# dbolya/yolact

Hardware: AMD Instinct MI355X
Metric: images/sec (550x550, batch 8 per GPU), YOLACT yolact_resnet50 forward + Detect (Fast NMS) (higher is better)
Workload: dtype f32 (fp32 in / fp32 accumulate / fp32 out; 93 % of the GEMM time on fp16x2 tiles = every fp32 operand as two fp16 pieces by round to nearest (22 significant bits + 2 signs: exact for ~2/3 of all fp32 values, one fp32 ulp otherwise), 3 exact piece products per product on the fp16 matrix pipe; measure

## Files before the change

include/yolact_amd.h:

```cpp
#ifndef YOLACT_AMD_H
#define YOLACT_AMD_H
#include <stddef.h>
#include <stdint.h>

#ifdef __cplusplus
extern "C" {
#endif

#define YMI_ABI_VERSION 9

#define YMI_EFORMAT (-4)
#define YMI_EUNSUPPORTED (-5)

enum { YMI_ACT_NONE = 0, YMI_ACT_RELU = 1, YMI_ACT_LEAKY01 = 2, YMI_ACT_TANH = 3, YMI_ACT_SIGMOID = 4 };
enum { YMI_RES_NONE = 0, YMI_RES_ADD = 1, YMI_RES_BILINEAR = 2 };

typedef struct {
  int32_t n0, n1;
  int32_t act;
  int32_t row_stride;
  int64_t batch_stride;
  float *ptr;
} ymi_conv_seg;

typedef struct {
  const float *x;
  const float *w;
  const float *scale;
  const float *bias;
  const float *res;
  int32_t B, H, W, Cin, ldx;
  int32_t Ho, Wo, Cout;
  int32_t kh, kw, stride, pad;
  int32_t Kpad;
  int32_t res_mode;
  int32_t res_ld;
  int32_t res_H, res_W;
  int32_t res_after_act;
  int32_t nseg;
  int32_t tile;
  int32_t cin_alg;
  int32_t split_k;
  ymi_conv_seg seg[3];
  const void *w_x3;
  float *split_ws;
  int32_t cout_alg;
  int32_t _pad2;
  const void *w_h2;
  const float *scale_h2;
  const float *winv_h2;
  const float *x_amax;
  float *y_amax;
  float x_amax_mul;
  int32_t _pad3;
} ymi_conv_desc;

enum { YMI_TILE_AUTO = 0, YMI_TILE_128x128 = 1, YMI_TILE_128x64 = 2, YMI_TILE_64x64 = 3, YMI_TILE_128x32 = 4,
       YMI_TILE_64x128 = 5, YMI_TILE_32x32_K4 = 6, YMI_TILE_64x32_K2 = 7, YMI_TILE_32x64_K2 = 8,
       YMI_TILE_64x64_S3 = 9, YMI_TILE_64x64_S4 = 10, YMI_TILE_64x128_S3 = 11, YMI_TILE_128x64_S3 = 12,
       YMI_TILE_32x32_K4_S4 = 13, YMI_TILE_64x32_K2_S3 = 14, YMI_TILE_32x64_K2_S3 = 15,
       YMI_TILE_128x128_W8 = 16, YMI_TILE_256x128_W8 = 17, YMI_TILE_128x256_W8 = 18,
       YMI_TILE_128x128_S3 = 19, YMI_TILE_128x128_W8_S3 = 20, YMI_TILE_256x128_W8_S3 = 21, YMI_TILE_128x128_W8_S4 = 22,
       YMI_TILE_WG_128x256 = 23,
       YMI_TILE_X3 = 32,
       YMI_TILE_H2 = 64,
       YMI_TILE_DCNP = 128 };
enum { YMI_DCNP_64x128 = 1, YMI_DCNP_64x128_W8 = 2, YMI_DCNP_64x64 = 3, YMI_DCNP_128x128_W8 = 4, YMI_DCNP_128x64_W8 = 5,
       YMI_DCNP_32x128 = 6,
       YMI_DCNP_96x128_W6 = 7, YMI_DCNP_128x128_W8_R1 = 8, YMI_DCNP_160x128_W10 = 9, YMI_DCNP_192x128_W12 = 10,
       YMI_DCNP_64x256_W8 = 11, YMI_DCNP_96x256_W12 = 12, YMI_DCNP_128x256_W16 = 13,
       YMI_DCNP_128x256_W8T = 14, YMI_DCNP_128x128_W4T = 15, YMI_DCNP_256x128_W8T = 16,
       YMI_DCNP_128x32_W4 = 17, YMI_DCNP_256x32_W8 = 18, YMI_DCNP_64x32_W2 = 19,
       YMI_DCNP_WS_128x32_W4 = 20, YMI_DCNP_WS_256x32_W8 = 21, YMI_DCNP_WS_256x32_W4 = 22, YMI_DCNP_WS_512x32_W8 = 23,
       YMI_DCNP_WS_128x64_W4 = 24, YMI_DCNP_WS_256x64_W8 = 25, YMI_DCNP_WS_256x64_W4 = 26, YMI_DCNP_WS_512x64_W8 = 27,
       YMI_DCNP_PATCH_C64 = 28,
       YMI_DCNP_PC_128x128 = 29,
       YMI_DCNP_PATCH2_256 = 30, YMI_DCNP_PATCH2_192 = 31 };

int ymi_abi_version(void);
const char *ymi_strerror(int code);

int ymi_conv2d_nhwc_f32(const ymi_conv_desc *d, void *stream);
double ymi_conv_flops(const ymi_conv_desc *d);
int ymi_conv_pick_tile(const ymi_conv_desc *d);

typedef struct {
  const float *x;
  const float *u;
  const float *scale;
  const float *bias;
  float *y;
  float *V, *M;
  int32_t B, H, W, C, Cout;
  int32_t act;
  int32_t tile;
  int32_t nseg;
  int32_t m;
  int32_t _pad0;
  ymi_conv_seg seg[3];
  const void *u_x3;
  int32_t cout_alg;
  int32_t v_planes;
  const void *u_h2;
  const float *uinv_h2;
  const float *x_amax;
  float *y_amax;
  const float *x_up;
  int32_t up_relu, _pad4;
  const void *proj_w_h2;
  const float *proj_scale_h2, *proj_bias;
  float *proj_y, *proj_y_amax;
  int32_t proj_cout, proj_ldy, proj_act, _pad5;
} ymi_wino_desc;
int ymi_conv3x3_winograd_f32(const ymi_wino_desc *d, void *stream);

#define YMI_AMAX_SUB 16
#define YMI_AMAX_STRIDE 64
int ymi_amax_f32(const float *x, long n, float *out, void *stream);

int ymi_nchw_to_nhwc4_f32(const float *x, float *y, int B, int C, int H, int W, void *stream);
int ymi_nchw_to_nhwc4_amax_f32(const float *x, float *y, int B, int C, int H, int W, float *amax, void *stream);
int ymi_nhwc_to_nchw_f32(const float *x, float *y, int B, int C, int H, int W, void *stream);
int ymi_maxpool3x3s2_nhwc_f32(const float *x, float *y, int B, int H, int W, int C, int Ho, int Wo, void *stream);
int ymi_bilinear_nhwc_f32(const float *x, float *y, int B, int Hi, int Wi, int C, int Ho, int Wo,
                          float scale_h, float scale_w, int relu, void *stream);

int ymi_bilinear_add_nhwc_f32(const float *x, float *y, int B, int Hi, int Wi, int C, int Ho, int Wo, float *y_amax, void *stream);

int ymi_conv2d_direct_nhwc_f32(const float *x, const float *w, const float *bias, float *y, int B, int H, int W,
                               int Cin, int Ho, int Wo, int Cout, int kh, int kw, int stride, int pad, int relu,
                               void *stream);
int ymi_global_maxpool_nhwc_f32(const float *x, float *y, int B, int HW, int C, void *stream);

typedef struct {
  const float *conf;
  const float *loc;
  const float *coef;
  const float *priors;
  int32_t B, P, C, D;
  int32_t conf_is_logits;
  int32_t top_k;
  int32_t max_det;
  float conf_thresh;
  float nms_thresh;
  int32_t cross_class;
  int32_t conf_ld;
  int32_t _pad1;
  float *scores_t;
  int32_t *keep;
  int32_t *num_keep;
  float *maxsc;
  int32_t *argmax;
  float *cand_score;
  int32_t *cand_prior;
  int32_t *out_count;
  float *out_box;
  float *out_score;
  int64_t *out_class;
  float *out_coef;
  int32_t *out_prior;
  float *out_rec;
} ymi_detect_desc;
int ymi_detect_f32(const ymi_detect_desc *d, void *stream);

typedef struct {
  float box_scale;
  int32_t _pad0;
  void *ws;
} ymi_detect_greedy_ws;
int ymi_detect_traditional_f32(const ymi_detect_desc *d, const ymi_detect_greedy_ws *g, void *stream);

int ymi_lincomb_crop_f32(const float *proto, const float *coef, const float *box, float *masks_lo,
                         int ph, int pw, int D, int N, int crop, void *stream);
int ymi_mask_upsample_f32(const float *masks_lo, float *out, int N, int ph, int pw, int h, int w,
                          float thresh, void *stream);
int ymi_lincomb_crop_batch_f32(const float *proto, const float *coef, const float *box, const int32_t *count,
                               float *masks_lo, int B, int cap, int ph, int pw, int D, int crop, void *stream);
int ymi_mask_upsample_batch_f32(const float *masks_lo, const int32_t *count, float *out, int B, int cap, int ph, int pw,
                                int h, int w, float thresh, void *stream);
int ymi_boxes_to_pixels(const float *box, int64_t *out, int N, int w, int h, void *stream);

int ymi_fast_base_transform_f32(const float *img, float *out, int N, int H, int W, int oh, int ow,
                                const float *mean_bgr, const float *std_bgr, int mode, int out_nhwc4, void *stream);

int ymi_mask_iou_f32(const float *masks_a, const float *masks_b, int A, int B, long n, int iscrowd, float *ws, float *iou,
                     void *stream);

int ymi_jaccard_f32(const float *box_a, const float *box_b, int A, int B, int iscrowd, float *out, void *stream);
int ymi_mask_bits_f32(const float *masks, int N, long n, uint64_t *bits, void *stream);
int ymi_mask_upsample_bits(const float *masks_lo, int N, int ph, int pw, int h, int w, float thresh, uint64_t *bits, void *stream);
int ymi_mask_iou_bits(const uint64_t *bits_a, const uint64_t *bits_b, int A, int B, long W64, int iscrowd, float *iou, void *stream);

#define YMI_AP_NUM_THRESH 10
#define YMI_AP_MAX_DET 1024
#define YMI_AP_MAX_GT 2048
typedef struct {
  const int64_t *cls;
  const float *box_score;
  const float *mask_score;
  const float *box_iou;
  const float *mask_iou;
  const float *crowd_box_iou;
  const float *crowd_mask_iou;
  const int32_t *gt_cls;
  const int32_t *crowd_cls;
  int64_t *rec_key;
  float *rec_score;
  int32_t *rec_flags;
  int64_t *gt_count;
  int64_t base, cap;
  int32_t N, G, Gc, num_classes;
} ymi_ap_match_desc;
typedef struct {
  const int64_t *sorted_key;
  const int64_t *perm;
  const int32_t *rec_flags;
  const int64_t *gt_count;
  double *ap;
  int32_t *empty;
  int64_t M, cap;
  int32_t num_classes, _pad0;
} ymi_ap_finalize_desc;
int ymi_ap_match_f32(const ymi_ap_match_desc *d, void *stream);
int ymi_ap_finalize_f64(const ymi_ap_finalize_desc *d, void *stream);

int ymi_composite_masks_u8(const float *img, const float *masks, const float *colors, int n, int h, int w, float alpha,
                           unsigned char *out, void *stream);

int ymi_mask_rle_f32(const float *masks, int N, int h, int w, uint32_t *counts, int32_t *nruns, int cap, void *stream);
int ymi_mask_rle_upsampled_f32(const float *masks_lo, int N, int ph, int pw, int h, int w, float thresh, uint32_t *counts,
                               int32_t *nruns, int cap, void *stream);
int ymi_rle_to_string(const uint32_t *counts, const int32_t *nruns, int N, int cap, uint8_t *str, int32_t *nchars,
                      int cap_chars, void *stream);

enum { YMI_JPEG_YCBCR = 0, YMI_JPEG_RGB = 1, YMI_JPEG_GRAY = 2 };
typedef struct {
  int32_t width, height;
  int32_t ncomp;
  int32_t progressive;
  int32_t orientation;
  int32_t color;
  int32_t out_width, out_height;
  int32_t hs[3], vs[3];
  int32_t hf[3], vf[3];
  int32_t bw[3], bh[3];
  int32_t dw[3], dh[3];
  int64_t coef_count;
  int64_t plane_bytes;
} ymi_jpeg_info;
int ymi_jpeg_parse(const uint8_t *data, size_t n, ymi_jpeg_info *info);
int ymi_jpeg_decode_coefs(const uint8_t *data, size_t n, int16_t *coefs, int64_t coef_capacity, uint16_t *qt,
                          ymi_jpeg_info *info);
int ymi_jpeg_reconstruct_bgr_u8(const ymi_jpeg_info *info, const int16_t *coefs, const uint16_t *qt, uint8_t *planes_ws,
                                uint8_t *out, void *stream);

enum { YMI_JPEG_SUB_444 = 0, YMI_JPEG_SUB_420 = 2 };
#define YMI_JPEG_HEADER_BYTES 623
typedef struct ymi_jpeg_enc_desc {
  const uint8_t *img;
  int32_t h, w;
  int64_t row_stride;
  int32_t quality;
  int32_t subsampling;
  uint8_t *out;
  int64_t out_capacity;
  int64_t *out_len;
  void *ws;
} ymi_jpeg_enc_desc;
int ymi_jpeg_write_header(int h, int w, int quality, int subsampling, uint8_t *out, size_t cap, size_t *n);
int ymi_jpeg_enc_qtables(int quality, uint16_t *qt);
int ymi_jpeg_encode_bgr_u8(const ymi_jpeg_enc_desc *d, void *stream);

int ymi_coco_poly_fill_u8(const double *xy, int k, int h, int w, uint8_t *mask);
int ymi_coco_rle_fill_u8(const uint32_t *counts, long n, int h, int w, uint8_t *mask);
int ymi_coco_rle_string_fill_u8(const char *s, long len, int h, int w, uint8_t *mask);

typedef struct {
  ymi_conv_desc conv;
  const float *offmask;
  int32_t ldo;
  int32_t mask_is_prob;
  int32_t om_layout;
  int32_t _pad1;
} ymi_dcn_desc;
int ymi_dcn_v2_forward_f32(const ymi_dcn_desc *d, void *stream);

typedef struct ymi_dcn_bwd_desc {
  const float *x;
  const float *offmask;
  const float *w;
  const float *gy;
  float *gx;
  float *g_offset;
  float *g_mask;
  float *gw;
  float *gbias;
  int32_t B, H, W, Cin, ldx, Ho, Wo, Cout;
  int32_t kh, kw, stride, pad, dilation, deformable_groups;
  int32_t ldo, mask_is_prob, om_layout, _pad0;
} ymi_dcn_bwd_desc;
int ymi_dcn_v2_backward_f32(const ymi_dcn_bwd_desc *d, void *stream);

typedef struct ymi_stem_desc {
  const float *x;
  float *y;
  int32_t B, H, W, cout_pad;
  const void *w_h2;
  const float *scale_h2, *bias;
  float *y_amax;
  int32_t kpad, _pad0;
} ymi_stem_desc;
int ymi_stem_pool_f32(const ymi_stem_desc *d, void *stream);

typedef struct ymi_chain_desc {
  const float *x, *res;
  float *y, *z;
  const void *w_a_h2, *w_b_h2;
  const float *scale_a_h2, *bias_a, *scale_b_h2, *bias_b;
  const float *x_amax;
  float *y_amax, *z_amax;
  int64_t M;
  int32_t ldx, res_ld, ldy, ldz;
  int32_t k_a, n_a, n_b;
  int32_t cout_pad_a, cout_pad_b;
  int32_t act_a, act_b, _pad0;
  const float *res_amax;
  float gain_a, bias_max_a;
} ymi_chain_desc;
int ymi_pointwise_chain_f32(const ymi_chain_desc *d, void *stream);

enum { YMI_OP_NOP = 0, YMI_OP_CONV = 1, YMI_OP_WINO = 2, YMI_OP_DCN = 3, YMI_OP_CHAIN = 4, YMI_OP_STEM = 5, YMI_OP_INPUT = 6,
       YMI_OP_BILINEAR = 7, YMI_OP_MAXPOOL = 8, YMI_OP_BILINEAR_ADD = 9, YMI_OP_RECORD = 10, YMI_OP_WAIT = 11, YMI_OP_MEMSET = 12 };
enum { YMI_SEC_NONE = 0, YMI_SEC_BACKBONE = 1, YMI_SEC_FPN = 2, YMI_SEC_PROTO = 3, YMI_SEC_HEADS = 4 };
typedef struct ymi_plan_op {
  int32_t kind;
  int32_t stream;
  int32_t section;
  int32_t _pad;
  const void *desc;
  void *p[3];
  int64_t i[8];
  double f[2];
} ymi_plan_op;
int ymi_event_create(void **ev);
int ymi_event_destroy(void *ev);
int ymi_plan_run(const ymi_plan_op *ops, int first, int last, void *stream_a, void *stream_b, void *const *events, int overlap,
                 int skip_sections, int32_t *failed_op);

enum {
  YMI_WS_WINO_V = 1,
  YMI_WS_WINO_M = 2,
  YMI_WS_SPLITK = 3,
  YMI_WS_MASK_IOU = 4,
  YMI_WS_JPEG_COEFS = 5,
  YMI_WS_JPEG_PLANES = 6,
  YMI_WS_DETECT_SCORES_T = 7,
  YMI_WS_DETECT_PER_PRIOR = 8,
  YMI_WS_DETECT_CAND = 9,
  YMI_WS_DETECT_REC = 10,
  YMI_WS_AMAX_SLOT = 11,
  YMI_WS_RLE_COUNTS = 12,
  YMI_WS_DETECT_GREEDY = 13,
  YMI_WS_JPEG_ENC = 14,
  YMI_WS_JPEG_ENC_OUT = 15
};
typedef struct { int32_t A, B; int64_t n; } ymi_mask_iou_shape;
typedef struct { int32_t N, h, w, cap; } ymi_rle_shape;
int64_t ymi_workspace_bytes(int what, const void *desc);

int ymi_calib_mfma_f16(float *out, int blocks, int iters, double *flops, void *stream);
int ymi_calib_hbm_copy(const float *src, float *dst, long n_floats, double *bytes, void *stream);
int ymi_calib_l2_read(const float *src, long n_floats, int blocks, int iters, float *out, double *bytes, void *stream);
int ymi_calib_latency(const int32_t *chain, long n, int start, int hops, int32_t *out, void *stream);

int ymi_debug_set_trace(void *buf, long cap_blocks);
int ymi_prof_enable(int on);
int ymi_prof_count(void);
int ymi_prof_read(int i, float *ms, double *flops, int32_t *tile, int32_t *kind);
int ymi_prof_reset(void);

#ifdef __cplusplus
}
#endif
#endif
```

yolact_amd/_lib.py:

```python
from __future__ import annotations

import ctypes as C
import os

_HERE = os.path.dirname(os.path.abspath(__file__))
LIB_PATH = os.path.join(_HERE, 'libyolact_amd.so')

ABI_VERSION = 9

ACT_NONE, ACT_RELU, ACT_LEAKY01, ACT_TANH, ACT_SIGMOID = 0, 1, 2, 3, 4
RES_NONE, RES_ADD, RES_BILINEAR = 0, 1, 2
TILE_AUTO, TILE_128x128, TILE_128x64, TILE_64x64, TILE_128x32, TILE_64x128 = 0, 1, 2, 3, 4, 5
TILE_32x32_K4, TILE_64x32_K2, TILE_32x64_K2 = 6, 7, 8
TILE_64x64_S3, TILE_64x64_S4, TILE_64x128_S3, TILE_128x64_S3, TILE_32x32_K4_S4, TILE_64x32_K2_S3, TILE_32x64_K2_S3 = range(9, 16)
TILE_NAMES = {1: '128x128', 2: '128x64', 3: '64x64', 4: '128x32', 5: '64x128', 6: '32x32k4', 7: '64x32k2', 8: '32x64k2',
              9: '64x64s3', 10: '64x64s4', 11: '64x128s3', 12: '128x64s3', 13: '32x32k4s4', 14: '64x32k2s3', 15: '32x64k2s3',
              16: '128x128w8', 17: '256x128w8', 18: '128x256w8', 19: '128x128s3', 20: '128x128w8s3', 21: '256x128w8s3',
              22: '128x128w8s4'}
TILE_128x128_W8, TILE_256x128_W8, TILE_128x256_W8 = 16, 17, 18
TILE_128x128_S3, TILE_128x128_W8_S3, TILE_256x128_W8_S3, TILE_128x128_W8_S4 = 19, 20, 21, 22
TILE_WG_128x256 = 23
TILE_X3 = 32
X3_BASE_TILES = (1, 2, 3, 5, 6, 7, 8, 9, 11, 12, 16, 17, 19, 20, 21, 22)
for _t in X3_BASE_TILES:
    TILE_NAMES[_t | TILE_X3] = TILE_NAMES[_t] + 'x3'
BASIC_TILES = (1, 2, 3, 4, 5)
TILE_H2 = 64
H2_BASE_TILES = X3_BASE_TILES + (18, 13, 14, 15)
for _t in H2_BASE_TILES:
    TILE_NAMES[_t | TILE_H2] = TILE_NAMES[_t] + 'h2'
TILE_NAMES[TILE_WG_128x256 | TILE_H2] = 'wg128x256h2'
TILE_DCNP = 128
DCNP_64x128, DCNP_64x128_W8, DCNP_64x64, DCNP_128x128_W8, DCNP_128x64_W8, DCNP_32x128 = 1, 2, 3, 4, 5, 6
DCNP_96x128_W6, DCNP_128x128_W8_R1, DCNP_160x128_W10, DCNP_192x128_W12, DCNP_64x256_W8, DCNP_96x256_W12, DCNP_128x256_W16 = range(7, 14)
DCNP_TILES = {1: 'dcnp64x128', 2: 'dcnp64x128w8', 3: 'dcnp64x64', 4: 'dcnp128x128w8', 5: 'dcnp128x64w8', 6: 'dcnp32x128',
              7: 'dcnp96x128w6', 8: 'dcnp128x128w8r1', 9: 'dcnp160x128w10', 10: 'dcnp192x128w12',
              11: 'dcnp64x256w8', 12: 'dcnp96x256w12', 13: 'dcnp128x256w16',
              14: 'dcnp128x256w8t', 15: 'dcnp128x128w4t', 16: 'dcnp256x128w8t',
              17: 'dcnp128x32w4', 18: 'dcnp256x32w8', 19: 'dcnp64x32w2'}
DCNP_128x32_W4, DCNP_256x32_W8, DCNP_64x32_W2 = 17, 18, 19
DCNP_PLAIN_ONLY = (14, 15, 16, 17, 18, 19)
WS_TILES = {20: 'ws128x32w4', 21: 'ws256x32w8', 22: 'ws256x32w4', 23: 'ws512x32w8',
            24: 'ws128x64w4', 25: 'ws256x64w8', 26: 'ws256x64w4', 27: 'ws512x64w8'}
DCNP_WS_128x32_W4, DCNP_WS_512x64_W8 = 20, 27
DCNP_PATCH_C64 = 28
PATCH_TILES = {28: 'patch8x16c64'}
PC_TILES = {29: 'pc128x128'}
DCNP_PC_128x128 = 29
PATCH2_TILES = {30: 'patch2p256', 31: 'patch2p192'}
DCNP_PATCH2_256, DCNP_PATCH2_192 = 30, 31
for _t, _n in list(DCNP_TILES.items()) + list(WS_TILES.items()) + list(PATCH_TILES.items()) + list(PC_TILES.items()) + list(PATCH2_TILES.items()):
    TILE_NAMES[_t | TILE_H2 | TILE_DCNP] = _n
WINO_PLANES = 1024
KSPLIT_TILES = (6, 7, 8, 13, 14, 15, 6 | 32, 7 | 32, 8 | 32, 6 | 64, 7 | 64, 8 | 64, 13 | 64, 14 | 64, 15 | 64)


class ConvSeg(C.Structure):
    _fields_ = [('n0', C.c_int32), ('n1', C.c_int32), ('act', C.c_int32), ('row_stride', C.c_int32),
                ('batch_stride', C.c_int64), ('ptr', C.c_void_p)]


class ConvDesc(C.Structure):
    _fields_ = [('x', C.c_void_p), ('w', C.c_void_p), ('scale', C.c_void_p), ('bias', C.c_void_p),
                ('res', C.c_void_p),
                ('B', C.c_int32), ('H', C.c_int32), ('W', C.c_int32), ('Cin', C.c_int32), ('ldx', C.c_int32),
                ('Ho', C.c_int32), ('Wo', C.c_int32), ('Cout', C.c_int32),
                ('kh', C.c_int32), ('kw', C.c_int32), ('stride', C.c_int32), ('pad', C.c_int32),
                ('Kpad', C.c_int32), ('res_mode', C.c_int32), ('res_ld', C.c_int32),
                ('res_H', C.c_int32), ('res_W', C.c_int32), ('res_after_act', C.c_int32),
                ('nseg', C.c_int32), ('tile', C.c_int32), ('cin_alg', C.c_int32), ('split_k', C.c_int32),
                ('seg', ConvSeg * 3), ('w_x3', C.c_void_p), ('split_ws', C.c_void_p), ('cout_alg', C.c_int32),
                ('_pad2', C.c_int32),
                ('w_h2', C.c_void_p), ('scale_h2', C.c_void_p), ('winv_h2', C.c_void_p), ('x_amax', C.c_void_p),
                ('y_amax', C.c_void_p), ('x_amax_mul', C.c_float), ('_pad3', C.c_int32)]


class WinoDesc(C.Structure):
    _fields_ = [('x', C.c_void_p), ('u', C.c_void_p), ('scale', C.c_void_p), ('bias', C.c_void_p), ('y', C.c_void_p),
                ('V', C.c_void_p), ('M', C.c_void_p),
                ('B', C.c_int32), ('H', C.c_int32), ('W', C.c_int32), ('C', C.c_int32), ('Cout', C.c_int32),
                ('act', C.c_int32), ('tile', C.c_int32), ('nseg', C.c_int32), ('m', C.c_int32), ('_pad0', C.c_int32),
                ('seg', ConvSeg * 3), ('u_x3', C.c_void_p), ('cout_alg', C.c_int32), ('v_planes', C.c_int32),
                ('u_h2', C.c_void_p), ('uinv_h2', C.c_void_p), ('x_amax', C.c_void_p), ('y_amax', C.c_void_p),
                ('x_up', C.c_void_p), ('up_relu', C.c_int32), ('_pad4', C.c_int32),
                ('proj_w_h2', C.c_void_p), ('proj_scale_h2', C.c_void_p), ('proj_bias', C.c_void_p),
                ('proj_y', C.c_void_p), ('proj_y_amax', C.c_void_p),
                ('proj_cout', C.c_int32), ('proj_ldy', C.c_int32), ('proj_act', C.c_int32), ('_pad5', C.c_int32)]


class DcnDesc(C.Structure):
    _fields_ = [('conv', ConvDesc), ('offmask', C.c_void_p), ('ldo', C.c_int32), ('mask_is_prob', C.c_int32),
                ('om_layout', C.c_int32), ('_pad1', C.c_int32)]


class DcnBwdDesc(C.Structure):
    _fields_ = [('x', C.c_void_p), ('offmask', C.c_void_p), ('w', C.c_void_p), ('gy', C.c_void_p),
                ('gx', C.c_void_p), ('g_offset', C.c_void_p), ('g_mask', C.c_void_p), ('gw', C.c_void_p), ('gbias', C.c_void_p),
                ('B', C.c_int32), ('H', C.c_int32), ('W', C.c_int32), ('Cin', C.c_int32), ('ldx', C.c_int32),
                ('Ho', C.c_int32), ('Wo', C.c_int32), ('Cout', C.c_int32),
                ('kh', C.c_int32), ('kw', C.c_int32), ('stride', C.c_int32), ('pad', C.c_int32), ('dilation', C.c_int32),
                ('deformable_groups', C.c_int32),
                ('ldo', C.c_int32), ('mask_is_prob', C.c_int32), ('om_layout', C.c_int32), ('_pad0', C.c_int32)]


class DetectDesc(C.Structure):
    _fields_ = [('conf', C.c_void_p), ('loc', C.c_void_p), ('coef', C.c_void_p), ('priors', C.c_void_p),
                ('B', C.c_int32), ('P', C.c_int32), ('C', C.c_int32), ('D', C.c_int32),
                ('conf_is_logits', C.c_int32), ('top_k', C.c_int32), ('max_det', C.c_int32),
                ('conf_thresh', C.c_float), ('nms_thresh', C.c_float), ('cross_class', C.c_int32),
                ('conf_ld', C.c_int32), ('_pad1', C.c_int32),
                ('scores_t', C.c_void_p), ('keep', C.c_void_p), ('num_keep', C.c_void_p),
                ('maxsc', C.c_void_p), ('argmax', C.c_void_p),
                ('cand_score', C.c_void_p), ('cand_prior', C.c_void_p),
                ('out_count', C.c_void_p), ('out_box', C.c_void_p), ('out_score', C.c_void_p),
                ('out_class', C.c_void_p), ('out_coef', C.c_void_p), ('out_prior', C.c_void_p), ('out_rec', C.c_void_p)]


class DetectGreedyWs(C.Structure):
    _fields_ = [('box_scale', C.c_float), ('_pad0', C.c_int32), ('ws', C.c_void_p)]


class JpegInfo(C.Structure):
    _fields_ = [('width', C.c_int32), ('height', C.c_int32), ('ncomp', C.c_int32), ('progressive', C.c_int32),
                ('orientation', C.c_int32), ('color', C.c_int32), ('out_width', C.c_int32), ('out_height', C.c_int32),
                ('hs', C.c_int32 * 3), ('vs', C.c_int32 * 3), ('hf', C.c_int32 * 3), ('vf', C.c_int32 * 3),
                ('bw', C.c_int32 * 3), ('bh', C.c_int32 * 3), ('dw', C.c_int32 * 3), ('dh', C.c_int32 * 3),
                ('coef_count', C.c_int64), ('plane_bytes', C.c_int64)]


class JpegEncDesc(C.Structure):
    _fields_ = [('img', C.c_void_p), ('h', C.c_int32), ('w', C.c_int32), ('row_stride', C.c_int64), ('quality', C.c_int32),
                ('subsampling', C.c_int32), ('out', C.c_void_p), ('out_capacity', C.c_int64), ('out_len', C.c_void_p),
                ('ws', C.c_void_p)]


JPEG_SUB_444, JPEG_SUB_420 = 0, 2
JPEG_HEADER_BYTES = 623


class ChainDesc(C.Structure):
    _fields_ = [('x', C.c_void_p), ('res', C.c_void_p), ('y', C.c_void_p), ('z', C.c_void_p),
                ('w_a_h2', C.c_void_p), ('w_b_h2', C.c_void_p),
                ('scale_a_h2', C.c_void_p), ('bias_a', C.c_void_p), ('scale_b_h2', C.c_void_p), ('bias_b', C.c_void_p),
                ('x_amax', C.c_void_p), ('y_amax', C.c_void_p), ('z_amax', C.c_void_p),
                ('M', C.c_int64), ('ldx', C.c_int32), ('res_ld', C.c_int32), ('ldy', C.c_int32), ('ldz', C.c_int32),
                ('k_a', C.c_int32), ('n_a', C.c_int32), ('n_b', C.c_int32), ('cout_pad_a', C.c_int32), ('cout_pad_b', C.c_int32),
                ('act_a', C.c_int32), ('act_b', C.c_int32), ('_pad0', C.c_int32),
                ('res_amax', C.c_void_p), ('gain_a', C.c_float), ('bias_max_a', C.c_float)]


class StemDesc(C.Structure):
    _fields_ = [('x', C.c_void_p), ('y', C.c_void_p), ('B', C.c_int32), ('H', C.c_int32), ('W', C.c_int32), ('cout_pad', C.c_int32),
                ('w_h2', C.c_void_p), ('scale_h2', C.c_void_p), ('bias', C.c_void_p), ('y_amax', C.c_void_p),
                ('kpad', C.c_int32), ('_pad0', C.c_int32)]


class PlanOp(C.Structure):
    _fields_ = [('kind', C.c_int32), ('stream', C.c_int32), ('section', C.c_int32), ('_pad', C.c_int32), ('desc', C.c_void_p),
                ('p', C.c_void_p * 3), ('i', C.c_int64 * 8), ('f', C.c_double * 2)]


(OP_NOP, OP_CONV, OP_WINO, OP_DCN, OP_CHAIN, OP_STEM, OP_INPUT, OP_BILINEAR, OP_MAXPOOL, OP_BILINEAR_ADD, OP_RECORD, OP_WAIT,
 OP_MEMSET) = range(13)
SEC_NONE, SEC_BACKBONE, SEC_FPN, SEC_PROTO, SEC_HEADS = range(5)


class MaskIouShape(C.Structure):
    _fields_ = [('A', C.c_int32), ('B', C.c_int32), ('n', C.c_int64)]


class ApMatchDesc(C.Structure):
    _fields_ = [('cls', C.c_void_p), ('box_score', C.c_void_p), ('mask_score', C.c_void_p), ('box_iou', C.c_void_p),
                ('mask_iou', C.c_void_p), ('crowd_box_iou', C.c_void_p), ('crowd_mask_iou', C.c_void_p), ('gt_cls', C.c_void_p),
                ('crowd_cls', C.c_void_p), ('rec_key', C.c_void_p), ('rec_score', C.c_void_p), ('rec_flags', C.c_void_p),
                ('gt_count', C.c_void_p), ('base', C.c_int64), ('cap', C.c_int64),
                ('N', C.c_int32), ('G', C.c_int32), ('Gc', C.c_int32), ('num_classes', C.c_int32)]


class ApFinalizeDesc(C.Structure):
    _fields_ = [('sorted_key', C.c_void_p), ('perm', C.c_void_p), ('rec_flags', C.c_void_p), ('gt_count', C.c_void_p),
                ('ap', C.c_void_p), ('empty', C.c_void_p), ('M', C.c_int64), ('cap', C.c_int64),
                ('num_classes', C.c_int32), ('_pad0', C.c_int32)]


AP_NUM_THRESH, AP_MAX_DET, AP_MAX_GT = 10, 1024, 2048


class RleShape(C.Structure):
    _fields_ = [('N', C.c_int32), ('h', C.c_int32), ('w', C.c_int32), ('cap', C.c_int32)]


(WS_WINO_V, WS_WINO_M, WS_SPLITK, WS_MASK_IOU, WS_JPEG_COEFS, WS_JPEG_PLANES, WS_DETECT_SCORES_T, WS_DETECT_PER_PRIOR,
 WS_DETECT_CAND, WS_DETECT_REC, WS_AMAX_SLOT, WS_RLE_COUNTS, WS_DETECT_GREEDY, WS_JPEG_ENC, WS_JPEG_ENC_OUT) = range(1, 16)

EFORMAT, EUNSUPPORTED = -4, -5

_P, _I, _F = C.c_void_p, C.c_int, C.c_float
SYMBOLS = [
    ('ymi_abi_version', C.c_int, []),
    ('ymi_strerror', C.c_char_p, [C.c_int]),
    ('ymi_conv2d_nhwc_f32', C.c_int, [C.POINTER(ConvDesc), _P]),
    ('ymi_conv3x3_winograd_f32', C.c_int, [C.POINTER(WinoDesc), _P]),
    ('ymi_conv_flops', C.c_double, [C.POINTER(ConvDesc)]),
    ('ymi_conv_pick_tile', C.c_int, [C.POINTER(ConvDesc)]),
    ('ymi_amax_f32', C.c_int, [_P, C.c_long, _P, _P]),
    ('ymi_nchw_to_nhwc4_f32', C.c_int, [_P, _P, _I, _I, _I, _I, _P]),
    ('ymi_nchw_to_nhwc4_amax_f32', C.c_int, [_P, _P, _I, _I, _I, _I, _P, _P]),
    ('ymi_nhwc_to_nchw_f32', C.c_int, [_P, _P, _I, _I, _I, _I, _P]),
    ('ymi_maxpool3x3s2_nhwc_f32', C.c_int, [_P, _P, _I, _I, _I, _I, _I, _I, _P]),
    ('ymi_bilinear_nhwc_f32', C.c_int, [_P, _P, _I, _I, _I, _I, _I, _I, _F, _F, _I, _P]),
    ('ymi_bilinear_add_nhwc_f32', C.c_int, [_P, _P, _I, _I, _I, _I, _I, _I, _P, _P]),
    ('ymi_conv2d_direct_nhwc_f32', C.c_int, [_P, _P, _P, _P] + [_I] * 12 + [_P]),
    ('ymi_global_maxpool_nhwc_f32', C.c_int, [_P, _P, _I, _I, _I, _P]),
    ('ymi_detect_f32', C.c_int, [C.POINTER(DetectDesc), _P]),
    ('ymi_detect_traditional_f32', C.c_int, [C.POINTER(DetectDesc), C.POINTER(DetectGreedyWs), _P]),
    ('ymi_lincomb_crop_f32', C.c_int, [_P, _P, _P, _P, _I, _I, _I, _I, _I, _P]),
    ('ymi_mask_upsample_f32', C.c_int, [_P, _P, _I, _I, _I, _I, _I, _F, _P]),
    ('ymi_lincomb_crop_batch_f32', C.c_int, [_P, _P, _P, _P, _P, _I, _I, _I, _I, _I, _I, _P]),
    ('ymi_mask_upsample_batch_f32', C.c_int, [_P, _P, _P, _I, _I, _I, _I, _I, _I, _F, _P]),
    ('ymi_boxes_to_pixels', C.c_int, [_P, _P, _I, _I, _I, _P]),
    ('ymi_dcn_v2_forward_f32', C.c_int, [C.POINTER(DcnDesc), _P]),
    ('ymi_dcn_v2_backward_f32', C.c_int, [C.POINTER(DcnBwdDesc), _P]),
    ('ymi_composite_masks_u8', C.c_int, [_P, _P, _P, _I, _I, _I, _F, _P, _P]),
    ('ymi_mask_iou_f32', C.c_int, [_P, _P, _I, _I, C.c_long, _I, _P, _P, _P]),
    ('ymi_jaccard_f32', C.c_int, [_P, _P, _I, _I, _I, _P, _P]),
    ('ymi_mask_bits_f32', C.c_int, [_P, _I, C.c_long, _P, _P]),
    ('ymi_mask_upsample_bits', C.c_int, [_P, _I, _I, _I, _I, _I, _F, _P, _P]),
    ('ymi_mask_iou_bits', C.c_int, [_P, _P, _I, _I, C.c_long, _I, _P, _P]),
    ('ymi_ap_match_f32', C.c_int, [C.POINTER(ApMatchDesc), _P]),
    ('ymi_ap_finalize_f64', C.c_int, [C.POINTER(ApFinalizeDesc), _P]),
    ('ymi_stem_pool_f32', C.c_int, [_P, _P]),
    ('ymi_pointwise_chain_f32', C.c_int, [_P, _P]),
    ('ymi_mask_rle_f32', C.c_int, [_P, _I, _I, _I, _P, _P, _I, _P]),
    ('ymi_mask_rle_upsampled_f32', C.c_int, [_P, _I, _I, _I, _I, _I, _F, _P, _P, _I, _P]),
    ('ymi_rle_to_string', C.c_int, [_P, _P, _I, _I, _P, _P, _I, _P]),
    ('ymi_fast_base_transform_f32', C.c_int, [_P, _P, _I, _I, _I, _I, _I, C.POINTER(C.c_float), C.POINTER(C.c_float), _I, _I, _P]),
    ('ymi_jpeg_parse', C.c_int, [_P, C.c_size_t, C.POINTER(JpegInfo)]),
    ('ymi_jpeg_decode_coefs', C.c_int, [_P, C.c_size_t, _P, C.c_int64, _P, C.POINTER(JpegInfo)]),
    ('ymi_jpeg_reconstruct_bgr_u8', C.c_int, [C.POINTER(JpegInfo), _P, _P, _P, _P, _P]),
    ('ymi_jpeg_write_header', C.c_int, [_I, _I, _I, _I, _P, C.c_size_t, C.POINTER(C.c_size_t)]),
    ('ymi_jpeg_enc_qtables', C.c_int, [_I, _P]),
    ('ymi_jpeg_encode_bgr_u8', C.c_int, [C.POINTER(JpegEncDesc), _P]),
    ('ymi_coco_poly_fill_u8', C.c_int, [_P, _I, _I, _I, _P]),
    ('ymi_coco_rle_fill_u8', C.c_int, [_P, C.c_long, _I, _I, _P]),
    ('ymi_coco_rle_string_fill_u8', C.c_int, [C.c_char_p, C.c_long, _I, _I, _P]),
    ('ymi_event_create', C.c_int, [C.POINTER(C.c_void_p)]),
    ('ymi_event_destroy', C.c_int, [_P]),
    ('ymi_plan_run', C.c_int, [C.POINTER(PlanOp), _I, _I, _P, _P, C.POINTER(C.c_void_p), _I, _I, C.POINTER(C.c_int32)]),
    ('ymi_workspace_bytes', C.c_int64, [_I, _P]),
    ('ymi_calib_mfma_f16', C.c_int, [_P, _I, _I, C.POINTER(C.c_double), _P]),
    ('ymi_calib_hbm_copy', C.c_int, [_P, _P, C.c_long, C.POINTER(C.c_double), _P]),
    ('ymi_calib_l2_read', C.c_int, [_P, C.c_long, _I, _I, _P, C.POINTER(C.c_double), _P]),
    ('ymi_calib_latency', C.c_int, [_P, C.c_long, _I, _I, _P, _P]),
    ('ymi_debug_set_trace', C.c_int, [_P, C.c_long]),
    ('ymi_prof_enable', C.c_int, [_I]),
    ('ymi_prof_count', C.c_int, []),
    ('ymi_prof_read', C.c_int, [_I, C.POINTER(C.c_float), C.POINTER(C.c_double), C.POINTER(C.c_int32),
                                C.POINTER(C.c_int32)]),
    ('ymi_prof_reset', C.c_int, []),
]

_lib = None


def lib():
    global _lib
    if _lib is None:
        if not os.path.exists(LIB_PATH):
            raise RuntimeError(
                'yolact_amd: HIP library %s not found. Build it with `python -c "import __graft_entry__ as g; '
                'g.build()"` or `make -C yolact_amd/csrc`. There is no CPU fallback.' % LIB_PATH)
        l = C.CDLL(LIB_PATH)
        for name, res, args in SYMBOLS:
            fn = getattr(l, name)
            fn.restype = res
            fn.argtypes = args
        if l.ymi_abi_version() != ABI_VERSION:
            raise RuntimeError('yolact_amd: ABI mismatch: library %d, binding %d' % (l.ymi_abi_version(), ABI_VERSION))
        _lib = l
    return _lib


def check(rc: int, what: str = ''):
    if rc != 0:
        msg = lib().ymi_strerror(rc).decode()
        raise RuntimeError('yolact_amd: %s failed: %s (code %d)' % (what or 'call', msg, rc))


def stream_ptr():
    import torch
    return C.c_void_p(torch.cuda.current_stream().cuda_stream)


def require_cuda(t, name='tensor'):
    if not t.is_cuda:
        raise RuntimeError('yolact_amd: %s must live on the GPU (MI355X/HIP); there is no CPU path in the product '
                           '(the CPU oracle lives under oracle/ and is test-only)' % name)
```

yolact_amd/csrc/plan_exec.cpp:

```cpp
#include "../../include/yolact_amd.h"
#include <hip/hip_runtime_api.h>

extern "C" {

int ymi_event_create(void **ev) {
  if (!ev) return -3;
  hipEvent_t e;
  const hipError_t rc = hipEventCreateWithFlags(&e, hipEventDisableTiming);
  if (rc != hipSuccess) return (int)rc;
  *ev = (void *)e;
  return 0;
}

int ymi_event_destroy(void *ev) {
  if (!ev) return -3;
  return (int)hipEventDestroy((hipEvent_t)ev);
}

int ymi_plan_run(const ymi_plan_op *ops, int first, int last, void *stream_a, void *stream_b, void *const *events, int overlap,
                 int skip_sections, int32_t *failed_op) {
  if (!ops || first < 0 || last < first) return -1;
  void *const sb = overlap ? stream_b : stream_a;
  for (int k = first; k < last; ++k) {
    const ymi_plan_op &o = ops[k];
    if (o.section && (skip_sections & (1 << o.section))) continue;
    void *const s = o.stream == 1 ? sb : stream_a;
    int rc = 0;
    switch (o.kind) {
      case YMI_OP_NOP: break;
      case YMI_OP_CONV: rc = ymi_conv2d_nhwc_f32((const ymi_conv_desc *)o.desc, s); break;
      case YMI_OP_WINO: rc = ymi_conv3x3_winograd_f32((const ymi_wino_desc *)o.desc, s); break;
      case YMI_OP_DCN: rc = ymi_dcn_v2_forward_f32((const ymi_dcn_desc *)o.desc, s); break;
      case YMI_OP_CHAIN: rc = ymi_pointwise_chain_f32((const ymi_chain_desc *)o.desc, s); break;
      case YMI_OP_STEM: rc = ymi_stem_pool_f32((const ymi_stem_desc *)o.desc, s); break;
      case YMI_OP_INPUT:
        rc = o.p[2] ? ymi_nchw_to_nhwc4_amax_f32((const float *)o.p[0], (float *)o.p[1], (int)o.i[0], (int)o.i[1], (int)o.i[2], (int)o.i[3],
                                                 (float *)o.p[2], s)
                    : ymi_nchw_to_nhwc4_f32((const float *)o.p[0], (float *)o.p[1], (int)o.i[0], (int)o.i[1], (int)o.i[2], (int)o.i[3], s);
        break;
      case YMI_OP_BILINEAR:
        rc = ymi_bilinear_nhwc_f32((const float *)o.p[0], (float *)o.p[1], (int)o.i[0], (int)o.i[1], (int)o.i[2], (int)o.i[3], (int)o.i[4],
                                   (int)o.i[5], (float)o.f[0], (float)o.f[1], (int)o.i[6], s);
        break;
      case YMI_OP_MAXPOOL:
        rc = ymi_maxpool3x3s2_nhwc_f32((const float *)o.p[0], (float *)o.p[1], (int)o.i[0], (int)o.i[1], (int)o.i[2], (int)o.i[3],
                                       (int)o.i[4], (int)o.i[5], s);
        break;
      case YMI_OP_BILINEAR_ADD:
        rc = ymi_bilinear_add_nhwc_f32((const float *)o.p[0], (float *)o.p[1], (int)o.i[0], (int)o.i[1], (int)o.i[2], (int)o.i[3],
                                       (int)o.i[4], (int)o.i[5], (float *)o.p[2], s);
        break;
      case YMI_OP_RECORD:
        if (overlap) rc = (int)hipEventRecord((hipEvent_t)events[o.i[0]], (hipStream_t)s);
        break;
      case YMI_OP_WAIT:
        if (overlap) rc = (int)hipStreamWaitEvent((hipStream_t)s, (hipEvent_t)events[o.i[0]], 0);
        break;
      case YMI_OP_MEMSET:
        rc = (int)hipMemsetAsync(o.p[0], 0, (size_t)o.i[0], (hipStream_t)s);
        break;
      default: rc = -1;
    }
    if (rc != 0) {
      if (failed_op) *failed_op = k;
      return rc;
    }
  }
  return 0;
}

}
```

yolact_amd/csrc/winograd.hip:

```cpp
#include "gemm_h2.h"

int ymi_internal_grouped_gemm(const ymi_conv_desc *d, int groups, long x_gs, long w_gs, long y_gs, double prof_flops,
                              int prof_kind, hipStream_t s, const void *a2 = nullptr, unsigned a2_plane = 0, long a2_gs = 0,
                              unsigned sc_gs = 0);
int ymi_internal_wgemm(const void *v, const void *u, const float *uinv, const float *x_amax, float amax_mul, float *m, int G, long T,
                       int C, int Ng, int cout_pad, double prof_flops, int prof_kind, hipStream_t s);
int ymi_internal_prof_begin(double flops, int tile, int kind, hipStream_t s);
void ymi_internal_prof_end(int idx, hipStream_t s);

namespace {

typedef _Float16 f16x4 __attribute__((ext_vector_type(4)));

__device__ __forceinline__ void store_v_planes(_Float16 *o, long e, long stride_e2, long plane, const f32x4 v, float s) {
  f16x4 h, l;
#pragma unroll
  for (int k = 0; k < 4; ++k) {
    const float t = v[k] * s;
    h[k] = (_Float16)t;
    l[k] = (_Float16)(t - (float)h[k]);
  }
  *reinterpret_cast<f16x4 *>(o + e * stride_e2) = h;
  *reinterpret_cast<f16x4 *>(o + e * stride_e2 + plane) = l;
}

__device__ __forceinline__ f32x4 ld4(const float *p, bool ok) {
  const f32x4 z = {0.f, 0.f, 0.f, 0.f};
  return ok ? *reinterpret_cast<const f32x4 *>(p) : z;
}

template <bool PLANES>
__global__ __launch_bounds__(256) void wino_in_k(const float *__restrict__ x, float *__restrict__ V, int H, int W, int C4,
                                                 int th, int tw, long T, long total, const float *__restrict__ x_amax) {
  float vs = 1.f, vinv = 1.f;
  if (PLANES) ymi_h2_scale(ymi_amax_read(x_amax) * 4.f, vs, vinv);
  for (unsigned i = blockIdx.x * 256u + threadIdx.x; i < (unsigned)total; i += gridDim.x * 256u) {
    const unsigned tu = i / (unsigned)C4, ru = tu / (unsigned)tw, bu = ru / (unsigned)th;
    const int c4 = (int)(i - tu * (unsigned)C4), tx = (int)(tu - ru * (unsigned)tw), ty = (int)(ru - bu * (unsigned)th);
    const long t = tu, b = bu;
    const int y0 = 2 * ty - 1, x0 = 2 * tx - 1;
    const float *base = x + ((b * H) * (long)W) * (C4 * 4L) + c4 * 4;
    f32x4 d[4][4];
#pragma unroll
    for (int iy = 0; iy < 4; ++iy) {
      const int yy = y0 + iy;
      const bool yok = (unsigned)yy < (unsigned)H;
#pragma unroll
      for (int ix = 0; ix < 4; ++ix) {
        const int xx = x0 + ix;
        const bool ok = yok && (unsigned)xx < (unsigned)W;
        d[iy][ix] = ld4(base + ((long)(ok ? yy : 0) * W + (ok ? xx : 0)) * (C4 * 4L), ok);
      }
    }
    f32x4 u[4][4];
#pragma unroll
    for (int j = 0; j < 4; ++j) {
      u[0][j] = d[0][j] - d[2][j];
      u[1][j] = d[1][j] + d[2][j];
      u[2][j] = d[2][j] - d[1][j];
      u[3][j] = d[1][j] - d[3][j];
    }
    const long stride_e = T * (C4 * 4L);
    float *o = V + t * (C4 * 4L) + c4 * 4;
    _Float16 *o2 = reinterpret_cast<_Float16 *>(V) + t * (C4 * 4L) + c4 * 4;
#pragma unroll
    for (int iy = 0; iy < 4; ++iy) {
      const f32x4 v0 = u[iy][0] - u[iy][2], v1 = u[iy][1] + u[iy][2], v2 = u[iy][2] - u[iy][1], v3 = u[iy][1] - u[iy][3];
      if (PLANES) {
        store_v_planes(o2, iy * 4 + 0, 2 * stride_e, stride_e, v0, vs);
        store_v_planes(o2, iy * 4 + 1, 2 * stride_e, stride_e, v1, vs);
        store_v_planes(o2, iy * 4 + 2, 2 * stride_e, stride_e, v2, vs);
        store_v_planes(o2, iy * 4 + 3, 2 * stride_e, stride_e, v3, vs);
      } else {
        *reinterpret_cast<f32x4 *>(o + (iy * 4 + 0) * stride_e) = v0;
        *reinterpret_cast<f32x4 *>(o + (iy * 4 + 1) * stride_e) = v1;
        *reinterpret_cast<f32x4 *>(o + (iy * 4 + 2) * stride_e) = v2;
        *reinterpret_cast<f32x4 *>(o + (iy * 4 + 3) * stride_e) = v3;
      }
    }
  }
}

__global__ __launch_bounds__(256) void wino_out_k(const float *__restrict__ Mm, float *__restrict__ y,
                                                  const float *__restrict__ scale, const float *__restrict__ bias, int Ho,
                                                  int Wo, int N4, int th, int tw, long T, int act, long total,
                                                  float *__restrict__ y_amax) {
  float am = 0.f;
  const ymi_amax_pre apre = ymi_amax_prefetch(y_amax);
  for (unsigned i = blockIdx.x * 256u + threadIdx.x; i < (unsigned)total; i += gridDim.x * 256u) {
    const unsigned tu = i / (unsigned)N4, ru = tu / (unsigned)tw, bu = ru / (unsigned)th;
    const int n4 = (int)(i - tu * (unsigned)N4), tx = (int)(tu - ru * (unsigned)tw), ty = (int)(ru - bu * (unsigned)th);
    const long t = tu, b = bu;
    const long stride_e = T * (N4 * 4L);
    const float *src = Mm + t * (N4 * 4L) + n4 * 4;
    f32x4 m[4][4];
#pragma unroll
    for (int e = 0; e < 16; ++e) m[e >> 2][e & 3] = *reinterpret_cast<const f32x4 *>(src + e * stride_e);
    f32x4 s[2][4];
#pragma unroll
    for (int j = 0; j < 4; ++j) {
      s[0][j] = (m[0][j] + m[1][j]) + m[2][j];
      s[1][j] = (m[1][j] - m[2][j]) - m[3][j];
    }
    f32x4 sc = {1.f, 1.f, 1.f, 1.f}, bi = {0.f, 0.f, 0.f, 0.f};
    if (scale) sc = *reinterpret_cast<const f32x4 *>(scale + n4 * 4);
    if (bias) bi = *reinterpret_cast<const f32x4 *>(bias + n4 * 4);
    const float slope = ymi_act_slope(act);
    f32x4 vv[2][2];
#pragma unroll
    for (int iy = 0; iy < 2; ++iy) {
      const f32x4 o0 = (s[iy][0] + s[iy][1]) + s[iy][2], o1 = (s[iy][1] - s[iy][2]) - s[iy][3];
#pragma unroll
      for (int ix = 0; ix < 2; ++ix) {
        f32x4 v = (ix == 0 ? o0 : o1) * sc + bi;
#pragma unroll
        for (int e = 0; e < 4; ++e) v[e] = fmaxf(v[e], slope * v[e]);
        vv[iy][ix] = v;
        const bool ok = 2 * ty + iy < Ho && 2 * tx + ix < Wo;
        am = fmaxf(am, ok ? ymi_absmax4(v) : 0.f);
      }
    }
#pragma unroll
    for (int iy = 0; iy < 2; ++iy)
#pragma unroll
      for (int ix = 0; ix < 2; ++ix) {
        const int oy = 2 * ty + iy, ox = 2 * tx + ix;
        if (oy < Ho && ox < Wo) *reinterpret_cast<f32x4 *>(y + ((b * Ho + oy) * (long)Wo + ox) * (N4 * 4L) + n4 * 4) = vv[iy][ix];
      }
  }
  if (y_amax) ymi_amax_finish(apre, am);
}

struct SegTab { ymi_conv_seg seg[3]; int nseg; };

__device__ __forceinline__ float wino_act(float v, int act) {
  switch (act) {
    case YMI_ACT_RELU: return v > 0.f ? v : 0.f;
    case YMI_ACT_LEAKY01: return v > 0.f ? v : 0.1f * v;
    case YMI_ACT_TANH: return tanhf(v);
    case YMI_ACT_SIGMOID: return 1.f / (1.f + expf(-v));
    default: return v;
  }
}

__device__ __forceinline__ int seg_vec4(const SegTab &st, int n, int Cout) {
  if (n + 3 >= Cout) return -1;
#pragma unroll
  for (int k = 0; k < 3; ++k)
    if (k < st.nseg && n >= st.seg[k].n0 && n + 3 < st.seg[k].n1 && ((n - st.seg[k].n0) & 3) == 0 &&
        (st.seg[k].row_stride & 3) == 0 && (st.seg[k].batch_stride & 3) == 0 && (((uintptr_t)st.seg[k].ptr) & 15) == 0)
      return k;
  return -1;
}

struct SegVec {
  float *ptr; long bs; int rs, act;
  f32x4 sc, bi;
};
__device__ __forceinline__ SegVec seg_vec_setup(const SegTab &st, int k, const float *__restrict__ scale,
                                                const float *__restrict__ bias, int n) {
  ymi_conv_seg sg = st.seg[0];
  if (k == 1) sg = st.seg[1];
  if (k == 2) sg = st.seg[2];
  SegVec v;
  v.ptr = sg.ptr + (n - sg.n0); v.bs = sg.batch_stride; v.rs = sg.row_stride; v.act = sg.act;
#pragma unroll
  for (int e = 0; e < 4; ++e) { v.sc[e] = scale ? scale[n + e] : 1.f; v.bi[e] = bias ? bias[n + e] : 0.f; }
  return v;
}

constexpr int YMI_AMAX_SLOT = YMI_AMAX_SUB * YMI_AMAX_STRIDE;
__device__ __forceinline__ void seg_amax_add(float (&am)[3], int k, float v) {
  am[0] = k == 0 ? fmaxf(am[0], v) : am[0];
  am[1] = k == 1 ? fmaxf(am[1], v) : am[1];
  am[2] = k == 2 ? fmaxf(am[2], v) : am[2];
}
__device__ __forceinline__ void seg_amax_commit(float *y_amax, int nseg, const ymi_amax_pre &apre0, const float (&am)[3]) {
  if (!y_amax) return;
  ymi_amax_finish(apre0, am[0]);
  if (nseg > 1) ymi_amax_finish(ymi_amax_prefetch(y_amax + YMI_AMAX_SLOT), am[1]);
  if (nseg > 2) ymi_amax_finish(ymi_amax_prefetch(y_amax + 2 * YMI_AMAX_SLOT), am[2]);
}

__device__ __forceinline__ float seg_vec_store(const SegVec &sv, f32x4 v, long b, long pix) {
  v = v * sv.sc + sv.bi;
  if (sv.act <= YMI_ACT_LEAKY01) {
    const float slope = ymi_act_slope(sv.act);
#pragma unroll
    for (int e = 0; e < 4; ++e) v[e] = fmaxf(v[e], slope * v[e]);
  } else {
#pragma unroll
    for (int e = 0; e < 4; ++e) v[e] = wino_act(v[e], sv.act);
  }
  *reinterpret_cast<f32x4 *>(sv.ptr + b * sv.bs + pix * sv.rs) = v;
  return ymi_absmax4(v);
}

__global__ __launch_bounds__(256) void wino_out_seg_k(const float *__restrict__ Mm, const SegTab st,
                                                      const float *__restrict__ scale, const float *__restrict__ bias,
                                                      int Ho, int Wo, int N4, int Cout, int th, int tw, long T, long total, float *__restrict__ y_amax) {
  float am[3] = {0.f, 0.f, 0.f};
  const ymi_amax_pre apre = ymi_amax_prefetch(y_amax);
  for (unsigned i = blockIdx.x * 256u + threadIdx.x; i < (unsigned)total; i += gridDim.x * 256u) {
    const unsigned tu = i / (unsigned)N4, ru = tu / (unsigned)tw, bu = ru / (unsigned)th;
    const int n4 = (int)(i - tu * (unsigned)N4), tx = (int)(tu - ru * (unsigned)tw), ty = (int)(ru - bu * (unsigned)th);
    const long t = tu, b = bu;
    const long stride_e = T * (N4 * 4L);
    const float *src = Mm + t * (N4 * 4L) + n4 * 4;
    f32x4 m[4][4];
#pragma unroll
    for (int e = 0; e < 16; ++e) m[e >> 2][e & 3] = *reinterpret_cast<const f32x4 *>(src + e * stride_e);
    f32x4 s[2][4];
#pragma unroll
    for (int j = 0; j < 4; ++j) {
      s[0][j] = (m[0][j] + m[1][j]) + m[2][j];
      s[1][j] = (m[1][j] - m[2][j]) - m[3][j];
    }
    f32x4 o[2][2];
#pragma unroll
    for (int iy = 0; iy < 2; ++iy) {
      o[iy][0] = (s[iy][0] + s[iy][1]) + s[iy][2];
      o[iy][1] = (s[iy][1] - s[iy][2]) - s[iy][3];
    }
    const int kv = seg_vec4(st, n4 * 4, Cout);
    if (kv >= 0) {
      const SegVec sv = seg_vec_setup(st, kv, scale, bias, n4 * 4);
#pragma unroll
      for (int iy = 0; iy < 2; ++iy)
#pragma unroll
        for (int ix = 0; ix < 2; ++ix) {
          const int oy = 2 * ty + iy, ox = 2 * tx + ix;
          if (oy < Ho && ox < Wo) seg_amax_add(am, kv, seg_vec_store(sv, o[iy][ix], b, (long)oy * Wo + ox));
        }
      continue;
    }
#pragma unroll
    for (int e = 0; e < 4; ++e) {
      const int n = n4 * 4 + e;
      if (n >= Cout) continue;
      float *ptr = nullptr; long bs = 0; int rs = 0, act = 0, n0 = 0, ks = 0;
#pragma unroll
      for (int k = 0; k < 3; ++k)
        if (k < st.nseg && n >= st.seg[k].n0 && n < st.seg[k].n1) {
          ptr = st.seg[k].ptr; bs = st.seg[k].batch_stride; rs = st.seg[k].row_stride; act = st.seg[k].act; n0 = st.seg[k].n0; ks = k;
        }
      if (!ptr) continue;
      const float sc = scale ? scale[n] : 1.f, bi = bias ? bias[n] : 0.f;
#pragma unroll
      for (int iy = 0; iy < 2; ++iy) {
        const int oy = 2 * ty + iy;
        if (oy >= Ho) continue;
#pragma unroll
        for (int ix = 0; ix < 2; ++ix) {
          const int ox = 2 * tx + ix;
          if (ox >= Wo) continue;
          const float val = wino_act(o[iy][ix][e] * sc + bi, act);
          seg_amax_add(am, ks, fabsf(val));
          ptr[b * bs + ((long)oy * Wo + ox) * rs + (n - n0)] = val;
        }
      }
    }
  }
  seg_amax_commit(y_amax, st.nseg, apre, am);
}


__device__ __forceinline__ void bt6(const f32x4 v0, const f32x4 v1, const f32x4 v2, const f32x4 v3, const f32x4 v4, const f32x4 v5,
                                    f32x4 &t0, f32x4 &t1, f32x4 &t2, f32x4 &t3, f32x4 &t4, f32x4 &t5) {
  const f32x4 a = v4 - v2 * 4.f, b = v3 - v1 * 4.f;
  const f32x4 c = v4 - v2, e = (v3 - v1) * 2.f;
  t0 = (v0 * 4.f - v2 * 5.f) + v4;
  t1 = a + b;
  t2 = a - b;
  t3 = c + e;
  t4 = c - e;
  t5 = (v1 * 4.f - v3 * 5.f) + v5;
}

__device__ __forceinline__ void up2_coord(int dst, int in_size, float &l1) {
  float src = 0.5f * ((float)dst + 0.5f) - 0.5f;
  src = src < 0.f ? 0.f : src;
  int i0 = (int)src;
  if (i0 > in_size - 1) i0 = in_size - 1;
  l1 = src - (float)i0;
}

template <bool PLANES, bool UPS = false>
__global__ __launch_bounds__(256) void wino43_in_k(const float *__restrict__ x, float *__restrict__ V, int H, int W, int C4,
                                                   int th, int tw, long T, long total, const float *__restrict__ x_amax,
                                                   int up_relu = 0) {
  float vs = 1.f, vinv = 1.f;
  if (PLANES) ymi_h2_scale(ymi_amax_read(x_amax) * 100.f, vs, vinv);
  for (unsigned i = blockIdx.x * 256u + threadIdx.x; i < (unsigned)total; i += gridDim.x * 256u) {
    const unsigned tu = i / (unsigned)C4, ru = tu / (unsigned)tw, bu = ru / (unsigned)th;
    const int c4 = (int)(i - tu * (unsigned)C4), tx = (int)(tu - ru * (unsigned)tw), ty = (int)(ru - bu * (unsigned)th);
    const long t = tu, b = bu;
    const int y0 = 4 * ty - 1, x0 = 4 * tx - 1;
    f32x4 u[6][6];
    if constexpr (UPS) {
      const int Hl = H >> 1, Wl = W >> 1;
      const float *lbase = x + ((b * Hl) * (long)Wl) * (C4 * 4L) + c4 * 4;
      f32x4 lo[4][4];
#pragma unroll
      for (int k = 0; k < 4; ++k) {
        int wy = 2 * ty - 1 + k; wy = wy < 0 ? 0 : (wy > Hl - 1 ? Hl - 1 : wy);
#pragma unroll
        for (int q = 0; q < 4; ++q) {
          int wx = 2 * tx - 1 + q; wx = wx < 0 ? 0 : (wx > Wl - 1 ? Wl - 1 : wx);
          lo[k][q] = *reinterpret_cast<const f32x4 *>(lbase + ((long)wy * Wl + wx) * (C4 * 4L));
        }
      }
      float lx[6], ly[6];
#pragma unroll
      for (int j = 0; j < 6; ++j) { up2_coord(x0 + j, Wl, lx[j]); up2_coord(y0 + j, Hl, ly[j]); }
      f32x4 hrow[4][6];
#pragma unroll
      for (int k = 0; k < 4; ++k)
#pragma unroll
        for (int j = 0; j < 6; ++j) hrow[k][j] = (1.f - lx[j]) * lo[k][j >> 1] + lx[j] * lo[k][(j >> 1) + 1];
#pragma unroll
      for (int j = 0; j < 6; ++j) {
        const bool xok = (unsigned)(x0 + j) < (unsigned)W;
        f32x4 dcol[6];
#pragma unroll
        for (int iy = 0; iy < 6; ++iy) {
          const bool ok = xok && (unsigned)(y0 + iy) < (unsigned)H;
          f32x4 v = (1.f - ly[iy]) * hrow[iy >> 1][j] + ly[iy] * hrow[(iy >> 1) + 1][j];
          if (up_relu) {
#pragma unroll
            for (int e = 0; e < 4; ++e) v[e] = v[e] < 0.f ? 0.f : v[e];
          }
          const f32x4 z = {0.f, 0.f, 0.f, 0.f};
          dcol[iy] = ok ? v : z;
        }
        bt6(dcol[0], dcol[1], dcol[2], dcol[3], dcol[4], dcol[5], u[0][j], u[1][j], u[2][j], u[3][j], u[4][j], u[5][j]);
      }
    } else {
    const float *base = x + ((b * H) * (long)W) * (C4 * 4L) + c4 * 4;
#pragma unroll
    for (int j = 0; j < 6; ++j) {
      const int xx = x0 + j;
      const bool xok = (unsigned)xx < (unsigned)W;
      f32x4 dcol[6];
#pragma unroll
      for (int iy = 0; iy < 6; ++iy) {
        const int yy = y0 + iy;
        const bool ok = xok && (unsigned)yy < (unsigned)H;
        dcol[iy] = ld4(base + ((long)(ok ? yy : 0) * W + (ok ? xx : 0)) * (C4 * 4L), ok);
      }
      bt6(dcol[0], dcol[1], dcol[2], dcol[3], dcol[4], dcol[5], u[0][j], u[1][j], u[2][j], u[3][j], u[4][j], u[5][j]);
    }
    }
    const long stride_e = T * (C4 * 4L);
    float *o = V + t * (C4 * 4L) + c4 * 4;
    _Float16 *o2 = reinterpret_cast<_Float16 *>(V) + t * (C4 * 4L) + c4 * 4;
#pragma unroll
    for (int iy = 0; iy < 6; ++iy) {
      f32x4 v[6];
      bt6(u[iy][0], u[iy][1], u[iy][2], u[iy][3], u[iy][4], u[iy][5], v[0], v[1], v[2], v[3], v[4], v[5]);
#pragma unroll
      for (int l = 0; l < 6; ++l) {
        if (PLANES) store_v_planes(o2, iy * 6 + l, 2 * stride_e, stride_e, v[l], vs);
        else *reinterpret_cast<f32x4 *>(o + (iy * 6 + l) * stride_e) = v[l];
      }
    }
  }
}

__device__ __forceinline__ void at6(const f32x4 v0, const f32x4 v1, const f32x4 v2, const f32x4 v3, const f32x4 v4, const f32x4 v5,
                                    f32x4 &s0, f32x4 &s1, f32x4 &s2, f32x4 &s3) {
  const f32x4 p12 = v1 + v2, m12 = v1 - v2, p34 = v3 + v4, m34 = v3 - v4;
  s0 = (v0 + p12) + p34;
  s1 = m12 + m34 * 2.f;
  s2 = p12 + p34 * 4.f;
  s3 = (m12 + m34 * 8.f) + v5;
}

__device__ __forceinline__ void wino43_out_tile(const float *__restrict__ src, long stride_e, f32x4 (&o)[4][4]) {
  f32x4 s[4][6];
#pragma unroll
  for (int j = 0; j < 6; ++j) {
    f32x4 mc[6];
#pragma unroll
    for (int iy = 0; iy < 6; ++iy) mc[iy] = *reinterpret_cast<const f32x4 *>(src + (iy * 6 + j) * stride_e);
    at6(mc[0], mc[1], mc[2], mc[3], mc[4], mc[5], s[0][j], s[1][j], s[2][j], s[3][j]);
  }
#pragma unroll
  for (int iy = 0; iy < 4; ++iy) at6(s[iy][0], s[iy][1], s[iy][2], s[iy][3], s[iy][4], s[iy][5], o[iy][0], o[iy][1], o[iy][2], o[iy][3]);
}

__global__ __launch_bounds__(256) void wino43_out_k(const float *__restrict__ Mm, float *__restrict__ y,
                                                    const float *__restrict__ scale, const float *__restrict__ bias, int Ho,
                                                    int Wo, int N4, int th, int tw, long T, int act, long total,
                                                    float *__restrict__ y_amax) {
  float am = 0.f;
  const ymi_amax_pre apre = ymi_amax_prefetch(y_amax);
  for (unsigned i = blockIdx.x * 256u + threadIdx.x; i < (unsigned)total; i += gridDim.x * 256u) {
    const unsigned tu = i / (unsigned)N4, ru = tu / (unsigned)tw, bu = ru / (unsigned)th;
    const int n4 = (int)(i - tu * (unsigned)N4), tx = (int)(tu - ru * (unsigned)tw), ty = (int)(ru - bu * (unsigned)th);
    const long t = tu, b = bu;
    f32x4 o[4][4];
    wino43_out_tile(Mm + t * (N4 * 4L) + n4 * 4, T * (N4 * 4L), o);
    f32x4 sc = {1.f, 1.f, 1.f, 1.f}, bi = {0.f, 0.f, 0.f, 0.f};
    if (scale) sc = *reinterpret_cast<const f32x4 *>(scale + n4 * 4);
    if (bias) bi = *reinterpret_cast<const f32x4 *>(bias + n4 * 4);
    const float slope = ymi_act_slope(act);
#pragma unroll
    for (int iy = 0; iy < 4; ++iy)
#pragma unroll
      for (int ix = 0; ix < 4; ++ix) {
        f32x4 v = o[iy][ix] * sc + bi;
#pragma unroll
        for (int e = 0; e < 4; ++e) v[e] = fmaxf(v[e], slope * v[e]);
        o[iy][ix] = v;
        const bool ok = 4 * ty + iy < Ho && 4 * tx + ix < Wo;
        am = fmaxf(am, ok ? ymi_absmax4(v) : 0.f);
      }
#pragma unroll
    for (int iy = 0; iy < 4; ++iy)
#pragma unroll
      for (int ix = 0; ix < 4; ++ix) {
        const int oy = 4 * ty + iy, ox = 4 * tx + ix;
        if (oy < Ho && ox < Wo) *reinterpret_cast<f32x4 *>(y + ((b * Ho + oy) * (long)Wo + ox) * (N4 * 4L) + n4 * 4) = o[iy][ix];
      }
  }
  if (y_amax) ymi_amax_finish(apre, am);
}

struct ProjArgs {
  const void *w_h2; const float *scale_h2, *bias; float *y, *y_amax;
  int cout, ldy, act; unsigned w_plane;
};
constexpr int PJ_ROW = 528, PJ_YPLANE = 16 * PJ_ROW, PJ_WPLANE = 32 * PJ_ROW, PJ_LDS = 2 * PJ_WPLANE + 4 * 2 * PJ_YPLANE;

__global__ __launch_bounds__(256) void wino43_out_proj_k(const float *__restrict__ Mm, const float *__restrict__ scale,
                                                         const float *__restrict__ bias, int Ho, int Wo, int th, int tw, long T,
                                                         int act, const ProjArgs pp) {
#if defined(__HIP_DEVICE_COMPILE__)
  __shared__ __attribute__((aligned(16))) char lds[PJ_LDS];
  typedef _Float16 f16x8 __attribute__((ext_vector_type(8)));
  typedef _Float16 f16x4 __attribute__((ext_vector_type(4)));
  const int t = threadIdx.x, lane = t & 63, wave = __builtin_amdgcn_readfirstlane(t >> 6);
  const int lr = lane & 15, g = lane >> 4;
  const ymi_amax_pre apre = ymi_amax_prefetch(pp.y_amax);
  for (int u = t; u < 2 * 32 * 32; u += 256) {
    const int plane = u >> 10, row = (u >> 5) & 31, pc = u & 31;
    const f32x4 v = *reinterpret_cast<const f32x4 *>(reinterpret_cast<const char *>(pp.w_h2) + (size_t)plane * pp.w_plane + (size_t)row * 512 + pc * 16);
    *reinterpret_cast<f32x4 *>(lds + plane * PJ_WPLANE + row * PJ_ROW + pc * 16) = v;
  }
  __syncthreads();
  char *ytile = lds + 2 * PJ_WPLANE + wave * (2 * PJ_YPLANE);
  f32x4 sc = {1.f, 1.f, 1.f, 1.f}, bi = {0.f, 0.f, 0.f, 0.f};
  if (scale) sc = *reinterpret_cast<const f32x4 *>(scale + lane * 4);
  if (bias) bi = *reinterpret_cast<const f32x4 *>(bias + lane * 4);
  const float slope = ymi_act_slope(act);
  const float slope2 = ymi_act_slope(pp.act);
  float am = 0.f;
  for (long tl = (long)blockIdx.x * 4 + wave; tl < T; tl += (long)gridDim.x * 4) {
    const unsigned tu = (unsigned)tl, ru = tu / (unsigned)tw, bu = ru / (unsigned)th;
    const int tx = (int)(tu - ru * (unsigned)tw), ty = (int)(ru - bu * (unsigned)th);
    f32x4 o[4][4];
    wino43_out_tile(Mm + tl * 256L + lane * 4, T * 256L, o);
    float tm = 0.f;
#pragma unroll
    for (int iy = 0; iy < 4; ++iy)
#pragma unroll
      for (int ix = 0; ix < 4; ++ix) {
        f32x4 v = o[iy][ix] * sc + bi;
#pragma unroll
        for (int e = 0; e < 4; ++e) v[e] = fmaxf(v[e], slope * v[e]);
        o[iy][ix] = v;
        tm = fmaxf(tm, ymi_absmax4(v));
      }
    const unsigned tmb = ymi_wave_umax63(__builtin_bit_cast(unsigned, tm));
    float sT, invT;
    ymi_h2_scale(__builtin_bit_cast(float, (unsigned)__builtin_amdgcn_readlane((int)tmb, 63)), sT, invT);
#pragma unroll
    for (int iy = 0; iy < 4; ++iy)
#pragma unroll
      for (int ix = 0; ix < 4; ++ix) {
        const f32x4 v = o[iy][ix] * sT;
        f16x4 h4, l4;
#pragma unroll
        for (int e = 0; e < 4; ++e) {
          const _Float16 h = (_Float16)v[e];
          h4[e] = h;
          l4[e] = (_Float16)(v[e] - (float)h);
        }
        char *dst = ytile + (iy * 4 + ix) * PJ_ROW + lane * 8;
        *reinterpret_cast<f16x4 *>(dst) = h4;
        *reinterpret_cast<f16x4 *>(dst + PJ_YPLANE) = l4;
      }
    __builtin_amdgcn_fence(__ATOMIC_RELEASE, "wavefront");
    __builtin_amdgcn_wave_barrier();
    f32x4 acc[2];
    acc[0] = f32x4{0.f, 0.f, 0.f, 0.f};
    acc[1] = f32x4{0.f, 0.f, 0.f, 0.f};
#pragma unroll
    for (int c = 0; c < 8; ++c) {
      const f16x8 xh = *reinterpret_cast<const f16x8 *>(ytile + lr * PJ_ROW + c * 64 + g * 16);
      const f16x8 xl = *reinterpret_cast<const f16x8 *>(ytile + PJ_YPLANE + lr * PJ_ROW + c * 64 + g * 16);
#pragma unroll
      for (int j = 0; j < 2; ++j) {
        const f16x8 wh = *reinterpret_cast<const f16x8 *>(lds + (j * 16 + lr) * PJ_ROW + c * 64 + g * 16);
        const f16x8 wl = *reinterpret_cast<const f16x8 *>(lds + PJ_WPLANE + (j * 16 + lr) * PJ_ROW + c * 64 + g * 16);
        acc[j] = ymi_mfma16(wl, xh, acc[j]);
        acc[j] = ymi_mfma16(wh, xl, acc[j]);
        acc[j] = ymi_mfma16(wh, xh, acc[j]);
      }
    }
    __builtin_amdgcn_fence(__ATOMIC_ACQUIRE, "wavefront");
    __builtin_amdgcn_wave_barrier();
    const int oy = 4 * ty + (lr >> 2), ox = 4 * tx + (lr & 3);
#pragma unroll
    for (int j = 0; j < 2; ++j) {
      const int n = j * 16 + 4 * g;
      if (n < pp.cout && oy < Ho && ox < Wo) {
        f32x4 v;
#pragma unroll
        for (int e = 0; e < 4; ++e) {
          const float r = acc[j][e] * (pp.scale_h2[n + e] * invT) + (pp.bias ? pp.bias[n + e] : 0.f);
          v[e] = fmaxf(r, slope2 * r);
        }
        am = fmaxf(am, ymi_absmax4(v));
        *reinterpret_cast<f32x4 *>(pp.y + (((long)bu * Ho + oy) * (long)Wo + ox) * pp.ldy + n) = v;
      }
    }
  }
  if (pp.y_amax) ymi_amax_finish(apre, am);
#endif
}

__global__ __launch_bounds__(256) void wino43_out_seg_k(const float *__restrict__ Mm, const SegTab st,
                                                        const float *__restrict__ scale, const float *__restrict__ bias,
                                                        int Ho, int Wo, int N4, int Cout, int th, int tw, long T, long total, float *__restrict__ y_amax) {
  float am[3] = {0.f, 0.f, 0.f};
  const ymi_amax_pre apre = ymi_amax_prefetch(y_amax);
  for (unsigned i = blockIdx.x * 256u + threadIdx.x; i < (unsigned)total; i += gridDim.x * 256u) {
    const unsigned tu = i / (unsigned)N4, ru = tu / (unsigned)tw, bu = ru / (unsigned)th;
    const int n4 = (int)(i - tu * (unsigned)N4), tx = (int)(tu - ru * (unsigned)tw), ty = (int)(ru - bu * (unsigned)th);
    const long t = tu, b = bu;
    f32x4 o[4][4];
    wino43_out_tile(Mm + t * (N4 * 4L) + n4 * 4, T * (N4 * 4L), o);
    const int kv = seg_vec4(st, n4 * 4, Cout);
    if (kv >= 0) {
      const SegVec sv = seg_vec_setup(st, kv, scale, bias, n4 * 4);
#pragma unroll
      for (int iy = 0; iy < 4; ++iy)
#pragma unroll
        for (int ix = 0; ix < 4; ++ix) {
          const int oy = 4 * ty + iy, ox = 4 * tx + ix;
          if (oy < Ho && ox < Wo) seg_amax_add(am, kv, seg_vec_store(sv, o[iy][ix], b, (long)oy * Wo + ox));
        }
      continue;
    }
#pragma unroll
    for (int e = 0; e < 4; ++e) {
      const int n = n4 * 4 + e;
      if (n >= Cout) continue;
      float *ptr = nullptr; long bs = 0; int rs = 0, act = 0, n0 = 0, ks = 0;
#pragma unroll
      for (int k = 0; k < 3; ++k)
        if (k < st.nseg && n >= st.seg[k].n0 && n < st.seg[k].n1) {
          ptr = st.seg[k].ptr; bs = st.seg[k].batch_stride; rs = st.seg[k].row_stride; act = st.seg[k].act; n0 = st.seg[k].n0; ks = k;
        }
      if (!ptr) continue;
      const float sc = scale ? scale[n] : 1.f, bi = bias ? bias[n] : 0.f;
#pragma unroll
      for (int iy = 0; iy < 4; ++iy) {
        const int oy = 4 * ty + iy;
        if (oy >= Ho) continue;
#pragma unroll
        for (int ix = 0; ix < 4; ++ix) {
          const int ox = 4 * tx + ix;
          if (ox >= Wo) continue;
          const float val = wino_act(o[iy][ix][e] * sc + bi, act);
          seg_amax_add(am, ks, fabsf(val));
          ptr[b * bs + ((long)oy * Wo + ox) * rs + (n - n0)] = val;
        }
      }
    }
  }
  seg_amax_commit(y_amax, st.nseg, apre, am);
}

unsigned grid_for(long total) {
  long g = (total + 255) / 256;
  const long cap = 256L * 64;
  return (unsigned)(g > cap ? cap : g);
}

}

extern "C" int ymi_conv3x3_winograd_f32(const ymi_wino_desc *d, void *stream) {
  if (!d || (!d->x && !d->x_up) || !d->u || !d->V || !d->M) return YMI_ENULL;
  if (d->x_up && (d->m != 4 || (d->H & 1) || (d->W & 1) || (((uintptr_t)d->x_up) & 15))) return YMI_ESHAPE;
  if (d->B <= 0 || d->H <= 0 || d->W <= 0 || d->C <= 0 || d->Cout <= 0 || d->nseg < 0 || d->nseg > 3) return YMI_EARG;
  const bool proj = d->proj_w_h2 != nullptr;
  if (proj && (d->m != 4 || d->nseg != 0 || d->Cout != 256 || d->proj_cout <= 0 || d->proj_cout > 32 || (d->proj_cout & 3) ||
               (d->proj_ldy & 3) || d->proj_ldy < d->proj_cout || d->proj_act > YMI_ACT_LEAKY01 || d->proj_act < 0))
    return YMI_ESHAPE;
  if (proj && (!d->proj_scale_h2 || !d->proj_y || (((uintptr_t)d->proj_w_h2) & 15) || (((uintptr_t)d->proj_y) & 15))) return YMI_ENULL;
  if (d->nseg == 0 && ((!d->y && !proj) || (d->Cout & 3) || d->act > YMI_ACT_LEAKY01 || d->act < 0)) return YMI_ESHAPE;
  for (int k = 0; k < d->nseg; ++k) if (!d->seg[k].ptr) return YMI_ENULL;
  if (d->C & 31) return YMI_ESHAPE;
  if (d->m != 0 && d->m != 2 && d->m != 4) return YMI_EARG;
  const int mt = d->m == 4 ? 4 : 2;
  const int ng = (mt + 2) * (mt + 2);
  const int Ng = (d->Cout + 3) / 4 * 4;
  hipStream_t s = (hipStream_t)stream;
  const int th = (d->H + mt - 1) / mt, tw = (d->W + mt - 1) / mt;
  const long T = (long)d->B * th * tw;
  if (T * (long)(d->C > Ng ? d->C : Ng) >= (1L << 29)) return YMI_ESHAPE;
  const int C4 = d->C / 4, N4 = Ng / 4;
  const double alg = 2.0 * d->B * d->H * d->W * (double)(d->cout_alg > 0 ? d->cout_alg : d->Cout) * 9.0 * d->C;
  const double exe = 2.0 * ng * (double)T * d->C * Ng;
  const int outer = ymi_internal_prof_begin(alg, d->tile ? d->tile : YMI_TILE_64x64, mt == 4 ? 4 : 3, s);
  const bool h2 = (d->tile & YMI_TILE_H2) != 0;
  if (h2 && (!d->u_h2 || !d->uinv_h2 || !d->x_amax)) return YMI_ENULL;
  const bool planes = h2 && d->v_planes != 0;
#ifdef YMI_DIAGNOSTICS
  static const int wabl = [] { const char *e = getenv("YMI_WINO_ABLATE"); return e ? atoi(e) : 0; }();
  if (!(wabl & 1)) {
#endif
  if (mt == 4) {
    if (d->x_up) {
      if (planes) hipLaunchKernelGGL((wino43_in_k<true, true>), dim3(grid_for(T * C4)), dim3(256), 0, s, d->x_up, d->V, d->H, d->W, C4, th, tw, T, T * C4, d->x_amax, d->up_relu);
      else hipLaunchKernelGGL((wino43_in_k<false, true>), dim3(grid_for(T * C4)), dim3(256), 0, s, d->x_up, d->V, d->H, d->W, C4, th, tw, T, T * C4, d->x_amax, d->up_relu);
    } else if (planes) hipLaunchKernelGGL((wino43_in_k<true, false>), dim3(grid_for(T * C4)), dim3(256), 0, s, d->x, d->V, d->H, d->W, C4, th, tw, T, T * C4, d->x_amax, 0);
    else hipLaunchKernelGGL((wino43_in_k<false, false>), dim3(grid_for(T * C4)), dim3(256), 0, s, d->x, d->V, d->H, d->W, C4, th, tw, T, T * C4, d->x_amax, 0);
  } else {
    if (planes) hipLaunchKernelGGL(wino_in_k<true>, dim3(grid_for(T * C4)), dim3(256), 0, s, d->x, d->V, d->H, d->W, C4, th, tw, T, T * C4, d->x_amax);
    else hipLaunchKernelGGL(wino_in_k<false>, dim3(grid_for(T * C4)), dim3(256), 0, s, d->x, d->V, d->H, d->W, C4, th, tw, T, T * C4, d->x_amax);
  }
#ifdef YMI_DIAGNOSTICS
  }
#endif
  int rc = ymi_launch_status();
  if (rc) return rc;
  ymi_conv_desc g = {};
  g.x = d->V; g.w = d->u;
  g.B = 1; g.H = (int)T; g.W = 1; g.Cin = d->C; g.ldx = d->C;
  g.Ho = (int)T; g.Wo = 1; g.Cout = Ng;
  g.kh = g.kw = 1; g.stride = 1; g.pad = 0; g.Kpad = d->C;
  g.nseg = 1; g.tile = d->tile;
  g.w_x3 = d->u_x3;
  g.w_h2 = d->u_h2; g.scale_h2 = d->uinv_h2; g.winv_h2 = d->uinv_h2;
  g.x_amax = d->x_amax; g.x_amax_mul = mt == 4 ? 100.f : 4.f;
  g.seg[0].n0 = 0; g.seg[0].n1 = Ng; g.seg[0].act = YMI_ACT_NONE; g.seg[0].row_stride = Ng;
  g.seg[0].batch_stride = T * Ng; g.seg[0].ptr = d->M;
  const long cout_pad = ((long)d->Cout + 127) / 128 * 128;
  if ((d->tile & 31) == YMI_TILE_WG_128x256) {
    if (!planes || (d->tile & YMI_TILE_X3)) return YMI_EARG;
    rc = ymi_internal_wgemm(d->V, d->u_h2, d->uinv_h2, d->x_amax, mt == 4 ? 100.f : 4.f, d->M, ng, T, d->C, Ng, (int)cout_pad, exe,
                            mt == 4 ? 6 : 5, s);
  } else if (planes)
    rc = ymi_internal_grouped_gemm(&g, ng, T * d->C, cout_pad * d->C, T * Ng, exe, mt == 4 ? 6 : 5, s, d->V,
                                   (unsigned)(T * d->C * 2), 2L * T * d->C * 2, (unsigned)cout_pad);
  else
    rc = ymi_internal_grouped_gemm(&g, ng, T * d->C, cout_pad * d->C, T * Ng, exe, mt == 4 ? 6 : 5 , s,
                                   nullptr, 0, 0, (unsigned)cout_pad);
  if (rc) return rc;
  if (d->nseg > 0) {
    SegTab st;
    st.nseg = d->nseg;
    for (int k = 0; k < 3; ++k) st.seg[k] = d->seg[k];
    if (mt == 4)
      hipLaunchKernelGGL(wino43_out_seg_k, dim3(grid_for(T * N4)), dim3(256), 0, s, d->M, st, d->scale, d->bias, d->H, d->W,
                         N4, d->Cout, th, tw, T, T * N4, d->y_amax);
    else
      hipLaunchKernelGGL(wino_out_seg_k, dim3(grid_for(T * N4)), dim3(256), 0, s, d->M, st, d->scale, d->bias, d->H, d->W, N4,
                         d->Cout, th, tw, T, T * N4, d->y_amax);
    rc = ymi_launch_status();
    ymi_internal_prof_end(outer, s);
    return rc;
  }
  if (proj) {
    ProjArgs pa;
    pa.w_h2 = d->proj_w_h2; pa.scale_h2 = d->proj_scale_h2; pa.bias = d->proj_bias; pa.y = d->proj_y; pa.y_amax = d->proj_y_amax;
    pa.cout = d->proj_cout; pa.ldy = d->proj_ldy; pa.act = d->proj_act; pa.w_plane = (unsigned)(128L * 256 * 2);
    const long blocks = (T + 3) / 4;
    hipLaunchKernelGGL(wino43_out_proj_k, dim3((unsigned)(blocks < 256 ? blocks : 256)), dim3(256), 0, s, d->M, d->scale, d->bias, d->H,
                       d->W, th, tw, T, d->act, pa);
    rc = ymi_launch_status();
    ymi_internal_prof_end(outer, s);
    if (rc == YMI_OK) {
      const int pr = ymi_internal_prof_begin(2.0 * d->B * d->H * d->W * 256.0 * d->proj_cout, d->tile ? d->tile : YMI_TILE_64x64, 12, s);
      ymi_internal_prof_end(pr, s);
    }
    return rc;
  }
  if (mt == 4)
    hipLaunchKernelGGL(wino43_out_k, dim3(grid_for(T * N4)), dim3(256), 0, s, d->M, d->y, d->scale, d->bias, d->H, d->W, N4, th,
                       tw, T, d->act, T * N4, d->y_amax);
  else
    hipLaunchKernelGGL(wino_out_k, dim3(grid_for(T * N4)), dim3(256), 0, s, d->M, d->y, d->scale, d->bias, d->H, d->W, N4, th,
                       tw, T, d->act, T * N4, d->y_amax);
  rc = ymi_launch_status();
  ymi_internal_prof_end(outer, s);
  return rc;
}
```

yolact_amd/engine.py:

```python
from __future__ import annotations

import ctypes as C
import json
import os
from typing import List, Optional

import torch
import torch.nn as nn

from . import _lib as L
from .config import act_name, make_priors_host
from . import modules as M


def _ceil(a, b):
    return (a + b - 1) // b * b


SPLIT_DEFAULT = '2'
TUNE_GEN = 5
AMAX_SLOT_FLOATS = 16 * 64
TUNE_DIR = os.path.join(os.path.dirname(os.path.abspath(__file__)), 'tune')
_table_cache = {}


def _read_table_file(path):
    try:
        with open(path) as f:
            doc = json.load(f)
    except (OSError, ValueError):
        return {}
    if not isinstance(doc, dict) or doc.get('gen') != TUNE_GEN or not isinstance(doc.get('abi'), int) or doc['abi'] > L.ABI_VERSION:
        return {}
    return dict(doc.get('entries', {}))


def _write_table_file(path, entries, device=None, note=None):
    doc = {'gen': TUNE_GEN, 'abi': L.ABI_VERSION,
           'device': torch.cuda.get_device_name(device) if device is not None and device.type == 'cuda' else None,
           'note': note or 'tile id per conv shape (B,H,W,Cin,Cout,kh,kw,stride,pad,res_mode,nseg,Kpad); wino(...) -> '
                           '[m, gemm tile, direct ms, winograd ms, F(2x2) ms, F(4x4) ms]',
           'entries': {k: entries[k] for k in sorted(entries)}}
    tmp = path + '.tmp%d' % os.getpid()
    with open(tmp, 'w') as f:
        json.dump(doc, f, indent=0, separators=(',', ':'))
    os.replace(tmp, path)


def load_tune_table(device):
    arch = 'gfx950'
    if device.type == 'cuda':
        arch = getattr(torch.cuda.get_device_properties(device), 'gcnArchName', 'gfx950').split(':')[0]
    if arch not in _table_cache:
        _table_cache[arch] = _read_table_file(os.path.join(TUNE_DIR, arch + '.json'))
    return dict(_table_cache[arch])


def build_meta():
    try:
        with open(os.path.join(os.path.dirname(os.path.abspath(__file__)), 'build_meta.json')) as f:
            doc = json.load(f)
        return doc if isinstance(doc, dict) else {}
    except (OSError, ValueError):
        return {}


def patch_tile_allowed():
    return os.environ.get('YOLACT_AMD_PATCH', '1') == '1' and build_meta().get('lint', 'ok') != 'skipped'


def split3_planes(w: torch.Tensor) -> torch.Tensor:
    w = w.detach().to(torch.float32).contiguous()
    mask = -65536

    def hi(t):
        u = t.view(torch.int32) & mask
        return u.view(torch.float32), (u >> 16).to(torch.int16)
    h, hb = hi(w)
    r = w - h
    m, mb = hi(r)
    r2 = r - m
    l, lb = hi(r2)
    assert bool(((h + m + l - w).abs() <= 1e-38).all()) or not torch.isfinite(w).all()
    return torch.stack([hb, mb, lb], dim=-3).contiguous()


def split2_planes_f16(w: torch.Tensor):
    w = w.detach().to(torch.float32).contiguous()
    amax = w.abs().amax(dim=-1)
    _, e = torch.frexp(amax)
    s = torch.ldexp(torch.ones_like(amax), 14 - e)
    s = torch.where(amax > 0, s, torch.ones_like(s))
    t = w * s.unsqueeze(-1)
    h = t.to(torch.float16)
    l = (t - h.to(torch.float32)).to(torch.float16)
    assert bool(torch.isfinite(h.float()).all()), 'fp16x2 filter planes overflowed'
    planes = torch.stack([h, l], dim=-3).contiguous().view(torch.int16)
    return planes, (1.0 / s).contiguous()


class Packed:

    def __init__(self, weight, bias=None, bn: Optional[nn.BatchNorm2d] = None, stride=1, pad=0, cin_pad=None,
                 device=None):
        weight = weight.detach().to(torch.float32)
        Cout, Cin, kh, kw = weight.shape
        cin_p = cin_pad or Cin
        w = weight.permute(0, 2, 3, 1)
        if cin_p != Cin:
            w = torch.nn.functional.pad(w, (0, cin_p - Cin))
        K = kh * kw * cin_p
        self.Kpad, self.CoutPad = _ceil(K, 32), _ceil(Cout, 128)
        wp = torch.zeros(self.CoutPad, self.Kpad, dtype=torch.float32, device=weight.device)
        wp[:Cout, :K] = w.reshape(Cout, K)
        self.w = wp.to(device).contiguous()
        self._wp_host, self._w3, self._h2 = wp, None, None
        self.weight_oihw = weight if (kh == 3 and kw == 3) else None
        self.Cin, self.Cout, self.kh, self.kw, self.stride, self.pad = cin_p, Cout, kh, kw, stride, pad
        self.cin_alg = Cin
        self.cout_alg = Cout
        scale = shift = None
        if bn is not None:
            invstd = 1.0 / torch.sqrt(bn.running_var.detach().float() + bn.eps)
            scale = bn.weight.detach().float() * invstd
            shift = bn.bias.detach().float() - bn.running_mean.detach().float() * scale
            if bias is not None:
                shift = shift + bias.detach().float() * scale
        elif bias is not None:
            shift = bias.detach().float()
        self.scale = scale.to(device).contiguous() if scale is not None else None
        self.bias = shift.to(device).contiguous() if shift is not None else None

    def tiny_columns(self, binades=10, in_gain=None):
        memo = getattr(self, '_tiny_memo', None)
        if memo is None:
            memo = self._tiny_memo = {}
        mkey = (binades, None if in_gain is None else (id(in_gain), int(in_gain.numel())))
        if mkey in memo and (in_gain is None or memo[mkey][1] is in_gain):
            return memo[mkey][0]
        r = self._tiny_columns(binades, in_gain)
        memo[mkey] = (r, in_gain)
        return r

    def _tiny_columns(self, binades, in_gain):
        w = self._wp_host[:self.Cout, :self.kh * self.kw * self.Cin].abs().float().cpu()
        col = w.view(self.Cout, self.kh * self.kw, self.Cin).amax(dim=(0, 1))
        nzm = col > 0
        if int(nzm.sum()) <= 8:
            return False
        tiny = nzm & (col * float(2 ** binades) < col[nzm].median())
        if not bool(tiny.any()):
            return False
        if in_gain is None:
            return True
        g = in_gain.detach().float().cpu().flatten()
        if g.numel() < self.Cin:
            g = torch.nn.functional.pad(g, (0, self.Cin - g.numel()))
        g = g[:self.Cin]
        pos = g[g > 0]
        if pos.numel() == 0:
            return True
        return bool((tiny & (g >= pos.median() * float(2 ** max(binades - 4, 1)))).any())

    def out_gain(self):
        if getattr(self, '_out_gain', None) is None:
            g = self._wp_host[:self.Cout].abs().amax(dim=1).float().cpu()
            if self.scale is not None:
                g = g * self.scale.detach().abs().float().cpu()
            if self.bias is not None:
                g = g + self.bias.detach().abs().float().cpu()[:self.Cout]
            self._out_gain = g
        return self._out_gain

    def _invalidate(self):
        self._w3 = self._h2 = None
        self._out_gain = self._l1_gain = None
        self._tiny_memo = {}

    def scale_out_channels(self, f: torch.Tensor):
        f = f.detach().float().cpu()
        dev = self.w.device
        sc = self.scale.detach().float().cpu() if self.scale is not None else torch.ones(self.Cout)
        self.scale = (sc * f).to(dev).contiguous()
        if self.bias is not None:
            self.bias = (self.bias.detach().float().cpu() * f).to(dev).contiguous()
        self._invalidate()

    def scale_in_channels(self, f: torch.Tensor):
        f = f.detach().float().cpu()
        taps = self.kh * self.kw
        assert self.Kpad == taps * self.Cin and f.numel() == self.Cin
        wp = self._wp_host.detach().float().cpu().clone()
        wp.view(self.CoutPad, taps, self.Cin).mul_(f.view(1, 1, -1))
        self._wp_host = wp
        self.w = wp.to(self.w.device).contiguous()
        if self.weight_oihw is not None:
            self.weight_oihw = self.weight_oihw.detach().float().cpu() * f.view(1, -1, 1, 1)
        self._invalidate()

    def in_column_max(self):
        w = self._wp_host[:self.Cout, :self.kh * self.kw * self.Cin].detach().abs().float().cpu()
        return w.view(self.Cout, self.kh * self.kw, self.Cin).amax(dim=(0, 1))

    def l1_gain(self):
        if getattr(self, '_l1_gain', None) is None:
            g = self._wp_host[:self.Cout].detach().cpu().abs().double().sum(dim=1)
            if self.scale is not None:
                g = g * self.scale.detach().abs().double().cpu()
            b = float(self.bias.detach().abs().max().cpu()) if self.bias is not None else 0.0
            self._l1_gain = (float(g.max()) * (1.0 + 2.0 ** -20), b)
        return self._l1_gain

    def w3(self):
        if self._w3 is None:
            self._w3 = split3_planes(self._wp_host.cpu()).to(self.w.device)
        return self._w3


    def h2(self):
        if self._h2 is None:
            planes, winv = split2_planes_f16(self._wp_host.cpu())
            sc = torch.ones(self.CoutPad, dtype=torch.float32, device='cpu')
            if self.scale is not None:
                sc[:self.Cout] = self.scale.detach().float().cpu()
            dev = self.w.device
            self._h2 = (planes.to(dev), (sc * winv).contiguous().to(dev), winv.to(dev))
        return self._h2


class WinoPacked:

    G2 = torch.tensor([[1.0, 0.0, 0.0], [0.5, 0.5, 0.5], [0.5, -0.5, 0.5], [0.0, 0.0, 1.0]], dtype=torch.float64)
    G4 = torch.tensor([[1 / 4, 0, 0], [-1 / 6, -1 / 6, -1 / 6], [-1 / 6, 1 / 6, -1 / 6], [1 / 24, 1 / 12, 1 / 6],
                       [1 / 24, -1 / 12, 1 / 6], [0, 0, 1]], dtype=torch.float64)

    def __init__(self, weight, device, m=2):
        w = weight.detach().to(torch.float64).cpu()
        Cout, Cin = w.shape[:2]
        G = self.G4 if m == 4 else self.G2
        a = m + 2
        u = torch.einsum('ai,ncij,bj->abnc', G, w, G)
        self.m = m
        self.CoutPad = _ceil(Cout, 128)
        up = torch.zeros(a * a, self.CoutPad, Cin, dtype=torch.float32)
        up[:, :Cout] = u.reshape(a * a, Cout, Cin).to(torch.float32)
        self.u = up.to(device).contiguous()
        self._up_host, self._u3, self._uh2 = up, None, None

    def u3(self):
        if self._u3 is None:
            self._u3 = split3_planes(self._up_host).to(self.u.device)
        return self._u3


def _wino_h2(self):
    if self._uh2 is None:
        planes, uinv = split2_planes_f16(self._up_host)
        self._uh2 = (planes.to(self.u.device), uinv.to(self.u.device))
    return self._uh2


WinoPacked.h2 = _wino_h2


def wino_eligible(pk, res, segs, act, x_C):
    if not (pk.kh == 3 and pk.kw == 3 and pk.stride == 1 and pk.pad == 1 and pk.Cin % 32 == 0
            and pk.cin_alg == pk.Cin and x_C == pk.Cin and res is None):
        return False
    if segs is not None:
        return len(segs) <= 3
    return pk.Cout % 4 == 0 and act in (L.ACT_NONE, L.ACT_RELU, L.ACT_LEAKY01)


def pack_offmask(conv: nn.Conv2d, device, interleave: bool) -> Packed:
    w, b = conv.weight.detach().float(), conv.bias.detach().float()
    assert w.shape[0] == 27 and conv.stride[0] == conv.stride[1] and conv.padding == (1, 1), 'conv_offset_mask of a 3x3 one-group DCN'
    order = [c for k in range(9) for c in (2 * k, 2 * k + 1, 18 + k)] if interleave else list(range(27))
    wp, bp = w.new_zeros((32,) + tuple(w.shape[1:])), b.new_zeros(32)
    wp[:27], bp[:27] = w[order], b[order]
    pk = Packed(wp, bp, None, conv.stride[0], 1, None, device)
    pk.cout_alg = 27
    return pk


def pack_module(conv: nn.Conv2d, bn=None, device=None, cin_pad=None) -> Packed:
    assert conv.dilation == (1, 1) and conv.groups == 1
    assert conv.stride[0] == conv.stride[1] and conv.padding[0] == conv.padding[1]
    return Packed(conv.weight, conv.bias, bn, conv.stride[0], conv.padding[0], cin_pad, device)


class T:
    __slots__ = ('buf', 'B', 'H', 'W', 'C', 'slot', 'gain')

    def __init__(self, buf, B, H, W, C, slot=None, gain=None):
        self.buf, self.B, self.H, self.W, self.C = buf, B, H, W, C
        self.slot = slot
        self.gain = gain

    @property
    def ptr(self):
        return self.buf.data_ptr()

    def view(self):
        return self.buf[: self.B * self.H * self.W * self.C].view(self.B, self.H, self.W, self.C)


class Arena:

    def __init__(self, device):
        self.device = device
        self.free_list: List[torch.Tensor] = []
        self.all: List[torch.Tensor] = []

    def alloc(self, numel) -> torch.Tensor:
        best = None
        for i, b in enumerate(self.free_list):
            if b.numel() >= numel and (best is None or b.numel() < self.free_list[best].numel()):
                best = i
        if best is not None:
            return self.free_list.pop(best)
        b = torch.empty(numel, dtype=torch.float32, device=self.device)
        self.all.append(b)
        return b

    def free(self, t):
        if isinstance(t, _Borrowed):
            return
        buf = t.buf if isinstance(t, T) else t
        assert all(buf is not f for f in self.free_list)
        self.free_list.append(buf)

    def total_bytes(self):
        return sum(b.numel() * 4 for b in self.all)


def out_size(n, k, s, p):
    return (n + 2 * p - k) // s + 1


_SIDE_STREAMS = {}


def _side_stream(device):
    n = int(os.environ.get('YOLACT_AMD_SIDE_STREAMS', '2'))
    if n <= 0:
        return torch.cuda.Stream(device=device)
    pool = _side_pool(device, n)
    st = pool['streams'][pool['next'] % n]
    pool['next'] += 1
    return st


def _side_pool(device, n):
    key = (device.type, device.index if device.index is not None else torch.cuda.current_device())
    pool = _SIDE_STREAMS.get(key)
    if pool is None:
        pool = _SIDE_STREAMS[key] = {'streams': [torch.cuda.Stream(device=device) for _ in range(n)], 'next': 0}
    return pool


def side_stream_pool(device):
    n = int(os.environ.get('YOLACT_AMD_SIDE_STREAMS', '2'))
    return tuple(_side_pool(device, n)['streams']) if n > 0 else ()


class _OpList(list):
    version = 0

    def _bump(self):
        self.version += 1

    def __setitem__(self, k, v):
        self._bump(); list.__setitem__(self, k, v)

    def __delitem__(self, k):
        self._bump(); list.__delitem__(self, k)

    def append(self, v):
        self._bump(); list.append(self, v)

    def insert(self, k, v):
        self._bump(); list.insert(self, k, v)

    def pop(self, *a):
        self._bump(); return list.pop(self, *a)

    def extend(self, it):
        self._bump(); list.extend(self, it)


def _split_k_ids(tid, blocks, nk, Cout):
    out = []
    if blocks < 400 and Cout % 4 == 0:
        for S in (2, 3, 4, 5, 6, 8, 9, 12, 16):
            per = -(-nk // S)
            if per >= 4 and per * (S - 1) < nk and 128 <= blocks * S <= 1100:
                out.append(tid + 256 * S)
    return out


class Plan:
    def __init__(self, net, B, H, W, device, dry_two_streams=False):
        self.net, self.B, self.H, self.W, self.device = net, B, H, W, device
        self.ops = _OpList()
        self.conv_meta = []
        self.arena = Arena(device)
        self.keepalive = []
        self.lib = L.lib()
        self.two_streams = (device.type == 'cuda' and os.environ.get('YOLACT_AMD_STREAMS', '2') != '1') or dry_two_streams
        self.stream_b = _side_stream(device) if self.two_streams and device.type == 'cuda' else None
        self.overlap = True
        self.events = {}
        self._cur = 'A'
        wsel = os.environ.get('YOLACT_AMD_WINOGRAD', '1')
        self.use_winograd = device.type == 'cuda' and wsel != '0'
        self.wino_variants = (2,) if wsel == '2' else (4,) if wsel == '4' else (2, 4)
        self.wino_force = os.environ.get('YOLACT_AMD_WINOGRAD_FORCE', '0') == '1'
        smode = os.environ.get('YOLACT_AMD_SPLIT', SPLIT_DEFAULT)
        self.split = smode == '1'
        self.h2 = smode == '2'
        self.mode_key = '|x3' if self.split else '|h2' if self.h2 else ''
        self.amax = torch.zeros(512 * AMAX_SLOT_FLOATS, dtype=torch.float32, device=device)
        self._nslots = 0
        self.splitk = os.environ.get('YOLACT_AMD_SPLITK', '1') == '1'
        self.pipe = os.environ.get('YOLACT_AMD_PIPE', '1') == '1'
        self.wide_guard = os.environ.get('YOLACT_AMD_WIDE_GUARD', '1') == '1'
        self.om_pad = os.environ.get('YOLACT_AMD_OM_PAD', '1') == '1'
        self.om_interleave = os.environ.get('YOLACT_AMD_OM_INTERLEAVE', '1') == '1'
        self.native_exec = device.type == 'cuda' and os.environ.get('YOLACT_AMD_NATIVE_EXEC', '1') == '1'
        self._native, self._native_events, self._stem_desc = None, None, None
        self.wide_ops = set()
        self.wide_layers = []
        self._sk_ws = {}
        self.down_on_side_stream = os.environ.get('YOLACT_AMD_DOWN_STREAM', 'B') == 'B'
        self.wino_alt, self._wino_packed, self._wino_ws = {}, {}, {}
        self._upsrc, self.wino_up = {}, {}
        self._done_event = None
        self._priors_timed = False
        self.param_stamp = None
        self.tune_misses = 0
        self._build()
        if self.wide_layers:
            import warnings
            warnings.warn('yolact_amd: %d layer(s) consume compensated OUTLIER channels (tiny filter columns on channels their producer '
                          'amplifies, Packed.tiny_columns) and run on bf16x3 / exact-fp32 tiles instead of fp16x2, without Winograd and '
                          'the fp16x2-only fusions: %s.  YOLACT_AMD_WIDE_GUARD=0 keeps fp16x2 (at reduced accuracy for such checkpoints).'
                          % (len(self.wide_layers), ', '.join(self.wide_layers[:12]) + (' ...' if len(self.wide_layers) > 12 else '')),
                          RuntimeWarning, stacklevel=2)
        self._bind_wino_workspaces()
        self.sections = [None if op[0] in ('record', 'wait', 'detect', 'nop') else self.section_of(op[2]) for op in self.ops]

    def _arena(self):
        if self._cur == 'B':
            if not hasattr(self, 'arena_b'):
                self.arena_b = Arena(self.device)
            return self.arena_b
        return self.arena

    def _new(self, B, H, W, C, slot=None, gain=None) -> T:
        return T(self._arena().alloc(B * H * W * C), B, H, W, C, slot, gain)

    def _slot(self):
        self._nslots += 1
        assert self._nslots * AMAX_SLOT_FLOATS <= self.amax.numel()
        return self._nslots - 1

    def _slot_ptr(self, slot):
        return self.amax.data_ptr() + 4 * AMAX_SLOT_FLOATS * slot

    def bound(self, slot):
        return float(self.amax[slot * AMAX_SLOT_FLOATS:(slot + 1) * AMAX_SLOT_FLOATS].max())

    def free(self, t):
        self._arena().free(t)

    def conv(self, name, x: T, pk: Packed, act=L.ACT_NONE, res: Optional[T] = None, res_mode=L.RES_NONE,
             res_after_act=0, out: Optional[T] = None, segs=None, dcn_offmask: Optional[T] = None) -> Optional[T]:
        assert x.C == pk.Cin, (name, x.C, pk.Cin)
        Ho, Wo = out_size(x.H, pk.kh, pk.stride, pk.pad), out_size(x.W, pk.kw, pk.stride, pk.pad)
        d = L.ConvDesc()
        d.x, d.w = x.ptr, pk.w.data_ptr()
        d.scale = pk.scale.data_ptr() if pk.scale is not None else None
        d.bias = pk.bias.data_ptr() if pk.bias is not None else None
        d.B, d.H, d.W, d.Cin, d.ldx = x.B, x.H, x.W, pk.Cin, x.C
        d.Ho, d.Wo, d.Cout = Ho, Wo, pk.Cout
        d.kh, d.kw, d.stride, d.pad, d.Kpad = pk.kh, pk.kw, pk.stride, pk.pad, pk.Kpad
        d.res_mode = res_mode
        d.res_after_act = res_after_act
        if res is not None:
            d.res, d.res_ld, d.res_H, d.res_W = res.ptr, res.C, res.H, res.W
            if res_mode == L.RES_ADD:
                assert (res.B, res.H, res.W, res.C) == (x.B, Ho, Wo, pk.Cout), name
        d.tile = L.TILE_AUTO
        d.cin_alg = pk.cin_alg
        d.cout_alg = pk.cout_alg
        wide = self.h2 and self.wide_guard and pk.Cin % 32 == 0 and pk.tiny_columns(in_gain=x.gain)
        pk.wide = wide
        if wide:
            self.wide_layers.append(name)
        og = pk.out_gain()
        if res is not None and res.gain is not None and res.gain.numel() == og.numel():
            og = torch.maximum(og, res.gain)
        self.last_out_gain = og
        if (self.split or wide) and dcn_offmask is None:
            d.w_x3 = pk.w3().data_ptr()
        yslot = self._slot()
        for _ in range(len(segs) - 1 if segs else 0):
            self._slot()
        if self.h2:
            d.y_amax = self._slot_ptr(yslot)
        if x.slot is not None:
            d.x_amax = self._slot_ptr(x.slot)
        if self.h2:
            assert x.slot is not None, name
            planes, sc2, winv = pk.h2()
            d.w_h2, d.scale_h2, d.winv_h2 = planes.data_ptr(), sc2.data_ptr(), winv.data_ptr()
        self.last_yslot = yslot
        y = None
        if segs is None:
            y = out if out is not None else self._new(x.B, Ho, Wo, pk.Cout)
            y.slot = yslot
            y.gain = og
            d.nseg = 1
            d.seg[0] = L.ConvSeg(0, pk.Cout, act, pk.Cout, Ho * Wo * pk.Cout, y.ptr)
        else:
            d.nseg = len(segs)
            for i, s in enumerate(segs):
                d.seg[i] = L.ConvSeg(*s)
        self.keepalive.append(pk)
        if not hasattr(self, '_desc_info'):
            self._desc_info = {}
        self._desc_info[C.addressof(d)] = (pk, res.slot if res is not None else None)
        wino = None
        if (self.use_winograd and dcn_offmask is None and out is None and pk.weight_oihw is not None and not wide
                and wino_eligible(pk, res, segs, act, x.C)):
            wino = [w for w in (self._wino_op(x, pk, act, y, name, segs, m) for m in self.wino_variants) if w is not None]
            wino = wino or None
        if dcn_offmask is not None:
            dd = L.DcnDesc()
            dd.conv = d
            dd.offmask, dd.ldo = dcn_offmask.ptr, dcn_offmask.C
            dd.om_layout = 1 if (self.om_pad and self.om_interleave) else 0
            self.ops.append((self.lib.ymi_dcn_v2_forward_f32, C.pointer(dd), name, self._cur))
            self.conv_meta.append((name, dd.conv))
            if wide:
                self.wide_ops.add(len(self.ops) - 1)
        else:
            self.ops.append((self.lib.ymi_conv2d_nhwc_f32, C.pointer(d), name, self._cur))
            self.conv_meta.append((name, d))
            if wide:
                self.wide_ops.add(len(self.ops) - 1)
            if wino is not None:
                self.wino_alt[len(self.ops) - 1] = wino
                if id(x) in self._upsrc:
                    self.wino_up[len(self.ops) - 1] = self._upsrc[id(x)]
        return y

    def _wino_op(self, x: T, pk: Packed, act, y: Optional[T], name, segs=None, m=2):
        key = (id(pk), m)
        wp = self._wino_packed.get(key)
        if wp is None:
            wp = self._wino_packed[key] = WinoPacked(pk.weight_oihw, self.device, m)
        th, tw = (x.H + m - 1) // m, (x.W + m - 1) // m
        Tn = x.B * th * tw
        Ng = _ceil(pk.Cout, 4)
        if Tn * max(pk.Cin, Ng) >= (1 << 29):
            return None
        g = (m + 2) * (m + 2)
        need_v, need_m = g * Tn * pk.Cin, g * Tn * Ng
        ws = self._wino_ws.setdefault(self._cur, [None, None])
        if ws[0] is None or ws[0].numel() < need_v:
            ws[0] = torch.empty(need_v, dtype=torch.float32, device=self.device)
        if ws[1] is None or ws[1].numel() < need_m:
            ws[1] = torch.empty(need_m, dtype=torch.float32, device=self.device)
        d = L.WinoDesc()
        d.x, d.u = x.ptr, wp.u.data_ptr()
        if self.split:
            d.u_x3 = wp.u3().data_ptr()
        if self.h2:
            planes, uinv = wp.h2()
            d.u_h2, d.uinv_h2 = planes.data_ptr(), uinv.data_ptr()
        if x.slot is not None:
            d.x_amax = self._slot_ptr(x.slot)
        if self.h2:
            d.y_amax = self._slot_ptr(self.last_yslot)
        if segs is None:
            d.y = y.ptr
        else:
            d.nseg = len(segs)
            for i, s in enumerate(segs):
                d.seg[i] = L.ConvSeg(*s)
        d.scale = pk.scale.data_ptr() if pk.scale is not None else None
        d.bias = pk.bias.data_ptr() if pk.bias is not None else None
        d.B, d.H, d.W, d.C, d.Cout, d.act, d.tile, d.m = x.B, x.H, x.W, pk.Cin, pk.Cout, act, L.TILE_AUTO, m
        d.cout_alg = pk.cout_alg
        return d

    def _bind_wino_workspaces(self):
        for idx, alts in self.wino_alt.items():
            ws = self._wino_ws[self.ops[idx][3]]
            for d in alts:
                d.V, d.M = ws[0].data_ptr(), ws[1].data_ptr()

    def call(self, fn, *args, name=''):
        self.ops.append((fn, args, name, self._cur))

    def _stage_done(self, li, t):
        sel = self.net.backbone_selected
        if not self._early_lat_on or li not in sel or sel.index(li) >= len(sel) - 1:
            return
        self._pending_lat.append((li, t))

    def _flush_early_laterals(self):
        sel = self.net.backbone_selected
        n = len(sel)
        for li, t in self._pending_lat:
            j = sel.index(li)
            i = n - 1 - j
            self.record('latgo%d' % i)
            self.on('B')
            self.wait('latgo%d' % i)
            raw = self.conv('fpn.lat%d' % i, t, self._pack(self.net.fpn.lat_layers[i]))
            self.record('lat%d' % i)
            self.on('A')
            self.early_lat[j] = raw
        self._pending_lat = []

    def on(self, which):
        self._cur = which if self.two_streams else 'A'

    def record(self, ev):
        if self.two_streams:
            self.events[ev] = torch.cuda.Event() if self.device.type == 'cuda' else None
            self.ops.append(('record', ev, ev, self._cur))

    def wait(self, ev):
        if self.two_streams:
            self.ops.append(('wait', ev, ev, self._cur))

    def _pack(self, conv, bn=None, cin_pad=None) -> Packed:
        key = (id(conv), id(bn), cin_pad)
        pk = self._pk_cache.get(key)
        if pk is None:
            pk = self._pk_cache[key] = pack_module(conv, bn, self.device, cin_pad)
        return pk

    def _rebalance_outliers(self, bb):
        self.rebalanced = []
        if not (self.h2 and os.environ.get('YOLACT_AMD_REBALANCE', '1') == '1' and isinstance(bb, M.ResNetBackbone)):
            return

        def exps(gain, cols, thr=6):
            g = gain.double().clamp_min(0)
            pos = g[g > 0]
            if pos.numel() < 8:
                return None
            kg = torch.floor(torch.log2((g / pos.median()).clamp_min(2.0 ** -126)))
            c = cols.double()
            cpos = c[c > 0]
            if cpos.numel() < 8:
                return None
            kc = torch.floor(torch.log2((cpos.median() / c.clamp_min(2.0 ** -126))))
            k = torch.minimum(kg, kc).clamp(min=0, max=40)
            k = torch.where((kg >= thr) & (kc >= thr) & (c > 0), k, torch.zeros_like(k))
            return k if bool((k > 0).any()) else None
        layers = list(bb.layers)
        sel = list(self.net.backbone_selected)
        fpn = self.net.fpn
        for li, layer in enumerate(layers):
            blocks = list(layer)
            if not blocks or blocks[0].downsample is None:
                continue
            prod = [self._pack(b.conv3, b.bn3) for b in blocks] + [self._pack(blocks[0].downsample[0], blocks[0].downsample[1])]
            cons = [self._pack(b.conv1, b.bn1) for b in blocks[1:]]
            if li + 1 < len(layers):
                nb = list(layers[li + 1])[0]
                cons.append(self._pack(nb.conv1, nb.bn1))
                if nb.downsample is not None:
                    cons.append(self._pack(nb.downsample[0], nb.downsample[1]))
            if li in sel:
                cons.append(self._pack(fpn.lat_layers[len(sel) - 1 - sel.index(li)]))
            if not cons or any(pk.Cin != prod[0].Cout or pk.Kpad != pk.kh * pk.kw * pk.Cin for pk in cons):
                continue
            gain = torch.stack([pk.out_gain()[:prod[0].Cout] for pk in prod]).amax(0)
            cols = torch.stack([pk.in_column_max() for pk in cons]).amax(0)
            k = exps(gain, cols)
            if k is None:
                continue
            down, up = torch.pow(2.0, -k).float(), torch.pow(2.0, k).float()
            for pk in prod:
                pk.scale_out_channels(down)
            for pk in cons:
                pk.scale_in_channels(up)
            self.rebalanced.append(('C%d' % (li + 2), int((k > 0).sum()), int(k.max())))
        pm_ = list(self.net.proto_net)
        self._proto0_down = None
        if (len(pm_) > 2 and isinstance(pm_[0], nn.Conv2d) and isinstance(pm_[1], nn.ReLU) and isinstance(pm_[2], nn.Conv2d)
                and pm_[0].bias is not None):
            p0, p2 = self._pack(pm_[0]), self._pack(pm_[2])
            if p2.Cin == p0.Cout and p2.Kpad == p2.kh * p2.kw * p2.Cin:
                k = exps(p0.out_gain(), p2.in_column_max())
                if k is not None:
                    down, up = torch.pow(2.0, -k).float(), torch.pow(2.0, k).float()
                    p0.scale_out_channels(down)
                    p2.scale_in_channels(up)
                    self._proto0_down = down
                    self.rebalanced.append(('proto_net.0', int((k > 0).sum()), int(k.max())))

    def _build(self):
        net, B, H, W, dev = self.net, self.B, self.H, self.W, self.device
        cfg = net.cfg
        lib = self.lib
        ar = self.arena

        self.early_lat, self._pending_lat = {}, []
        self._early_lat_on = self.two_streams and os.environ.get('YOLACT_AMD_EARLY_LAT', '0') == '1'
        bb = net.backbone
        self._pk_cache = {}
        self._rebalance_outliers(bb)
        c1 = getattr(bb, 'conv1', None)
        self.fused_stem = (self.h2 and isinstance(bb, M.ResNetBackbone) and os.environ.get('YOLACT_AMD_FUSED_STEM', '1') == '1'
                           and c1 is not None and tuple(c1.kernel_size) == (7, 7) and tuple(c1.stride) == (2, 2)
                           and tuple(c1.padding) == (3, 3) and c1.in_channels == 3 and c1.out_channels == 64 and H >= 7 and W >= 7)
        x4 = None
        if not self.fused_stem:
            x4 = self._new(B, H, W, 4, slot=self._slot())
            self.in_args = [None, x4.ptr, B, 3, H, W]
            self.in_amax = (x4.ptr, B * H * W * 4, self._slot_ptr(x4.slot))
            self.ops.append(('input', None, 'nchw_to_nhwc4', 'A'))
        if isinstance(bb, M.ResNetBackbone):
            outs = self._resnet(bb, x4)
        else:
            outs = self._darknet(bb, x4)
        self._flush_early_laterals()
        sel = [outs[i] for i in net.backbone_selected]
        for i, t in enumerate(outs):
            if i not in net.backbone_selected and t is not None:
                ar.free(t)

        fpn = net.fpn
        n = len(sel)
        sums = [None] * n
        prev = None
        for i in range(n):
            j = n - 1 - i
            pk = self._pack(fpn.lat_layers[i])
            if j in self.early_lat and prev is not None:
                raw = self.early_lat[j]
                self.wait('lat%d' % i)
                slot = self._slot()
                self.call(lib.ymi_bilinear_add_nhwc_f32, prev.ptr, raw.ptr, raw.B, prev.H, prev.W, raw.C, raw.H, raw.W,
                          self._slot_ptr(slot) if self.h2 else None, name='fpn.add%d' % i)
                raw.slot = slot
                if raw.gain is not None and prev.gain is not None and raw.gain.numel() == prev.gain.numel():
                    raw.gain = torch.maximum(raw.gain, prev.gain)
                sums[j] = raw
            elif prev is None:
                sums[j] = self.conv('fpn.lat%d' % i, sel[j], pk)
            else:
                sums[j] = self.conv('fpn.lat%d' % i, sel[j], pk, res=prev, res_mode=L.RES_BILINEAR)
            prev = sums[j]
        for t in sel:
            ar.free(t)

        shapes = [(t.H, t.W) for t in sums]
        for _ in fpn.downsample_layers:
            shapes.append((out_size(shapes[-1][0], 3, 2, 1), out_size(shapes[-1][1], 3, 2, 1)))
        self.feat_shapes = shapes
        nlev = len(shapes)

        pm = net.prediction_layers[0]
        A = pm.num_priors
        Ccls, D = cfg.num_classes, net.mask_dim
        cells = [h * w for h, w in shapes]
        P = sum(cells) * A
        self.P, self.A, self.D, self.Ccls = P, A, D, Ccls
        Cp = _ceil(Ccls, 4) if os.environ.get('YOLACT_AMD_PAD_CONF', '1') == '1' else Ccls
        self.conf_ld = Cp
        self.loc = torch.empty(B, P, 4, device=dev)
        self.conf = torch.zeros(B, P, Cp, device=dev)
        self.coef = torch.empty(B, P, D, device=dev)
        up_pk = [pack_module(m, device=dev) for m in pm.upfeature if isinstance(m, nn.Conv2d)] \
            if hasattr(pm, 'upfeature') else []
        cw, cb = pm.conf_layer.weight, pm.conf_layer.bias
        if Cp != Ccls:
            cw = torch.nn.functional.pad(cw.view(A, Ccls, *cw.shape[1:]), (0, 0, 0, 0, 0, 0, 0, Cp - Ccls)).reshape(A * Cp, *cw.shape[1:])
            cb = torch.nn.functional.pad(cb.view(A, Ccls), (0, Cp - Ccls)).reshape(A * Cp)
        wcat = torch.cat([pm.bbox_layer.weight, pm.mask_layer.weight, cw], 0)
        bcat = torch.cat([pm.bbox_layer.bias, pm.mask_layer.bias, cb], 0)
        hp = pm.bbox_layer
        head_pk = Packed(wcat, bcat, None, hp.stride[0], hp.padding[0], None, dev)
        head_pk.cout_alg = A * (4 + D + Ccls)
        coef_act = {'tanh': L.ACT_TANH, 'sigmoid': L.ACT_SIGMOID, 'relu': L.ACT_RELU, 'none': L.ACT_NONE}[
            act_name(cfg.mask_proto_coeff_activation)]
        n_b, n_c, n_m = A * 4, A * Cp, A * D
        offs = [sum(cells[:l]) * A for l in range(nlev)]
        bbc = cfg.backbone
        pri = []
        for lvl, (fh, fw) in enumerate(shapes):
            pri += make_priors_host(fh, fw, bbc.pred_scales[lvl], bbc.pred_aspect_ratios[lvl], cfg.max_size, bbc)

        pmods = list(net.proto_net)
        up_convs = [m for m in pm.upfeature if isinstance(m, nn.Conv2d)] if hasattr(pm, 'upfeature') else []
        self._merged_p3 = None
        merge_p3 = (os.environ.get('YOLACT_AMD_MERGE_P3', '1') == '1' and len(up_convs) == 1 and len(pmods) > 2
                    and isinstance(pmods[0], nn.Conv2d) and isinstance(pmods[1], nn.ReLU)
                    and all(c.kernel_size == (3, 3) and c.padding == (1, 1) and c.stride == (1, 1) and c.bias is not None
                            for c in (up_convs[0], pmods[0]))
                    and up_convs[0].in_channels == pmods[0].in_channels and up_convs[0].out_channels % 4 == 0
                    and pmods[0].out_channels % 4 == 0)

        def head(lvl, f):
            off = offs[lvl]
            u = f
            if lvl == 0 and merge_p3:
                cu, cp = up_convs[0], pmods[0]
                u = self._new(f.B, f.H, f.W, cu.out_channels)
                t0 = self._new(f.B, f.H, f.W, cp.out_channels)
                pkm = Packed(torch.cat([cu.weight, cp.weight], 0), torch.cat([cu.bias, cp.bias], 0), None, 1, 1, None, dev)
                if getattr(self, '_proto0_down', None) is not None:
                    pkm.scale_out_channels(torch.cat([torch.ones(cu.out_channels), self._proto0_down]))
                hw = f.H * f.W
                self.conv('head0.up0+proto.0', f, pkm, segs=[
                    (0, cu.out_channels, L.ACT_RELU, cu.out_channels, hw * cu.out_channels, u.ptr),
                    (cu.out_channels, cu.out_channels + cp.out_channels, L.ACT_RELU, cp.out_channels, hw * cp.out_channels,
                     t0.ptr)])
                u.slot, t0.slot = self.last_yslot, self.last_yslot + 1
                u.gain, t0.gain = self.last_out_gain[:cu.out_channels], self.last_out_gain[cu.out_channels:]
                self._merged_p3 = t0
            else:
                for k, pk in enumerate(up_pk):
                    nu = self.conv('head%d.up%d' % (lvl, k), u, pk, act=L.ACT_RELU)
                    if u is not f:
                        self.free(u)
                    u = nu
            segs = [
                (0, n_b, L.ACT_NONE, n_b, P * 4, self.loc.data_ptr() + off * 4 * 4),
                (n_b, n_b + n_m, coef_act, n_m, P * D, self.coef.data_ptr() + off * D * 4),
                (n_b + n_m, n_b + n_m + n_c, L.ACT_NONE, n_c, P * Cp, self.conf.data_ptr() + off * Cp * 4),
            ]
            self.conv('head%d.out' % lvl, u, head_pk, segs=segs)
            if u is not f:
                self.free(u)

        def pred(j):
            i = n - 1 - j
            return self.conv('fpn.pred%d' % i, sums[j], pack_module(fpn.pred_layers[i], device=dev), act=L.ACT_RELU)

        assert net.proto_src == 0, 'prototypes are taken from P3 in every shipped config'
        self.record('fork')
        self.on('B')
        self.wait('fork')
        self.on('A')
        p3 = pred(0)
        self.free(sums[0])
        self.on('B')
        feats_b = [pred(j) for j in range(1, n)]
        for j in range(1, n):
            self.free(sums[j])
        for i, m in enumerate(fpn.downsample_layers):
            feats_b.append(self.conv('fpn.down%d' % i, feats_b[-1], pack_module(m, device=dev)))
        self.on('A')
        head(0, p3)
        self.record('head0')
        self.on('B')
        for lvl in range(1, nlev):
            head(lvl, feats_b[lvl - 1])
        self.wait('head0')
        for f in feats_b:
            self.free(f)
        self.ops.append(('detect', None, 'detect', self._cur))
        self.record('b_done')
        self.on('A')

        t = p3
        mods = list(net.proto_net)
        conv_idx = [i for i, m in enumerate(mods) if isinstance(m, nn.Conv2d)]
        self.proto_patch = None
        self.proto_patch_wino = None
        self.wino_proj = None
        prev_conv_op = None
        held = None
        for i, m in enumerate(mods):
            if i == 0 and self._merged_p3 is not None:
                self.free(t)
                t = self._merged_p3
                continue
            if isinstance(m, nn.Conv2d):
                last = i == conv_idx[-1]
                has_relu = (i + 1 < len(mods) and isinstance(mods[i + 1], nn.ReLU))
                if last:
                    a = {'relu': L.ACT_RELU, 'none': L.ACT_NONE, 'sigmoid': L.ACT_SIGMOID, 'tanh': L.ACT_TANH}[
                        act_name(cfg.mask_proto_prototype_activation)]
                    assert not has_relu
                else:
                    a = L.ACT_RELU if has_relu else L.ACT_NONE
                pk = self._pack(m)
                if last:
                    Ho, Wo = out_size(t.H, pk.kh, pk.stride, pk.pad), out_size(t.W, pk.kw, pk.stride, pk.pad)
                    self.proto_shape = (B, Ho, Wo, pk.Cout)
                    self.conv('proto.%d' % i, t, pk, segs=[(0, pk.Cout, a, pk.Cout, Ho * Wo * pk.Cout, None)])
                    self.proto_patch = self.ops[-1][1].contents
                    nt = None
                    if (self.h2 and prev_conv_op is not None and prev_conv_op in self.wino_alt and (pk.kh, pk.kw, pk.stride, pk.pad) == (1, 1, 1, 0)
                            and pk.Cin == 256 and pk.Cout <= 32 and pk.Cout % 4 == 0 and a <= L.ACT_LEAKY01 and not getattr(pk, 'wide', False)
                            and os.environ.get('YOLACT_AMD_WINO_PROJ', '1') == '1'):
                        self.wino_proj = (prev_conv_op, len(self.ops) - 1)
                else:
                    nt = self.conv('proto.%d' % i, t, pk, act=a)
                    prev_conv_op = len(self.ops) - 1
                self.free(t)
                if held is not None:
                    self.free(held)
                    held = None
                t = nt
            elif isinstance(m, M.InterpolateModule):
                prev_conv_op = None
                s = int(m.scale_factor)
                has_relu = (i + 1 < len(mods) and isinstance(mods[i + 1], nn.ReLU))
                y = self._new(t.B, t.H * s, t.W * s, t.C, slot=t.slot, gain=t.gain)
                self.call(lib.ymi_bilinear_nhwc_f32, t.ptr, y.ptr, t.B, t.H, t.W, t.C, y.H, y.W,
                          C.c_float(1.0 / s), C.c_float(1.0 / s), 1 if has_relu else 0, name='proto.interp')
                if s == 2 and os.environ.get('YOLACT_AMD_FUSED_UPSAMPLE', '1') == '1':
                    self._upsrc[id(y)] = (len(self.ops) - 1, t.ptr, 1 if has_relu else 0)
                    held = t
                else:
                    self.free(t)
                t = y
        assert self.proto_patch is not None and held is None
        self.wait('b_done')
        self.priors = torch.tensor(pri, dtype=torch.float32).view(-1, 4).to(dev)
        assert self.priors.shape[0] == P

    def _resnet(self, bb: M.ResNetBackbone, x4: T):
        dev, ar, lib = self.device, self.arena, self.lib
        pk0 = pack_module(bb.conv1, bb.bn1, dev, cin_pad=4)
        if self.fused_stem:
            B, H, W = self.B, self.H, self.W
            Hs, Ws = out_size(H, 7, 2, 3), out_size(W, 7, 2, 3)
            Hp, Wp = out_size(Hs, 3, 2, 1), out_size(Ws, 3, 2, 1)
            x = self._new(B, Hp, Wp, 64, slot=self._slot(), gain=pk0.out_gain())
            planes, sc2, winv = pk0.h2()
            sd = L.StemDesc()
            sd.y, sd.B, sd.H, sd.W, sd.cout_pad, sd.kpad = x.ptr, B, H, W, pk0.CoutPad, pk0.Kpad
            sd.w_h2, sd.scale_h2, sd.bias, sd.y_amax = planes.data_ptr(), sc2.data_ptr(), pk0.bias.data_ptr(), self._slot_ptr(x.slot)
            self.keepalive.append(pk0)
            md = L.ConvDesc()
            md.B, md.H, md.W, md.Cin, md.ldx, md.Ho, md.Wo, md.Cout = B, H, W, 4, 4, Hs, Ws, 64
            md.kh, md.kw, md.stride, md.pad, md.Kpad, md.cin_alg, md.cout_alg = 7, 7, 2, 3, pk0.Kpad, 3, 64
            self.conv_meta.append(('stem', md))
            self.ops.append(('stem', sd, 'stem+maxpool', 'A'))
            self._stem_desc = sd
        else:
            stem = self.conv('stem', x4, pk0, act=L.ACT_RELU)
            ar.free(x4)
            Hp, Wp = out_size(stem.H, 3, 2, 1), out_size(stem.W, 3, 2, 1)
            x = self._new(stem.B, Hp, Wp, stem.C, slot=stem.slot, gain=stem.gain)
            self.call(lib.ymi_maxpool3x3s2_nhwc_f32, stem.ptr, x.ptr, stem.B, stem.H, stem.W, stem.C, Hp, Wp, name='maxpool')
            ar.free(stem)
        outs = []
        for li, layer in enumerate(bb.layers):
            for bi, blk in enumerate(layer):
                nm = 'layer%d.%d' % (li, bi)
                side_down = blk.downsample is not None and self.two_streams and self.down_on_side_stream
                if side_down:
                    self.record(nm + '.in')
                    self.on('B')
                    self.wait(nm + '.in')
                    res = self.conv(nm + '.down', x, self._pack(blk.downsample[0], blk.downsample[1]))
                    self.record(nm + '.down')
                    self.on('A')
                o1 = self.conv(nm + '.conv1', x, self._pack(blk.conv1, blk.bn1), act=L.ACT_RELU)
                if blk.use_dcn:
                    dcn = blk.conv2
                    om = self.conv(nm + '.offmask', o1, pack_offmask(dcn.conv_offset_mask, dev, self.om_interleave) if self.om_pad
                                   else pack_module(dcn.conv_offset_mask, None, dev))
                    pk = Packed(dcn.weight, dcn.bias, blk.bn2, dcn.stride[0], 1, None, dev)
                    o2 = self.conv(nm + '.dcn', o1, pk, act=L.ACT_RELU, dcn_offmask=om)
                    ar.free(om)
                else:
                    o2 = self.conv(nm + '.conv2', o1, pack_module(blk.conv2, blk.bn2, dev), act=L.ACT_RELU)
                ar.free(o1)
                if side_down:
                    self.wait(nm + '.down')
                elif blk.downsample is not None:
                    res = self.conv(nm + '.down', x, self._pack(blk.downsample[0], blk.downsample[1]))
                else:
                    res = x
                y = self.conv(nm + '.conv3', o2, self._pack(blk.conv3, blk.bn3), act=L.ACT_RELU, res=res,
                              res_mode=L.RES_ADD)
                ar.free(o2)
                if side_down:
                    self.on('B')
                    self.free(res)
                    self.on('A')
                elif res is not x:
                    ar.free(res)
                ar.free(x)
                x = y
                if bi == 0:
                    self._flush_early_laterals()
            outs.append(x)
            self._stage_done(li, x)
            x = _Borrowed(x)
        return outs

    def _darknet(self, bb: M.DarkNetBackbone, x4: T):
        dev, ar = self.device, self.arena

        def unit(name, t, seq, cin_pad=None, res=None):
            pk = pack_module(seq[0], seq[1], dev, cin_pad=cin_pad)
            if res is None:
                return self.conv(name, t, pk, act=L.ACT_LEAKY01)
            return self.conv(name, t, pk, act=L.ACT_LEAKY01, res=res, res_mode=L.RES_ADD, res_after_act=1)

        x = unit('preconv', x4, bb._preconv, cin_pad=4)
        ar.free(x4)
        outs = []
        for li, layer in enumerate(bb.layers):
            mods = list(layer)
            y = unit('dark%d.down' % li, x, mods[0])
            ar.free(x)
            x = y
            for bi, blk in enumerate(mods[1:]):
                a = unit('dark%d.%d.conv1' % (li, bi), x, blk.conv1)
                y = unit('dark%d.%d.conv2' % (li, bi), a, blk.conv2, res=x)
                ar.free(a)
                ar.free(x)
                x = y
                if bi == 0:
                    self._flush_early_laterals()
            outs.append(x)
            self._stage_done(li, x)
            x = _Borrowed(x)
        return outs

    @staticmethod
    def section_of(name):
        if name.startswith('fpn.'):
            return 'fpn'
        if name.startswith('proto.'):
            return 'proto'
        if name.startswith('head'):
            return 'pred_heads'
        return 'backbone'

    def mark_done(self):
        if self.device.type == 'cuda' and not torch.cuda.is_current_stream_capturing():
            if self._done_event is None:
                self._done_event = torch.cuda.Event()
            self._done_event.record(torch.cuda.current_stream(self.device))

    def run(self, x: torch.Tensor, detect=None, timer=None, skip_proto=False):
        lib = self.lib
        cur = torch.cuda.current_stream(self.device)
        capturing = torch.cuda.is_current_stream_capturing()
        if self._done_event is not None and not capturing:
            cur.wait_event(self._done_event)
        sa = C.c_void_p(cur.cuda_stream)
        two = self.two_streams and self.overlap
        sb = C.c_void_p(self.stream_b.cuda_stream) if two else sa
        proto = None
        if not skip_proto:
            proto = torch.empty(self.proto_shape, dtype=torch.float32, device=self.device)
            self.proto_patch.seg[0].ptr = proto.data_ptr()
            if self.proto_patch_wino is not None:
                self.proto_patch_wino.proj_y = proto.data_ptr()
        if timer is not None and not all(hasattr(timer, a) for a in ('start', 'stop', 'env')):
            timer = None
        if timer is None and self.native_exec:
            nat = self._native_plan()
            if nat is not None:
                det = self._run_native(nat, x, sa, sb, two, detect, skip_proto)
                self.mark_done()
                return proto, det
        if self.h2:
            self.amax[:self._nslots * AMAX_SLOT_FLOATS].zero_()
        self._sec = None
        try:
            det = self._dispatch(x, cur, sa, sb, two, detect, timer, skip_proto)
        finally:
            if timer is not None and self._sec is not None:
                timer.stop(self._sec)
        self.mark_done()
        return proto, det

    _SEC_ID = {'backbone': L.SEC_BACKBONE, 'fpn': L.SEC_FPN, 'proto': L.SEC_PROTO, 'pred_heads': L.SEC_HEADS}

    def _native_plan(self):
        key = (self.ops.version, len(self.ops)) if isinstance(self.ops, _OpList) else tuple(map(id, self.ops))
        if self._native is not None and self._native[0] == key:
            return self._native[1]
        lib = self.lib
        n = len(self.ops)
        arr = (L.PlanOp * (n + 1))()
        arr[0].kind, arr[0].stream = L.OP_MEMSET, 0
        arr[0].p[0], arr[0].i[0] = self.amax.data_ptr(), 4 * self._nslots * AMAX_SLOT_FLOATS
        ev_index, det_idx, in_idx, ok = {}, None, None, True
        by_fn = {id(lib.ymi_conv2d_nhwc_f32): L.OP_CONV, id(lib.ymi_conv3x3_winograd_f32): L.OP_WINO,
                 id(lib.ymi_dcn_v2_forward_f32): L.OP_DCN, id(lib.ymi_pointwise_chain_f32): L.OP_CHAIN}
        for k, (fn, args, name, where) in enumerate(self.ops):
            o = arr[k + 1]
            o.stream = 1 if where == 'B' else 0
            o.section = self._SEC_ID.get(self.sections[k], 0) if self.sections[k] else 0
            if fn == 'input':
                a = self.in_args
                o.kind, in_idx = L.OP_INPUT, k + 1
                o.p[1] = a[1]
                o.p[2] = self.in_amax[2] if self.h2 else None
                o.i[0], o.i[1], o.i[2], o.i[3] = a[2], a[3], a[4], a[5]
            elif fn == 'stem':
                o.kind, o.desc = L.OP_STEM, C.addressof(args)
            elif fn == 'nop':
                o.kind = L.OP_NOP
            elif fn in ('record', 'wait'):
                o.kind = L.OP_RECORD if fn == 'record' else L.OP_WAIT
                o.i[0] = ev_index.setdefault(args, len(ev_index))
            elif fn == 'detect':
                o.kind, det_idx = L.OP_NOP, k + 1
            elif id(fn) in by_fn:
                o.kind, o.desc = by_fn[id(fn)], C.addressof(args.contents)
            elif fn is lib.ymi_bilinear_nhwc_f32:
                o.kind = L.OP_BILINEAR
                o.p[0], o.p[1] = args[0], args[1]
                for q in range(6):
                    o.i[q] = args[2 + q]
                o.f[0], o.f[1], o.i[6] = args[8].value, args[9].value, args[10]
            elif fn is lib.ymi_maxpool3x3s2_nhwc_f32:
                o.kind = L.OP_MAXPOOL
                o.p[0], o.p[1] = args[0], args[1]
                for q in range(6):
                    o.i[q] = args[2 + q]
            elif fn is lib.ymi_bilinear_add_nhwc_f32:
                o.kind = L.OP_BILINEAR_ADD
                o.p[0], o.p[1], o.p[2] = args[0], args[1], args[8]
                for q in range(6):
                    o.i[q] = args[2 + q]
            else:
                ok = False
                break
        if not ok or det_idx is None:
            self._native = (key, None)
            return None
        if self._native_events is None or len(self._native_events) < len(ev_index):
            for h in (self._native_events or ()):
                if h:
                    lib.ymi_event_destroy(C.c_void_p(h))
            evs = (C.c_void_p * max(len(ev_index), 1))()
            for q in range(len(ev_index)):
                h = C.c_void_p()
                L.check(lib.ymi_event_create(C.byref(h)), 'ymi_event_create')
                evs[q] = h.value
            self._native_events = evs
        nat = (arr, det_idx, self._native_events, in_idx, n + 1)
        self._native = (key, nat)
        return nat

    def _run_native(self, nat, x, sa, sb, two, detect, skip_proto):
        arr, det_idx, evs, in_idx, n = nat
        lib = self.lib
        if in_idx is not None:
            arr[in_idx].p[0] = x.data_ptr()
        if self._stem_desc is not None:
            self._stem_desc.x = x.data_ptr()
        skip = (1 << L.SEC_PROTO) if skip_proto else 0
        failed = C.c_int32(-1)
        ov = 1 if two else 0

        def go(first, last):
            rc = lib.ymi_plan_run(arr, first, last, sa, sb, evs, ov, skip, C.byref(failed))
            if rc != 0:
                L.check(rc, self.ops[failed.value - 1][2] if failed.value > 0 else 'plan op')
        go(0 if self.h2 else 1, det_idx)
        det = None
        if detect is not None:
            det = detect(sb if self.ops[det_idx - 1][3] == 'B' else sa)
        go(det_idx + 1, n)
        return det

    def __del__(self):
        try:
            if getattr(self, '_native_events', None) is not None:
                for h in self._native_events:
                    if h:
                        self.lib.ymi_event_destroy(h)
        except Exception:
            pass

    def _dispatch(self, x, cur, sa, sb, two, detect, timer, skip_proto=False):
        lib = self.lib
        det = None
        for (fn, args, name, where), nsec in zip(self.ops, self.sections):
            s = sb if where == 'B' else sa
            if timer is not None and nsec is not None and nsec != self._sec:
                if self._sec is not None:
                    timer.stop(self._sec)
                timer.start(nsec)
                self._sec = nsec
                if nsec == 'pred_heads' and not self._priors_timed:
                    with timer.env('makepriors'):
                        self._priors_timed = True
            if fn == 'input':
                a = self.in_args
                if self.h2:
                    rc = lib.ymi_nchw_to_nhwc4_amax_f32(x.data_ptr(), a[1], a[2], a[3], a[4], a[5], self.in_amax[2], s)
                else:
                    rc = lib.ymi_nchw_to_nhwc4_f32(x.data_ptr(), a[1], a[2], a[3], a[4], a[5], s)
            elif fn == 'nop' or (skip_proto and nsec == 'proto'):
                continue
            elif fn == 'stem':
                args.x = x.data_ptr()
                rc = lib.ymi_stem_pool_f32(C.byref(args), s)
            elif fn == 'record':
                if two:
                    self.events[args].record(self.stream_b if where == 'B' else cur)
                continue
            elif fn == 'wait':
                if two:
                    (self.stream_b if where == 'B' else cur).wait_event(self.events[args])
                continue
            elif fn == 'detect':
                if detect is not None:
                    det = detect(s)
                continue
            elif isinstance(args, tuple):
                rc = fn(*args, s)
            else:
                rc = fn(args, s)
            if rc != 0:
                L.check(rc, name)
        return det

    def tune(self, x: torch.Tensor, reps: int = 3):
        mode = os.environ.get('YOLACT_AMD_AUTOTUNE', '1')
        self.tune_table, self.wino_table, self.tune_misses = [], [], 0
        if mode == '0':
            return []
        cache_path = os.environ.get('YOLACT_AMD_TUNE_CACHE')
        disk = {}
        if mode != 'force':
            disk.update(load_tune_table(self.device))
            if cache_path and os.path.exists(cache_path):
                disk.update(_read_table_file(cache_path))
        n0 = len(disk)
        self.run(x)
        s = L.stream_ptr()
        e0, e1 = torch.cuda.Event(enable_timing=True), torch.cuda.Event(enable_timing=True)
        measure = mode != 'table'
        self._tune_direct(e0, e1, s, reps, disk, measure)
        self._tune_winograd(e0, e1, s, reps, disk, measure)
        self._fuse_pointwise_chains(e0, e1, s, reps, disk, measure)
        torch.cuda.synchronize(self.device)
        if cache_path and (len(disk) != n0 or mode == 'force'):
            _write_table_file(cache_path, disk, self.device)
        self.tune_entries = disk
        return self.tune_table

    autotune = tune

    def _splitk_ws(self, where, numel):
        ws = self._sk_ws.get(where)
        if ws is None or ws.numel() < numel:
            ws = self._sk_ws[where] = torch.empty(numel, dtype=torch.float32, device=self.device)
            for fn, dptr, _n, w in self.ops:
                if fn is self.lib.ymi_conv2d_nhwc_f32 and w == where and dptr.contents.split_k > 1:
                    dptr.contents.split_ws = ws.data_ptr()
                elif fn is self.lib.ymi_dcn_v2_forward_f32 and w == where and dptr.contents.conv.split_k > 1:
                    dptr.contents.conv.split_ws = ws.data_ptr()
        return ws

    @staticmethod
    def _splitk_ok(d):
        return (d.kh == 1 and d.kw == 1 and d.pad == 0 and d.Cin == d.Kpad and d.Cin % 32 == 0 and d.nseg == 1
                and d.Cout % 4 == 0 and d.seg[0].act <= L.ACT_LEAKY01 and d.res_mode in (L.RES_NONE, L.RES_ADD)
                and d.B * d.Ho * d.Wo <= 16384 and d.Kpad >= 256)

    def _fuse_pointwise_chains(self, e0, e1, s, reps, disk, measure):
        self.chain_table = []
        if not self.h2 or os.environ.get('YOLACT_AMD_CHAIN', '1') != '1':
            return
        lib = self.lib

        def timed(run):
            run()
            best = 1e30
            for _ in range(2):
                e0.record()
                for _ in range(reps):
                    run()
                e1.record()
                e1.synchronize()
                best = min(best, e0.elapsed_time(e1) / reps)
            return best
        i = 0
        while i < len(self.ops):
            f3, p3, n3, w3 = self.ops[i]
            i += 1
            if f3 is not lib.ymi_conv2d_nhwc_f32 or (i - 1) in self.wide_ops:
                continue
            d3 = p3.contents
            M = d3.B * d3.Ho * d3.Wo
            P_ = d3.Cin
            if not ((d3.kh, d3.kw, d3.stride, d3.pad, d3.nseg) == (1, 1, 1, 0, 1) and P_ in (64, 128, 256) and d3.Cout == 4 * P_
                    and d3.res_mode == L.RES_ADD and not d3.res_after_act and d3.seg[0].n0 == 0 and d3.seg[0].act <= L.ACT_LEAKY01
                    and d3.w_h2 and d3.x_amax and M * max(d3.seg[0].row_stride, d3.res_ld) < (1 << 29)):
                continue
            if P_ > 64 and os.environ.get('YOLACT_AMD_CHAIN2', '0') not in ('1', 'force'):
                continue
            pair = False
            if i < len(self.ops) and self.ops[i][0] is lib.ymi_conv2d_nhwc_f32 and self.ops[i][3] == w3 and i not in self.wide_ops:
                d1 = self.ops[i][1].contents
                pair = ((d1.kh, d1.kw, d1.stride, d1.pad, d1.Cin, d1.Cout, d1.nseg) == (1, 1, 1, 0, 4 * P_, P_, 1)
                        and d1.res_mode == L.RES_NONE and d1.x == d3.seg[0].ptr and d1.ldx == d3.seg[0].row_stride
                        and d1.seg[0].n0 == 0 and d1.seg[0].act <= L.ACT_LEAKY01 and bool(d1.w_h2))
            if P_ > 64 and not pair:
                continue
            cd = L.ChainDesc()
            cd.x, cd.res, cd.y = d3.x, d3.res, d3.seg[0].ptr
            cd.w_a_h2, cd.scale_a_h2, cd.bias_a = d3.w_h2, d3.scale_h2, d3.bias
            cd.x_amax, cd.y_amax = d3.x_amax, d3.y_amax
            cd.M, cd.ldx, cd.res_ld, cd.ldy = M, d3.ldx, d3.res_ld, d3.seg[0].row_stride
            cd.k_a, cd.n_a, cd.n_b, cd.cout_pad_a, cd.cout_pad_b = P_, 4 * P_, P_, _ceil(4 * P_, 128), _ceil(P_, 128)
            cd.act_a = d3.seg[0].act
            if P_ > 64:
                info = getattr(self, '_desc_info', {}).get(C.addressof(d3))
                if info is None or info[1] is None:
                    continue
                cd.gain_a, cd.bias_max_a = info[0].l1_gain()
                cd.res_amax = self._slot_ptr(info[1])
            name = n3
            if pair:
                f1, p1, n1, w1 = self.ops[i]
                cd.z, cd.ldz, cd.z_amax, cd.act_b = d1.seg[0].ptr, d1.seg[0].row_stride, d1.y_amax, d1.seg[0].act
                cd.w_b_h2, cd.scale_b_h2, cd.bias_b = d1.w_h2, d1.scale_h2, d1.bias
                name = n3 + '+' + n1
            if pair:
                def span(ptr, ld):
                    return (int(ptr), int(ptr) + 4 * M * int(ld))

                def overlap(a, b):
                    return a[0] < b[1] and b[0] < a[1]
                zs, xs = span(cd.z, cd.ldz), span(cd.x, cd.ldx)
                in_place = int(cd.z) == int(cd.x) and cd.ldz == cd.ldx
                if overlap(zs, span(cd.y, cd.ldy)) or overlap(zs, span(cd.res, cd.res_ld)) or (overlap(zs, xs) and not in_place):
                    continue
            cptr = C.pointer(cd)
            key = ('chain' if pair else 'chain1') + str((d3.B, d3.Ho, d3.Wo) + ((P_,) if P_ > 64 else ())) + self.mode_key
            ent = disk.get(key)
            if P_ > 64 and os.environ.get('YOLACT_AMD_CHAIN2') == 'force':
                ent = [1, 0.0, 0.0]
            if ent is None:
                self.tune_misses += 1
                if not measure or lib.ymi_pointwise_chain_f32(cptr, s) != 0:
                    continue
                t_plan = timed((lambda: (f3(p3, s), f1(p1, s))) if pair else (lambda: f3(p3, s)))
                t_one = timed(lambda: lib.ymi_pointwise_chain_f32(cptr, s))
                ent = disk[key] = [1 if t_one < 0.97 * t_plan else 0, round(t_plan, 4), round(t_one, 4)]
            self.chain_table.append((name, ent[0], ent[1], ent[2]))
            if ent[0] and lib.ymi_pointwise_chain_f32(cptr, s) == 0:
                self.keepalive.append(cd)
                self.ops[i - 1] = (lib.ymi_pointwise_chain_f32, cptr, name, w3)
                if pair:
                    self.ops[i] = ('nop', None, n1 + '[fused into ' + n3 + ']', w1)
                    i += 1

    def _apply_choice(self, fn, dptr, where, val, s):
        d = dptr.contents.conv if fn is self.lib.ymi_dcn_v2_forward_f32 else dptr.contents
        tile, S = int(val) & 255, int(val) >> 8
        d.tile = tile
        if S > 1:
            is_dcn = fn is self.lib.ymi_dcn_v2_forward_f32
            if tile & L.TILE_DCNP:
                nk_ = d.Kpad // 32
                if -(-nk_ // S) * (S - 1) >= nk_:
                    return -1
            elif is_dcn or not self._splitk_ok(d) or (d.Kpad // 32) % S:
                return -1
            d.split_k = S
            d.split_ws = self._splitk_ws(where, S * d.B * d.Ho * d.Wo * d.Cout).data_ptr()
        else:
            d.split_k = 0
        return fn(dptr, s)

    @staticmethod
    def _pipe_ok(d):
        return ((d.kh, d.kw, d.pad) in ((3, 3, 1), (1, 1, 0)) and d.Cin % 32 == 0 and d.Kpad == d.kh * d.kw * d.Cin and d.Kpad >= 64
                and d.nseg == 1 and d.Cout % 4 == 0 and d.seg[0].n0 == 0 and d.seg[0].act <= L.ACT_LEAKY01
                and d.seg[0].row_stride % 4 == 0 and d.seg[0].batch_stride == d.Ho * d.Wo * d.seg[0].row_stride
                and d.res_mode in (L.RES_NONE, L.RES_ADD))

    @staticmethod
    def dcnp_candidates(d, dcn=False):
        M, nk = d.B * d.Ho * d.Wo, d.Kpad // 32
        out = []
        for t, name in sorted(L.DCNP_TILES.items()):
            bm, bn = (int(v) for v in name[4:].split('w')[0].split('x'))
            if (bn > 128 and d.Cout < 256) or (dcn and t in L.DCNP_PLAIN_ONLY) or (bn == 32) != (d.Cout <= 32):
                continue
            tid = t | L.TILE_H2 | L.TILE_DCNP
            out.append(tid)
            out += _split_k_ids(tid, -(-M // bm) * -(-d.Cout // bn), nk, d.Cout)
        return out

    @staticmethod
    def patch2_candidates(d):
        if os.environ.get('YOLACT_AMD_PATCH2', '1') != '1':
            return []
        if not ((d.kh, d.kw, d.stride, d.pad) == (3, 3, 1, 1) and d.Cin % 32 == 0 and d.Kpad == 9 * d.Cin and d.Cout >= 64 and d.Cout % 4 == 0
                and d.res_mode == L.RES_NONE and 1 <= d.nseg <= 3 and d.w_h2):
            return []
        cov = 0
        for i in range(d.nseg):
            g = d.seg[i]
            if (g.n0 != cov or g.n0 % 128 or g.act > L.ACT_LEAKY01 or g.act < 0 or g.row_stride % 4 or g.row_stride < g.n1 - g.n0
                    or g.batch_stride != d.Ho * d.Wo * g.row_stride):
                return []
            cov = g.n1
        if cov < d.Cout:
            return []
        return [t | L.TILE_H2 | L.TILE_DCNP for t in sorted(L.PATCH2_TILES)]

    @staticmethod
    def pc_candidates(d):
        if os.environ.get('YOLACT_AMD_PC', '0') != '1' or d.Cout <= 32:
            return []
        M, nk = d.B * d.Ho * d.Wo, d.Kpad // 32
        out = []
        for t, name in sorted(L.PC_TILES.items()):
            bm, bn = (int(v) for v in os.environ.get('YOLACT_AMD_PC_SHAPE', name[2:]).split('x'))
            if bn > 128 and d.Cout < 256:
                continue
            tid = t | L.TILE_H2 | L.TILE_DCNP
            out.append(tid)
            out += _split_k_ids(tid, -(-M // bm) * -(-d.Cout // bn), nk, d.Cout)
        return out

    @staticmethod
    def ws_candidates(d):
        if d.res_mode != L.RES_NONE or d.Cout > 64:
            return []
        M, nk = d.B * d.Ho * d.Wo, d.Kpad // 32
        out = []
        for t, name in sorted(L.WS_TILES.items()):
            bm, bn = (int(v) for v in name[2:].split('w')[0].split('x'))
            if (bn == 32) != (d.Cout <= 32):
                continue
            cap = (64 * 1024) // (bn * 128)
            blocks, n = -(-M // bm), 0
            for S in (1, 2, 3, 4, 5, 6, 8, 9, 12, 16):
                per = -(-nk // S)
                if per > cap or (S > 1 and per * (S - 1) >= nk):
                    continue
                if n and blocks * S > 1200:
                    break
                out.append((t | L.TILE_H2 | L.TILE_DCNP) + 256 * (S if S > 1 else 0))
                n += 1
                if n == 3:
                    break
        return out

    def direct_candidates(self, fn, d, wide=False):
        is_dcn = fn is self.lib.ymi_dcn_v2_forward_f32
        h2_, split_ = self.h2 and not wide, self.split or (wide and not is_dcn)
        if is_dcn:
            cands = [t for t in L.BASIC_TILES if t != L.TILE_128x32]
        elif d.Cin % 32 != 0:
            cands = [L.TILE_128x64, L.TILE_64x64] if d.Cout <= 64 else list(L.BASIC_TILES)
        elif d.Cout <= 32:
            cands = [L.TILE_128x32, L.TILE_64x64, L.TILE_64x64_S3, L.TILE_32x32_K4, L.TILE_32x32_K4_S4,
                     L.TILE_64x32_K2, L.TILE_64x32_K2_S3]
        elif d.Cout <= 64:
            cands = [L.TILE_128x64, L.TILE_128x64_S3, L.TILE_64x64, L.TILE_64x64_S3, L.TILE_64x64_S4,
                     L.TILE_32x32_K4, L.TILE_32x32_K4_S4, L.TILE_64x32_K2, L.TILE_64x32_K2_S3,
                     L.TILE_32x64_K2, L.TILE_32x64_K2_S3]
        else:
            cands = [t for t in sorted(L.TILE_NAMES) if t != L.TILE_128x32 and not (t & (L.TILE_X3 | L.TILE_H2))]
            if d.Cout < 256:
                cands = [t for t in cands if t != L.TILE_128x256_W8]
        spflag = (L.TILE_X3 if split_ else L.TILE_H2 if h2_ else 0) if not (is_dcn and split_) else 0
        if spflag:
            base_ok = L.H2_BASE_TILES if spflag == L.TILE_H2 else L.X3_BASE_TILES
            cands = cands + [t | spflag for t in cands if t in base_ok
                             and (d.Cin % 32 == 0 or t in L.BASIC_TILES)]
        if is_dcn and h2_:
            cands = cands + self.dcnp_candidates(d, dcn=True)
        if not is_dcn and h2_ and self.pipe and self._pipe_ok(d):
            cands = cands + self.dcnp_candidates(d) + self.ws_candidates(d)
            cands = cands + self.pc_candidates(d)
        if not is_dcn and h2_ and self.pipe:
            cands = cands + self.patch2_candidates(d)
            if ((d.kh, d.kw, d.stride, d.pad, d.Cin, d.Cout) == (3, 3, 1, 1, 64, 64) and d.res_mode == L.RES_NONE
                    and patch_tile_allowed()):
                cands = cands + [L.DCNP_PATCH_C64 | L.TILE_H2 | L.TILE_DCNP]
        if not is_dcn and self._splitk_ok(d) and self.splitk:
            x3 = spflag
            for S in (2, 4):
                if (d.Kpad // 32) % S == 0 and d.Kpad // S >= 128:
                    cands += [(t | x3) + 256 * S for t in (L.TILE_128x128, L.TILE_64x128, L.TILE_128x64, L.TILE_64x64,
                                                          L.TILE_256x128_W8)]

        return cands

    def _tune_direct(self, e0, e1, s, reps, disk, measure):
        cache = {}
        for opi, (fn, dptr, name, where) in enumerate(self.ops):
            is_dcn = fn is self.lib.ymi_dcn_v2_forward_f32
            if fn is not self.lib.ymi_conv2d_nhwc_f32 and not is_dcn:
                continue
            d = dptr.contents.conv if is_dcn else dptr.contents
            key = (d.B, d.H, d.W, d.Cin, d.Cout, d.kh, d.kw, d.stride, d.pad, d.res_mode, d.nseg, d.Kpad) + (('dcn',) if is_dcn else ())
            wide = opi in self.wide_ops
            h2_, split_ = self.h2 and not wide, self.split or (wide and not is_dcn)
            skey = str(key) + ('|x3' if split_ else '|h2' if h2_ else '')
            key = key + (('wide',) if wide else ())
            if key not in cache and skey in disk:
                v_ = int(disk[skey])
                patch_off = ((v_ & 255) == (L.DCNP_PATCH_C64 | L.TILE_H2 | L.TILE_DCNP) and not patch_tile_allowed())
                if not patch_off and self._apply_choice(fn, dptr, where, disk[skey], s) == 0:
                    cache[key] = v_
            if key not in cache:
                self.tune_misses += 1
                if not measure:
                    cache[key] = L.TILE_AUTO
                    d.tile, d.split_k = L.TILE_AUTO, 0
                    continue
                cands = self.direct_candidates(fn, d, wide)
                def cname(v):
                    return L.TILE_NAMES[v & 255] + ('/k%d' % (v >> 8) if v >> 8 else '')
                best, best_ms, times = None, 1e30, {}
                ok_cands = []
                for t in cands:
                    if self._apply_choice(fn, dptr, where, t, s) == 0:
                        ok_cands.append(t)
                yslot = self.amax[(d.y_amax - self.amax.data_ptr()) // 4:][:AMAX_SLOT_FLOATS] if d.y_amax else None
                for rnd in range(2):
                    for t in ok_cands:
                        self._apply_choice(fn, dptr, where, t, s)
                        e0.record()
                        for _ in range(reps):
                            if yslot is not None:
                                yslot.zero_()
                            fn(dptr, s)
                        e1.record()
                        e1.synchronize()
                        ms = e0.elapsed_time(e1) / reps
                        times[cname(t)] = round(min(ms, times.get(cname(t), 1e30)), 4)
                for t in ok_cands:
                    if times[cname(t)] < best_ms:
                        best, best_ms = t, times[cname(t)]
                assert best is not None, name
                cache[key] = best
                disk[skey] = best
                self.tune_table.append((name, cname(best), times))
            self._apply_choice(fn, dptr, where, cache[key], s)

    def _tune_winograd(self, e0, e1, s, reps, disk, measure):
        lib = self.lib
        self.wino_toggle = {}
        wtiles = [L.TILE_64x64, L.TILE_64x128, L.TILE_128x64, L.TILE_128x128_W8, L.TILE_64x128_S3, L.TILE_32x64_K2,
                  L.TILE_128x128, L.TILE_128x128_S3, L.TILE_128x128_W8_S3, L.TILE_256x128_W8, L.TILE_256x128_W8_S3]
        if self.split:
            wtiles = wtiles + [t | L.TILE_X3 for t in wtiles]
        if self.h2:
            hb = wtiles + [L.TILE_128x256_W8]
            wtiles = wtiles + [t | L.TILE_H2 for t in hb] + [t | L.TILE_H2 | L.WINO_PLANES for t in hb]
            if os.environ.get('YOLACT_AMD_WGEMM', '1') == '1':
                wtiles = wtiles + [L.TILE_WG_128x256 | L.TILE_H2 | L.WINO_PLANES]
        memo = {}
        for idx, alts in sorted(self.wino_alt.items()):
            fn, dptr, name, where = self.ops[idx]
            if fn is not lib.ymi_conv2d_nhwc_f32:
                continue
            w0 = alts[0]
            key = 'wino' + str((w0.B, w0.H, w0.W, w0.C, w0.Cout, w0.act, w0.nseg, tuple(a.m for a in alts))) + (
                self.mode_key)
            if key not in memo and key in disk:
                ent = tuple(disk[key])
                ok = True
                if ent[1]:
                    wd = [a for a in alts if a.m == ent[0]]
                    if wd:
                        wd[0].tile, wd[0].v_planes = int(ent[1]) & 255, 1 if int(ent[1]) & L.WINO_PLANES else 0
                        ok = lib.ymi_conv3x3_winograd_f32(C.byref(wd[0]), s) == 0
                    else:
                        ok = False
                if ok:
                    memo[key] = ent
            if key not in memo:
                self.tune_misses += 1
                if not measure:
                    memo[key] = (0, 0, 0.0, 0.0, 0.0, 0.0)
                else:
                    def timed(f, arg):
                        f(arg, s)
                        best = 1e30
                        for _ in range(2):
                            e0.record()
                            for _ in range(reps):
                                f(arg, s)
                            e1.record()
                            e1.synchronize()
                            best = min(best, e0.elapsed_time(e1) / reps)
                        return best
                    t_direct = timed(fn, dptr)
                    best_m, best_t, best_ms, per_m = 0, 0, 1e30, {}
                    for wd in alts:
                        for t in wtiles:
                            wd.tile, wd.v_planes = t & 255, 1 if t & L.WINO_PLANES else 0
                            if lib.ymi_conv3x3_winograd_f32(C.byref(wd), s) != 0:
                                continue
                            ms = timed(lib.ymi_conv3x3_winograd_f32, C.pointer(wd))
                            per_m[wd.m] = min(ms, per_m.get(wd.m, 1e30))
                            if ms < best_ms:
                                best_m, best_t, best_ms = wd.m, t, ms
                    memo[key] = (best_m, best_t, round(t_direct, 4), round(best_ms, 4),
                                 round(per_m.get(2, 0.0), 4), round(per_m.get(4, 0.0), 4))
                    disk[key] = list(memo[key])
            best_m, best_t, t_direct, t_wino, t_f2, t_f4 = memo[key]
            self.wino_table.append((name, 'F%d/%s%s' % (best_m, L.TILE_NAMES.get(int(best_t) & 255, '-'),
                                                         'p' if int(best_t) & L.WINO_PLANES else ''), t_direct, t_wino, t_f2, t_f4))
            instep_direct = disk.get('instep|' + key) == 0 and not self.wino_force
            if best_t and not (self.wino_up.get(idx) is not None or (self.wino_proj is not None and self.wino_proj[0] == idx)):
                wd_ = [a for a in alts if a.m == best_m][0]
                wd_.tile, wd_.v_planes = int(best_t) & 255, 1 if int(best_t) & L.WINO_PLANES else 0
                self.wino_toggle.setdefault(key, []).append(
                    (idx, (fn, dptr, name, where), (lib.ymi_conv3x3_winograd_f32, C.pointer(wd_), name + '[wino]', where),
                     bool(t_wino < 0.97 * t_direct)))
            if best_t and (self.wino_force or (t_wino < 0.97 * t_direct and not instep_direct)):
                wd = [a for a in alts if a.m == best_m][0]
                wd.tile, wd.v_planes = int(best_t) & 255, 1 if int(best_t) & L.WINO_PLANES else 0
                self.ops[idx] = (lib.ymi_conv3x3_winograd_f32, C.pointer(wd), name + '[wino]', where)
                up = self.wino_up.get(idx)
                if up is not None and best_m == 4 and wd.H % 2 == 0 and wd.W % 2 == 0:
                    bidx, lo_ptr, relu = up
                    wd.x_up, wd.up_relu = lo_ptr, relu
                    bfn, bargs, bname, bwhere = self.ops[bidx]
                    self.ops[bidx] = ('nop', None, bname + '[fused into ' + name + ']', bwhere)
                if self.wino_proj is not None and self.wino_proj[0] == idx and best_m == 4 and wd.Cout == 256 and wd.nseg == 0:
                    pidx = self.wino_proj[1]
                    pfn, pdptr, pname, pwhere = self.ops[pidx]
                    if pfn is lib.ymi_conv2d_nhwc_f32 and pwhere == where:
                        pd = pdptr.contents
                        wd.proj_w_h2, wd.proj_scale_h2, wd.proj_bias = pd.w_h2, pd.scale_h2, pd.bias
                        wd.proj_y, wd.proj_y_amax = pd.seg[0].ptr, pd.y_amax
                        wd.proj_cout, wd.proj_ldy, wd.proj_act = pd.Cout, pd.seg[0].row_stride, pd.seg[0].act
                        scratch = torch.empty(self.proto_shape, dtype=torch.float32, device=self.device)
                        wd.proj_y = scratch.data_ptr()
                        rc = lib.ymi_conv3x3_winograd_f32(C.byref(wd), s)
                        torch.cuda.synchronize(self.device)
                        wd.proj_y = None
                        if rc != 0:
                            wd.proj_w_h2 = None
                            self.wino_proj_rejected = rc
                        else:
                            self.ops[pidx] = ('nop', None, pname + '[fused into ' + name + ']', pwhere)
                            self.proto_patch_wino = wd

    def set_winograd(self, key, on: bool):
        for idx, direct_op, wino_op, _ in self.wino_toggle.get(key, []):
            self.ops[idx] = wino_op if on else direct_op

    def conv_flops(self):
        return sum(self.lib.ymi_conv_flops(C.byref(d)) for _, d in self.conv_meta)


class _Borrowed(T):
    __slots__ = ()

    def __init__(self, t: T):
        super().__init__(t.buf, t.B, t.H, t.W, t.C, t.slot, t.gain)
```

Before: 2327.

## Batch shared-weight head convs across pyramid levels into one Winograd GEMM

Adds a multi-level Winograd 3x3 conv op that concatenates the tiles of several FPN levels into a single input transform, one GEMM and one output transform. The prediction head's upfeature conv and its output conv share weights across levels, so they now run once over all levels instead of per level. This cuts kernel launches and gives the small-level GEMMs a larger M dimension. The cost is per-tile level lookup overhead and a single shared amax scale across levels. A tuning pass is added for the merged op.

```diff
diff --git a/include/yolact_amd.h b/include/yolact_amd.h
--- a/include/yolact_amd.h
+++ b/include/yolact_amd.h
@@ -114,6 +114,35 @@
 } ymi_wino_desc;
 int ymi_conv3x3_winograd_f32(const ymi_wino_desc *d, void *stream);
 
+#define YMI_WINO_MAX_LEVELS 4
+typedef struct {
+  const float *x;
+  float *y;
+  const float *x_amax;
+  int32_t H, W;
+  int64_t row0;
+  int64_t seg_off[3];
+} ymi_wino_level;
+typedef struct {
+  ymi_wino_level lv[YMI_WINO_MAX_LEVELS];
+  int32_t nlev;
+  int32_t B, C, Cout;
+  int32_t act;
+  int32_t tile;
+  int32_t nseg;
+  int32_t cout_alg;
+  ymi_conv_seg seg[3];
+  const float *scale;
+  const float *bias;
+  const float *u;
+  const void *u_h2;
+  const float *uinv_h2;
+  float *V, *M;
+  float *x_amax_group;
+  float *y_amax;
+} ymi_wino_levels_desc;
+int ymi_conv3x3_winograd_levels_f32(const ymi_wino_levels_desc *d, void *stream);
+
 #define YMI_AMAX_SUB 16
 #define YMI_AMAX_STRIDE 64
 int ymi_amax_f32(const float *x, long n, float *out, void *stream);
@@ -330,7 +359,8 @@
 int ymi_pointwise_chain_f32(const ymi_chain_desc *d, void *stream);
 
 enum { YMI_OP_NOP = 0, YMI_OP_CONV = 1, YMI_OP_WINO = 2, YMI_OP_DCN = 3, YMI_OP_CHAIN = 4, YMI_OP_STEM = 5, YMI_OP_INPUT = 6,
-       YMI_OP_BILINEAR = 7, YMI_OP_MAXPOOL = 8, YMI_OP_BILINEAR_ADD = 9, YMI_OP_RECORD = 10, YMI_OP_WAIT = 11, YMI_OP_MEMSET = 12 };
+       YMI_OP_BILINEAR = 7, YMI_OP_MAXPOOL = 8, YMI_OP_BILINEAR_ADD = 9, YMI_OP_RECORD = 10, YMI_OP_WAIT = 11, YMI_OP_MEMSET = 12,
+       YMI_OP_WINO_LEVELS = 13 };
 enum { YMI_SEC_NONE = 0, YMI_SEC_BACKBONE = 1, YMI_SEC_FPN = 2, YMI_SEC_PROTO = 3, YMI_SEC_HEADS = 4 };
 typedef struct ymi_plan_op {
   int32_t kind;
diff --git a/yolact_amd/_lib.py b/yolact_amd/_lib.py
--- a/yolact_amd/_lib.py
+++ b/yolact_amd/_lib.py
@@ -88,6 +88,21 @@
                 ('proj_cout', C.c_int32), ('proj_ldy', C.c_int32), ('proj_act', C.c_int32), ('_pad5', C.c_int32)]
 
 
+WINO_MAX_LEVELS = 4
+
+
+class WinoLevel(C.Structure):
+    _fields_ = [('x', C.c_void_p), ('y', C.c_void_p), ('x_amax', C.c_void_p), ('H', C.c_int32), ('W', C.c_int32),
+                ('row0', C.c_int64), ('seg_off', C.c_int64 * 3)]
+
+
+class WinoLevelsDesc(C.Structure):
+    _fields_ = [('lv', WinoLevel * WINO_MAX_LEVELS), ('nlev', C.c_int32), ('B', C.c_int32), ('C', C.c_int32), ('Cout', C.c_int32),
+                ('act', C.c_int32), ('tile', C.c_int32), ('nseg', C.c_int32), ('cout_alg', C.c_int32),
+                ('seg', ConvSeg * 3), ('scale', C.c_void_p), ('bias', C.c_void_p), ('u', C.c_void_p), ('u_h2', C.c_void_p), ('uinv_h2', C.c_void_p),
+                ('V', C.c_void_p), ('M', C.c_void_p), ('x_amax_group', C.c_void_p), ('y_amax', C.c_void_p)]
+
+
 class DcnDesc(C.Structure):
     _fields_ = [('conv', ConvDesc), ('offmask', C.c_void_p), ('ldo', C.c_int32), ('mask_is_prob', C.c_int32),
                 ('om_layout', C.c_int32), ('_pad1', C.c_int32)]
@@ -161,7 +176,7 @@
 
 
 (OP_NOP, OP_CONV, OP_WINO, OP_DCN, OP_CHAIN, OP_STEM, OP_INPUT, OP_BILINEAR, OP_MAXPOOL, OP_BILINEAR_ADD, OP_RECORD, OP_WAIT,
- OP_MEMSET) = range(13)
+ OP_MEMSET, OP_WINO_LEVELS) = range(14)
 SEC_NONE, SEC_BACKBONE, SEC_FPN, SEC_PROTO, SEC_HEADS = range(5)
 
 
@@ -201,6 +216,7 @@
     ('ymi_strerror', C.c_char_p, [C.c_int]),
     ('ymi_conv2d_nhwc_f32', C.c_int, [C.POINTER(ConvDesc), _P]),
     ('ymi_conv3x3_winograd_f32', C.c_int, [C.POINTER(WinoDesc), _P]),
+    ('ymi_conv3x3_winograd_levels_f32', C.c_int, [C.POINTER(WinoLevelsDesc), _P]),
     ('ymi_conv_flops', C.c_double, [C.POINTER(ConvDesc)]),
     ('ymi_conv_pick_tile', C.c_int, [C.POINTER(ConvDesc)]),
     ('ymi_amax_f32', C.c_int, [_P, C.c_long, _P, _P]),
diff --git a/yolact_amd/csrc/plan_exec.cpp b/yolact_amd/csrc/plan_exec.cpp
--- a/yolact_amd/csrc/plan_exec.cpp
+++ b/yolact_amd/csrc/plan_exec.cpp
@@ -30,6 +30,7 @@
       case YMI_OP_NOP: break;
       case YMI_OP_CONV: rc = ymi_conv2d_nhwc_f32((const ymi_conv_desc *)o.desc, s); break;
       case YMI_OP_WINO: rc = ymi_conv3x3_winograd_f32((const ymi_wino_desc *)o.desc, s); break;
+      case YMI_OP_WINO_LEVELS: rc = ymi_conv3x3_winograd_levels_f32((const ymi_wino_levels_desc *)o.desc, s); break;
       case YMI_OP_DCN: rc = ymi_dcn_v2_forward_f32((const ymi_dcn_desc *)o.desc, s); break;
       case YMI_OP_CHAIN: rc = ymi_pointwise_chain_f32((const ymi_chain_desc *)o.desc, s); break;
       case YMI_OP_STEM: rc = ymi_stem_pool_f32((const ymi_stem_desc *)o.desc, s); break;
diff --git a/yolact_amd/csrc/winograd.hip b/yolact_amd/csrc/winograd.hip
--- a/yolact_amd/csrc/winograd.hip
+++ b/yolact_amd/csrc/winograd.hip
@@ -531,6 +531,49 @@
 #endif
 }
 
+__device__ __forceinline__ void wino43_seg_store(const SegTab &st, const f32x4 (&o)[4][4], const float *__restrict__ scale,
+                                                 const float *__restrict__ bias, long b, int ty, int tx, int Ho, int Wo, int n4,
+                                                 int Cout, float (&am)[3]) {
+  const int kv = seg_vec4(st, n4 * 4, Cout);
+  if (kv >= 0) {
+    const SegVec sv = seg_vec_setup(st, kv, scale, bias, n4 * 4);
+#pragma unroll
+    for (int iy = 0; iy < 4; ++iy)
+#pragma unroll
+      for (int ix = 0; ix < 4; ++ix) {
+        const int oy = 4 * ty + iy, ox = 4 * tx + ix;
+        if (oy < Ho && ox < Wo) seg_amax_add(am, kv, seg_vec_store(sv, o[iy][ix], b, (long)oy * Wo + ox));
+      }
+    return;
+  }
+#pragma unroll
+  for (int e = 0; e < 4; ++e) {
+    const int n = n4 * 4 + e;
+    if (n >= Cout) continue;
+    float *ptr = nullptr; long bs = 0; int rs = 0, act = 0, n0 = 0, ks = 0;
+#pragma unroll
+    for (int k = 0; k < 3; ++k)
+      if (k < st.nseg && n >= st.seg[k].n0 && n < st.seg[k].n1) {
+        ptr = st.seg[k].ptr; bs = st.seg[k].batch_stride; rs = st.seg[k].row_stride; act = st.seg[k].act; n0 = st.seg[k].n0; ks = k;
+      }
+    if (!ptr) continue;
+    const float sc = scale ? scale[n] : 1.f, bi = bias ? bias[n] : 0.f;
+#pragma unroll
+    for (int iy = 0; iy < 4; ++iy) {
+      const int oy = 4 * ty + iy;
+      if (oy >= Ho) continue;
+#pragma unroll
+      for (int ix = 0; ix < 4; ++ix) {
+        const int ox = 4 * tx + ix;
+        if (ox >= Wo) continue;
+        const float val = wino_act(o[iy][ix][e] * sc + bi, act);
+        seg_amax_add(am, ks, fabsf(val));
+        ptr[b * bs + ((long)oy * Wo + ox) * rs + (n - n0)] = val;
+      }
+    }
+  }
+}
+
 __global__ __launch_bounds__(256) void wino43_out_seg_k(const float *__restrict__ Mm, const SegTab st,
                                                         const float *__restrict__ scale, const float *__restrict__ bias,
                                                         int Ho, int Wo, int N4, int Cout, int th, int tw, long T, long total, float *__restrict__ y_amax) {
@@ -542,44 +585,143 @@
     const long t = tu, b = bu;
     f32x4 o[4][4];
     wino43_out_tile(Mm + t * (N4 * 4L) + n4 * 4, T * (N4 * 4L), o);
-    const int kv = seg_vec4(st, n4 * 4, Cout);
-    if (kv >= 0) {
-      const SegVec sv = seg_vec_setup(st, kv, scale, bias, n4 * 4);
-#pragma unroll
-      for (int iy = 0; iy < 4; ++iy)
-#pragma unroll
-        for (int ix = 0; ix < 4; ++ix) {
-          const int oy = 4 * ty + iy, ox = 4 * tx + ix;
-          if (oy < Ho && ox < Wo) seg_amax_add(am, kv, seg_vec_store(sv, o[iy][ix], b, (long)oy * Wo + ox));
-        }
-      continue;
-    }
-#pragma unroll
-    for (int e = 0; e < 4; ++e) {
-      const int n = n4 * 4 + e;
-      if (n >= Cout) continue;
-      float *ptr = nullptr; long bs = 0; int rs = 0, act = 0, n0 = 0, ks = 0;
-#pragma unroll
-      for (int k = 0; k < 3; ++k)
-        if (k < st.nseg && n >= st.seg[k].n0 && n < st.seg[k].n1) {
-          ptr = st.seg[k].ptr; bs = st.seg[k].batch_stride; rs = st.seg[k].row_stride; act = st.seg[k].act; n0 = st.seg[k].n0; ks = k;
-        }
-      if (!ptr) continue;
-      const float sc = scale ? scale[n] : 1.f, bi = bias ? bias[n] : 0.f;
-#pragma unroll
-      for (int iy = 0; iy < 4; ++iy) {
-        const int oy = 4 * ty + iy;
-        if (oy >= Ho) continue;
-#pragma unroll
-        for (int ix = 0; ix < 4; ++ix) {
-          const int ox = 4 * tx + ix;
-          if (ox >= Wo) continue;
-          const float val = wino_act(o[iy][ix][e] * sc + bi, act);
-          seg_amax_add(am, ks, fabsf(val));
-          ptr[b * bs + ((long)oy * Wo + ox) * rs + (n - n0)] = val;
-        }
-      }
-    }
+    wino43_seg_store(st, o, scale, bias, b, ty, tx, Ho, Wo, n4, Cout, am);
+  }
+  seg_amax_commit(y_amax, st.nseg, apre, am);
+}
+
+struct LvTab {
+  const float *x[YMI_WINO_MAX_LEVELS];
+  float *y[YMI_WINO_MAX_LEVELS];
+  const float *x_amax[YMI_WINO_MAX_LEVELS];
+  long seg_off[YMI_WINO_MAX_LEVELS][3];
+  unsigned row0[YMI_WINO_MAX_LEVELS];
+  int H[YMI_WINO_MAX_LEVELS], W[YMI_WINO_MAX_LEVELS], th[YMI_WINO_MAX_LEVELS], tw[YMI_WINO_MAX_LEVELS];
+  int nlev;
+};
+struct LvPos { int l, H, W, ty, tx; long b; };
+
+__device__ __forceinline__ LvPos lv_locate(const LvTab &tab, unsigned tu) {
+  LvPos p;
+  p.l = 0;
+  unsigned r0 = 0;
+  int th = tab.th[0], tw = tab.tw[0];
+  p.H = tab.H[0]; p.W = tab.W[0];
+#pragma unroll
+  for (int k = 1; k < YMI_WINO_MAX_LEVELS; ++k)
+    if (k < tab.nlev && tu >= tab.row0[k]) { p.l = k; r0 = tab.row0[k]; th = tab.th[k]; tw = tab.tw[k]; p.H = tab.H[k]; p.W = tab.W[k]; }
+  const unsigned tl = tu - r0, ru = tl / (unsigned)tw, bu = ru / (unsigned)th;
+  p.tx = (int)(tl - ru * (unsigned)tw); p.ty = (int)(ru - bu * (unsigned)th); p.b = bu;
+  return p;
+}
+template <typename P>
+__device__ __forceinline__ P lv_pick(P const (&a)[YMI_WINO_MAX_LEVELS], int l) {
+  P v = a[0];
+#pragma unroll
+  for (int k = 1; k < YMI_WINO_MAX_LEVELS; ++k) v = l == k ? a[k] : v;
+  return v;
+}
+
+__global__ __launch_bounds__(256) void wino43_in_lv_k(const LvTab tab, float *__restrict__ V, int C4, long T, long total,
+                                                      float *__restrict__ group) {
+  float amax = 0.f;
+#pragma unroll
+  for (int k = 0; k < YMI_WINO_MAX_LEVELS; ++k)
+    if (k < tab.nlev) amax = fmaxf(amax, ymi_amax_read(tab.x_amax[k]));
+  if (blockIdx.x == 0 && threadIdx.x < YMI_AMAX_SUB) group[threadIdx.x * YMI_AMAX_STRIDE] = amax;
+  float vs = 1.f, vinv = 1.f;
+  ymi_h2_scale(amax * 100.f, vs, vinv);
+  for (unsigned i = blockIdx.x * 256u + threadIdx.x; i < (unsigned)total; i += gridDim.x * 256u) {
+    const unsigned tu = i / (unsigned)C4;
+    const int c4 = (int)(i - tu * (unsigned)C4);
+    const LvPos p = lv_locate(tab, tu);
+    const int H = p.H, W = p.W, y0 = 4 * p.ty - 1, x0 = 4 * p.tx - 1;
+    const float *base = lv_pick(tab.x, p.l) + ((p.b * H) * (long)W) * (C4 * 4L) + c4 * 4;
+    f32x4 u[6][6];
+#pragma unroll
+    for (int j = 0; j < 6; ++j) {
+      const int xx = x0 + j;
+      const bool xok = (unsigned)xx < (unsigned)W;
+      f32x4 dcol[6];
+#pragma unroll
+      for (int iy = 0; iy < 6; ++iy) {
+        const int yy = y0 + iy;
+        const bool ok = xok && (unsigned)yy < (unsigned)H;
+        dcol[iy] = ld4(base + ((long)(ok ? yy : 0) * W + (ok ? xx : 0)) * (C4 * 4L), ok);
+      }
+      bt6(dcol[0], dcol[1], dcol[2], dcol[3], dcol[4], dcol[5], u[0][j], u[1][j], u[2][j], u[3][j], u[4][j], u[5][j]);
+    }
+    const long stride_e = T * (C4 * 4L);
+    _Float16 *o2 = reinterpret_cast<_Float16 *>(V) + (long)tu * (C4 * 4L) + c4 * 4;
+#pragma unroll
+    for (int iy = 0; iy < 6; ++iy) {
+      f32x4 v[6];
+      bt6(u[iy][0], u[iy][1], u[iy][2], u[iy][3], u[iy][4], u[iy][5], v[0], v[1], v[2], v[3], v[4], v[5]);
+#pragma unroll
+      for (int l = 0; l < 6; ++l) store_v_planes(o2, iy * 6 + l, 2 * stride_e, stride_e, v[l], vs);
+    }
+  }
+}
+
+__global__ __launch_bounds__(256) void wino43_out_lv_k(const float *__restrict__ Mm, const LvTab tab,
+                                                       const float *__restrict__ scale, const float *__restrict__ bias, int N4,
+                                                       long T, int act, long total, float *__restrict__ y_amax) {
+  float am = 0.f;
+  const ymi_amax_pre apre = ymi_amax_prefetch(y_amax);
+  for (unsigned i = blockIdx.x * 256u + threadIdx.x; i < (unsigned)total; i += gridDim.x * 256u) {
+    const unsigned tu = i / (unsigned)N4;
+    const int n4 = (int)(i - tu * (unsigned)N4);
+    const LvPos p = lv_locate(tab, tu);
+    const int Ho = p.H, Wo = p.W, ty = p.ty, tx = p.tx;
+    float *y = lv_pick(tab.y, p.l);
+    f32x4 o[4][4];
+    wino43_out_tile(Mm + (long)tu * (N4 * 4L) + n4 * 4, T * (N4 * 4L), o);
+    f32x4 sc = {1.f, 1.f, 1.f, 1.f}, bi = {0.f, 0.f, 0.f, 0.f};
+    if (scale) sc = *reinterpret_cast<const f32x4 *>(scale + n4 * 4);
+    if (bias) bi = *reinterpret_cast<const f32x4 *>(bias + n4 * 4);
+    const float slope = ymi_act_slope(act);
+#pragma unroll
+    for (int iy = 0; iy < 4; ++iy)
+#pragma unroll
+      for (int ix = 0; ix < 4; ++ix) {
+        f32x4 v = o[iy][ix] * sc + bi;
+#pragma unroll
+        for (int e = 0; e < 4; ++e) v[e] = fmaxf(v[e], slope * v[e]);
+        o[iy][ix] = v;
+        const bool ok = 4 * ty + iy < Ho && 4 * tx + ix < Wo;
+        am = fmaxf(am, ok ? ymi_absmax4(v) : 0.f);
+      }
+#pragma unroll
+    for (int iy = 0; iy < 4; ++iy)
+#pragma unroll
+      for (int ix = 0; ix < 4; ++ix) {
+        const int oy = 4 * ty + iy, ox = 4 * tx + ix;
+        if (oy < Ho && ox < Wo) *reinterpret_cast<f32x4 *>(y + ((p.b * Ho + oy) * (long)Wo + ox) * (N4 * 4L) + n4 * 4) = o[iy][ix];
+      }
+  }
+  if (y_amax) ymi_amax_finish(apre, am);
+}
+
+__global__ __launch_bounds__(256) void wino43_out_seg_lv_k(const float *__restrict__ Mm, const SegTab st, const LvTab tab,
+                                                           const float *__restrict__ scale, const float *__restrict__ bias, int N4,
+                                                           int Cout, long T, long total, float *__restrict__ y_amax) {
+  float am[3] = {0.f, 0.f, 0.f};
+  const ymi_amax_pre apre = ymi_amax_prefetch(y_amax);
+  for (unsigned i = blockIdx.x * 256u + threadIdx.x; i < (unsigned)total; i += gridDim.x * 256u) {
+    const unsigned tu = i / (unsigned)N4;
+    const int n4 = (int)(i - tu * (unsigned)N4);
+    const LvPos p = lv_locate(tab, tu);
+    SegTab sl = st;
+#pragma unroll
+    for (int k = 0; k < 3; ++k) {
+      long off = tab.seg_off[0][k];
+#pragma unroll
+      for (int q = 1; q < YMI_WINO_MAX_LEVELS; ++q) off = p.l == q ? tab.seg_off[q][k] : off;
+      if (k < st.nseg) sl.seg[k].ptr = st.seg[k].ptr + off;
+    }
+    f32x4 o[4][4];
+    wino43_out_tile(Mm + (long)tu * (N4 * 4L) + n4 * 4, T * (N4 * 4L), o);
+    wino43_seg_store(sl, o, scale, bias, p.b, p.ty, p.tx, p.H, p.W, n4, Cout, am);
   }
   seg_amax_commit(y_amax, st.nseg, apre, am);
 }
@@ -700,3 +842,69 @@
   ymi_internal_prof_end(outer, s);
   return rc;
 }
+
+extern "C" int ymi_conv3x3_winograd_levels_f32(const ymi_wino_levels_desc *d, void *stream) {
+  if (!d || !d->u || !d->u_h2 || !d->uinv_h2 || !d->V || !d->M || !d->x_amax_group) return YMI_ENULL;
+  if (d->nlev < 1 || d->nlev > YMI_WINO_MAX_LEVELS || d->B <= 0 || d->C <= 0 || d->Cout <= 0 || d->nseg < 0 || d->nseg > 3) return YMI_EARG;
+  if (!(d->tile & YMI_TILE_H2) || (d->tile & YMI_TILE_X3)) return YMI_EARG;
+  if (d->C & 31) return YMI_ESHAPE;
+  if (d->nseg == 0 && ((d->Cout & 3) || d->act > YMI_ACT_LEAKY01 || d->act < 0)) return YMI_ESHAPE;
+  for (int k = 0; k < d->nseg; ++k) if (!d->seg[k].ptr) return YMI_ENULL;
+  LvTab tab = {};
+  tab.nlev = d->nlev;
+  long T = 0;
+  double px = 0.0;
+  for (int l = 0; l < d->nlev; ++l) {
+    const ymi_wino_level &v = d->lv[l];
+    if (!v.x || !v.x_amax || (d->nseg == 0 && !v.y)) return YMI_ENULL;
+    if (v.H <= 0 || v.W <= 0) return YMI_EARG;
+    if ((((uintptr_t)v.x) & 15) || (((uintptr_t)v.y) & 15) || v.row0 != T) return YMI_ESHAPE;
+    tab.x[l] = v.x; tab.y[l] = v.y; tab.x_amax[l] = v.x_amax;
+    tab.H[l] = v.H; tab.W[l] = v.W; tab.th[l] = (v.H + 3) / 4; tab.tw[l] = (v.W + 3) / 4;
+    tab.row0[l] = (unsigned)T;
+    for (int k = 0; k < 3; ++k) tab.seg_off[l][k] = v.seg_off[k];
+    T += (long)d->B * tab.th[l] * tab.tw[l];
+    px += (double)d->B * v.H * v.W;
+  }
+  const int Ng = (d->Cout + 3) / 4 * 4;
+  if (T * (long)(d->C > Ng ? d->C : Ng) >= (1L << 29)) return YMI_ESHAPE;
+  const int C4 = d->C / 4, N4 = Ng / 4, ng = 36;
+  hipStream_t s = (hipStream_t)stream;
+  const double alg = 2.0 * px * (double)(d->cout_alg > 0 ? d->cout_alg : d->Cout) * 9.0 * d->C;
+  const double exe = 2.0 * ng * (double)T * d->C * Ng;
+  const int outer = ymi_internal_prof_begin(alg, d->tile, 4, s);
+  hipLaunchKernelGGL(wino43_in_lv_k, dim3(grid_for(T * C4)), dim3(256), 0, s, tab, d->V, C4, T, T * C4, d->x_amax_group);
+  int rc = ymi_launch_status();
+  if (rc) return rc;
+  const long cout_pad = ((long)d->Cout + 127) / 128 * 128;
+  if ((d->tile & 31) == YMI_TILE_WG_128x256) {
+    rc = ymi_internal_wgemm(d->V, d->u_h2, d->uinv_h2, d->x_amax_group, 100.f, d->M, ng, T, d->C, Ng, (int)cout_pad, exe, 6, s);
+  } else {
+    ymi_conv_desc g = {};
+    g.x = d->V; g.w = d->u;
+    g.B = 1; g.H = (int)T; g.W = 1; g.Cin = d->C; g.ldx = d->C;
+    g.Ho = (int)T; g.Wo = 1; g.Cout = Ng;
+    g.kh = g.kw = 1; g.stride = 1; g.pad = 0; g.Kpad = d->C;
+    g.nseg = 1; g.tile = d->tile;
+    g.w_h2 = d->u_h2; g.scale_h2 = d->uinv_h2; g.winv_h2 = d->uinv_h2;
+    g.x_amax = d->x_amax_group; g.x_amax_mul = 100.f;
+    g.seg[0].n0 = 0; g.seg[0].n1 = Ng; g.seg[0].act = YMI_ACT_NONE; g.seg[0].row_stride = Ng;
+    g.seg[0].batch_stride = T * Ng; g.seg[0].ptr = d->M;
+    rc = ymi_internal_grouped_gemm(&g, ng, T * d->C, cout_pad * d->C, T * Ng, exe, 6, s, d->V, (unsigned)(T * d->C * 2),
+                                   2L * T * d->C * 2, (unsigned)cout_pad);
+  }
+  if (rc) return rc;
+  if (d->nseg > 0) {
+    SegTab st;
+    st.nseg = d->nseg;
+    for (int k = 0; k < 3; ++k) st.seg[k] = d->seg[k];
+    hipLaunchKernelGGL(wino43_out_seg_lv_k, dim3(grid_for(T * N4)), dim3(256), 0, s, d->M, st, tab, d->scale, d->bias, N4, d->Cout,
+                       T, T * N4, d->y_amax);
+  } else {
+    hipLaunchKernelGGL(wino43_out_lv_k, dim3(grid_for(T * N4)), dim3(256), 0, s, d->M, tab, d->scale, d->bias, N4, T, d->act,
+                       T * N4, d->y_amax);
+  }
+  rc = ymi_launch_status();
+  ymi_internal_prof_end(outer, s);
+  return rc;
+}
diff --git a/yolact_amd/engine.py b/yolact_amd/engine.py
--- a/yolact_amd/engine.py
+++ b/yolact_amd/engine.py
@@ -270,6 +270,20 @@
     if segs is not None:
         return len(segs) <= 3
     return pk.Cout % 4 == 0 and act in (L.ACT_NONE, L.ACT_RELU, L.ACT_LEAKY01)
+
+
+def wino_level_table(B, shapes, m=4):
+    rows, r = [], 0
+    for H, W in shapes:
+        th, tw = (H + m - 1) // m, (W + m - 1) // m
+        rows.append((H, W, th, tw, r))
+        r += B * th * tw
+    return rows, r
+
+
+def head_level_offsets(shapes, A):
+    cells = [h * w for h, w in shapes]
+    return [sum(cells[:l]) * A for l in range(len(shapes))], sum(cells) * A
 
 
 def pack_offmask(conv: nn.Conv2d, device, interleave: bool) -> Packed:
@@ -434,6 +448,7 @@
         self._sk_ws = {}
         self.down_on_side_stream = os.environ.get('YOLACT_AMD_DOWN_STREAM', 'B') == 'B'
         self.wino_alt, self._wino_packed, self._wino_ws = {}, {}, {}
+        self.level_ops = []
         self._upsrc, self.wino_up = {}, {}
         self._done_event = None
         self._priors_timed = False
@@ -601,6 +616,96 @@
             ws = self._wino_ws[self.ops[idx][3]]
             for d in alts:
                 d.V, d.M = ws[0].data_ptr(), ws[1].data_ptr()
+        for _, d, where in self.level_ops:
+            ws = self._wino_ws[where]
+            d.V, d.M = ws[0].data_ptr(), ws[1].data_ptr()
+
+    def _merge_heads_ok(self, pm, up_pk, head_pk, feats):
+        if os.environ.get('YOLACT_AMD_MERGE_HEADS', '1') == '0' or os.environ.get('YOLACT_AMD_AUTOTUNE', '1') == '0':
+            return False
+        if self.wino_force:
+            return False
+        if not (self.use_winograd and self.h2 and 4 in self.wino_variants and getattr(self.net.cfg, 'share_prediction_module', False)):
+            return False
+        if len(up_pk) != 1 or not 2 <= len(feats) <= L.WINO_MAX_LEVELS:
+            return False
+        up = up_pk[0]
+        if any(pk.weight_oihw is None for pk in (up, head_pk)):
+            return False
+        if not (wino_eligible(up, None, None, L.ACT_RELU, feats[0].C) and wino_eligible(head_pk, None, [0] * 3, None, up.Cout)):
+            return False
+        if self.wide_guard and (any(up.tiny_columns(in_gain=f.gain) for f in feats) or head_pk.tiny_columns(in_gain=up.out_gain())):
+            return False
+        return all(f.slot is not None and f.C == feats[0].C and f.B == feats[0].B for f in feats)
+
+    def _levels_desc(self, name, pk, B, Cin, xs, act=L.ACT_NONE, ys=None, segs=None, seg_offs=None):
+        key = (id(pk), 4)
+        wp = self._wino_packed.get(key)
+        if wp is None:
+            wp = self._wino_packed[key] = WinoPacked(pk.weight_oihw, self.device, 4)
+        rows, Tn = wino_level_table(B, [(h, w) for _, h, w, _ in xs])
+        Ng = _ceil(pk.Cout, 4)
+        assert Tn * max(Cin, Ng) < (1 << 29), name
+        ws = self._wino_ws.setdefault(self._cur, [None, None])
+        for k, need in enumerate((36 * Tn * Cin, 36 * Tn * Ng)):
+            if ws[k] is None or ws[k].numel() < need:
+                ws[k] = torch.empty(need, dtype=torch.float32, device=self.device)
+        d = L.WinoLevelsDesc()
+        d.nlev, d.B, d.C, d.Cout, d.act, d.cout_alg = len(xs), B, Cin, pk.Cout, act, pk.cout_alg
+        d.tile = L.TILE_128x128 | L.TILE_H2
+        planes, uinv = wp.h2()
+        d.u, d.u_h2, d.uinv_h2 = wp.u.data_ptr(), planes.data_ptr(), uinv.data_ptr()
+        d.scale = pk.scale.data_ptr() if pk.scale is not None else None
+        d.bias = pk.bias.data_ptr() if pk.bias is not None else None
+        d.x_amax_group = self._slot_ptr(self._slot())
+        yslot = self._slot()
+        for _ in range(len(segs) - 1 if segs else 0):
+            self._slot()
+        d.y_amax = self._slot_ptr(yslot)
+        for l, ((ptr, H, W, slot), row) in enumerate(zip(xs, rows)):
+            lv = d.lv[l]
+            lv.x, lv.H, lv.W, lv.row0, lv.x_amax = ptr, H, W, row[4], self._slot_ptr(slot)
+            if segs is None:
+                lv.y = ys[l]
+            else:
+                for k in range(len(segs)):
+                    lv.seg_off[k] = seg_offs[l][k]
+        if segs is not None:
+            d.nseg = len(segs)
+            for i, sg in enumerate(segs):
+                d.seg[i] = L.ConvSeg(*sg)
+        self.keepalive.append(pk)
+        self.ops.append((self.lib.ymi_conv3x3_winograd_levels_f32, C.pointer(d), name + '[winolv]', self._cur))
+        self.level_ops.append((len(self.ops) - 1, d, self._cur))
+        md = L.ConvDesc()
+        md.B, md.H, md.W, md.Cin, md.ldx, md.Ho, md.Wo, md.Cout = B, xs[0][1], xs[0][2], Cin, Cin, xs[0][1], xs[0][2], pk.Cout
+        md.kh, md.kw, md.stride, md.pad, md.Kpad, md.nseg, md.cout_alg = 3, 3, 1, 1, pk.Kpad, max(d.nseg, 1), pk.cout_alg
+        self.conv_meta.append((name, md))
+        return yslot
+
+    def _merged_heads(self, feats, up, head_pk, offs, widths, coef_act, P, D, Cp):
+        B, Cin = feats[0].B, feats[0].C
+        n = len(feats)
+        sizes = [f.B * f.H * f.W * up.Cout for f in feats]
+        ubuf = self._arena().alloc(sum(sizes))
+        starts = [sum(sizes[:l]) for l in range(n)]
+        uptr = [ubuf.data_ptr() + 4 * st for st in starts]
+        uslot = self._levels_desc('head1-%d.up0' % n, up, B, Cin, [(f.ptr, f.H, f.W, f.slot) for f in feats], act=L.ACT_RELU, ys=uptr)
+        n_b, n_m, n_c = widths
+
+        def segs(off):
+            return [(0, n_b, L.ACT_NONE, n_b, P * 4, self.loc.data_ptr() + off * 4 * 4),
+                    (n_b, n_b + n_m, coef_act, n_m, P * D, self.coef.data_ptr() + off * D * 4),
+                    (n_b + n_m, n_b + n_m + n_c, L.ACT_NONE, n_c, P * Cp, self.conf.data_ptr() + off * Cp * 4)]
+        first = 1 if n >= 3 else 0
+        for l in range(first):
+            f = feats[l]
+            u = T(ubuf[starts[l]:starts[l] + sizes[l]], f.B, f.H, f.W, up.Cout, uslot, up.out_gain())
+            self.conv('head%d.out' % (l + 1), u, head_pk, segs=segs(offs[l + 1]))
+        self._levels_desc('head%d-%d.out' % (first + 1, n), head_pk, B, up.Cout,
+                          [(uptr[l], feats[l].H, feats[l].W, uslot) for l in range(first, n)], segs=segs(0),
+                          seg_offs=[(offs[l + 1] * 4, offs[l + 1] * D, offs[l + 1] * Cp) for l in range(first, n)])
+        self._arena().free(ubuf)
 
     def call(self, fn, *args, name=''):
         self.ops.append((fn, args, name, self._cur))
@@ -794,7 +899,7 @@
         coef_act = {'tanh': L.ACT_TANH, 'sigmoid': L.ACT_SIGMOID, 'relu': L.ACT_RELU, 'none': L.ACT_NONE}[
             act_name(cfg.mask_proto_coeff_activation)]
         n_b, n_c, n_m = A * 4, A * Cp, A * D
-        offs = [sum(cells[:l]) * A for l in range(nlev)]
+        offs, _ = head_level_offsets(shapes, A)
         bbc = cfg.backbone
         pri = []
         for lvl, (fh, fw) in enumerate(shapes):
@@ -864,8 +969,11 @@
         head(0, p3)
         self.record('head0')
         self.on('B')
-        for lvl in range(1, nlev):
-            head(lvl, feats_b[lvl - 1])
+        if self._merge_heads_ok(pm, up_pk, head_pk, feats_b):
+            self._merged_heads(feats_b, up_pk[0], head_pk, offs, (n_b, n_m, n_c), coef_act, P, D, Cp)
+        else:
+            for lvl in range(1, nlev):
+                head(lvl, feats_b[lvl - 1])
         self.wait('head0')
         for f in feats_b:
             self.free(f)
@@ -1098,7 +1206,8 @@
         arr[0].p[0], arr[0].i[0] = self.amax.data_ptr(), 4 * self._nslots * AMAX_SLOT_FLOATS
         ev_index, det_idx, in_idx, ok = {}, None, None, True
         by_fn = {id(lib.ymi_conv2d_nhwc_f32): L.OP_CONV, id(lib.ymi_conv3x3_winograd_f32): L.OP_WINO,
-                 id(lib.ymi_dcn_v2_forward_f32): L.OP_DCN, id(lib.ymi_pointwise_chain_f32): L.OP_CHAIN}
+                 id(lib.ymi_dcn_v2_forward_f32): L.OP_DCN, id(lib.ymi_pointwise_chain_f32): L.OP_CHAIN,
+                 id(lib.ymi_conv3x3_winograd_levels_f32): L.OP_WINO_LEVELS}
         for k, (fn, args, name, where) in enumerate(self.ops):
             o = arr[k + 1]
             o.stream = 1 if where == 'B' else 0
@@ -1249,6 +1358,7 @@
         measure = mode != 'table'
         self._tune_direct(e0, e1, s, reps, disk, measure)
         self._tune_winograd(e0, e1, s, reps, disk, measure)
+        self._tune_levels(e0, e1, s, reps, disk, measure)
         self._fuse_pointwise_chains(e0, e1, s, reps, disk, measure)
         torch.cuda.synchronize(self.device)
         if cache_path and (len(disk) != n0 or mode == 'force'):
@@ -1656,6 +1766,44 @@
                             self.ops[pidx] = ('nop', None, pname + '[fused into ' + name + ']', pwhere)
                             self.proto_patch_wino = wd
 
+    def _tune_levels(self, e0, e1, s, reps, disk, measure):
+        lib = self.lib
+        tiles = [L.TILE_64x64, L.TILE_64x128, L.TILE_128x64, L.TILE_128x128_W8, L.TILE_64x128_S3, L.TILE_32x64_K2, L.TILE_128x128,
+                 L.TILE_128x128_S3, L.TILE_128x128_W8_S3, L.TILE_256x128_W8, L.TILE_256x128_W8_S3, L.TILE_128x256_W8]
+        if os.environ.get('YOLACT_AMD_WGEMM', '1') == '1':
+            tiles = tiles + [L.TILE_WG_128x256]
+        for idx, d, where in self.level_ops:
+            name = self.ops[idx][2]
+            key = 'winolv' + str((d.B, tuple((d.lv[l].H, d.lv[l].W) for l in range(d.nlev)), d.C, d.Cout, d.act, d.nseg)) + self.mode_key
+            default = d.tile
+            ent = disk.get(key)
+            if ent is not None:
+                d.tile = int(ent[0])
+                if lib.ymi_conv3x3_winograd_levels_f32(C.byref(d), s) != 0:
+                    ent = None
+            if ent is None:
+                self.tune_misses += 1
+                best_t, best_ms = default, 0.0
+                if measure:
+                    best_ms = 1e30
+                    for t in tiles:
+                        d.tile = t | L.TILE_H2
+                        if lib.ymi_conv3x3_winograd_levels_f32(C.byref(d), s) != 0:
+                            continue
+                        for _ in range(2):
+                            e0.record()
+                            for _ in range(reps):
+                                lib.ymi_conv3x3_winograd_levels_f32(C.byref(d), s)
+                            e1.record()
+                            e1.synchronize()
+                            ms = e0.elapsed_time(e1) / reps
+                            if ms < best_ms:
+                                best_t, best_ms = d.tile, ms
+                    disk[key] = [int(best_t), round(best_ms, 4)]
+                ent = (best_t, best_ms)
+            d.tile = int(ent[0])
+            self.wino_table.append((name, 'F4/%sp' % L.TILE_NAMES.get(d.tile & 255, '-'), 0.0, float(ent[1]), 0.0, float(ent[1])))
+
     def set_winograd(self, key, on: bool):
         for idx, direct_op, wino_op, _ in self.wino_toggle.get(key, []):
             self.ops[idx] = wino_op if on else direct_op
```

New measurement: 2349 (median of 6 runs). About the same (+0.9%).
